# medical-genomics-group/VAMPomi

Measured on AMD Instinct MI355X. Metric: VAMP iterations/s (+ achieved HBM GB/s of the A/A^T kernels), higher is better.
Workload: dtype f64

## Files before the change

include/vampomi.h:

```cpp
#ifndef VAMPOMI_H
#define VAMPOMI_H

#include <stdint.h>

#ifdef __cplusplus
extern "C" {
#endif

#define VAMPOMI_ABI_VERSION 3
#define VAMPOMI_MAX_L 64
#define VAMPOMI_UNIQUE_ID_BYTES 128

typedef enum {
    VAMPOMI_OK = 0,
    VAMPOMI_ERR_ARG = 1,
    VAMPOMI_ERR_HIP = 2,
    VAMPOMI_ERR_RCCL = 3,
    VAMPOMI_ERR_IO = 4,
    VAMPOMI_ERR_NAN_PHEN = 5,
    VAMPOMI_ERR_STATE = 6,
    VAMPOMI_ERR_OOM = 7,
    VAMPOMI_ERR_MODEL = 8
} vampomi_status;

// ... 57 lines not shown

vampomi_status vampomi_denoise_bin(vampomi_ctx* ctx, const double* p1, double tau1, double* z1,
                                   double* sum_d, int mem);

typedef struct {
    double gam1, h2;
    int max_iter, CG_max_iter;
    double CG_err_tol;
    int EM_max_iter;
    double EM_err_thr, rho;
    int learn_vars, learn_prior_delay;
    double stop_criteria_thr, merge_vars_thr;
    int L;
    double vars[VAMPOMI_MAX_L];
    double probs[VAMPOMI_MAX_L];
    uint64_t seed;
    const char* out_dir;
    const char* out_name;
    int verbosity;
    const double* true_signal;
    const double* x1hat_init;
    int batch_rhs;
    const char* model;
} vampomi_params;

typedef struct {
    int iterations_run;
    int* cg_iters;
    int* ons_iters;
    int* L_hist;
    double* params;
    double* metrics;
    double* x1_hist;
    double* r1_hist;
    double* x1_final;
    double probs_final[VAMPOMI_MAX_L];
    double vars_final[VAMPOMI_MAX_L];
    int L_final;
    int64_t a_passes_ref;
    int64_t a_passes_exec;
    double* prior_hist;
} vampomi_result;

void vampomi_params_default(vampomi_params* p);
vampomi_status vampomi_infere(vampomi_ctx* ctx, const vampomi_params* p, vampomi_result* r);
vampomi_status vampomi_vamp_begin(vampomi_ctx* ctx, const vampomi_params* p, vampomi_result* r);
vampomi_status vampomi_vamp_step(vampomi_ctx* ctx, int* stopped);
vampomi_status vampomi_vamp_end(vampomi_ctx* ctx);
vampomi_status vampomi_step_phases(vampomi_ctx* ctx, double* solve_s, double* step_s);

vampomi_status vampomi_assoc_loo(vampomi_ctx* ctx, const double* est, double* pvals, double* stats,
                                 int mem);
vampomi_status vampomi_assoc_se(vampomi_ctx* ctx, const double* r1, double gam1, double* pvals, int mem);

vampomi_status vampomi_test_metrics(vampomi_ctx* ctx, const double* est, double* r2, double* corr2, int mem);

typedef struct {
    int64_t launches;
    double ms_total;
    double bytes_total;
    double flops_total;
    int64_t timed;
    double ms_timed;
} vampomi_kernel_stat;

typedef struct {
    vampomi_kernel_stat ax;
    vampomi_kernel_stat atx;
    vampomi_kernel_stat ax_k[4];
    vampomi_kernel_stat atx_k[4];
    int64_t a_passes_exec;
    int64_t host_syncs;
    vampomi_kernel_stat loo;
    vampomi_kernel_stat op;
    vampomi_kernel_stat op_k[4];
    vampomi_kernel_stat coll;
} vampomi_stats;

vampomi_status vampomi_set_timing(vampomi_ctx* ctx, int on);
vampomi_status vampomi_get_stats(vampomi_ctx* ctx, vampomi_stats* out);
vampomi_status vampomi_reset_stats(vampomi_ctx* ctx);

vampomi_status vampomi_dev_set_variant(vampomi_ctx* ctx, int which, int variant);
vampomi_status vampomi_dev_time_pass(vampomi_ctx* ctx, int which, int K, int reps, double* avg_ms);
vampomi_status vampomi_dev_read_ceiling(vampomi_ctx* ctx, int reps, double* us_med, double* bytes, int* variant);
vampomi_status vampomi_dev_kernel_name(const vampomi_ctx* ctx, int which, int K, int mode, char* out, int cap);
vampomi_status vampomi_dev_ax_plan(int64_t N, int64_t M, int cus, int variant, int K, int* T, int* TR, int* S,
                                   int* grid, int* nslots, char* name, int cap);
vampomi_status vampomi_dev_op_plan(int64_t N, int64_t M, int cus, int variant, int K, int* T, int* S, int* TR,
                                   int* grid, int64_t* nslots, char* name, int cap);
vampomi_status vampomi_dev_op_lds(int64_t N, int64_t M, int cus, int variant, int K, int64_t* out);
vampomi_status vampomi_dev_op_timestamps(vampomi_ctx* ctx, unsigned long long* out, int cap, int* n);
vampomi_status vampomi_dev_mem_plan(int64_t N, int64_t Mt, int nranks, int rank, int cus, int probit, int writer,
                                    int64_t* bytes);
vampomi_status vampomi_dev_op_apply(vampomi_ctx* ctx, int K, const double* ar, const double* qo, const double* p,
                                    const double* z, const double* beta, double diag, double tau, double gam2,
                                    double* d, double* ad, double* dp);

#ifdef __cplusplus
}
#endif
#endif
```

vampomi_amd/__init__.py:

```python
from __future__ import annotations

import ctypes as C
from dataclasses import dataclass, field
from typing import Optional, Sequence

import numpy as np

from ._lib import (CLI_PATH, GEN_GAUSS, GEN_METH, LIB_PATH, MAX_L, MEM_DEVICE, MEM_HOST, UNIQUE_ID_BYTES,
                   Params, Result, ShardDesc, Stats, VampomiError, check, load)

__all__ = ["Data", "Vamp", "VampOptions", "divide_work", "comm_unique_id", "VampomiError", "LIB_PATH", "CLI_PATH",
           "GEN_GAUSS", "GEN_METH", "load"]


def _dp(a: np.ndarray):
    return a.ctypes.data_as(C.c_void_p)


def divide_work(Mt: int, nranks: int, rank: int):
    M, S, Mm = C.c_int64(), C.c_int64(), C.c_int64()
    load().vampomi_divide_work(Mt, nranks, rank, C.byref(M), C.byref(S), C.byref(Mm))
    return M.value, S.value, Mm.value


# ... 134 lines not shown
        check(self._lib.vampomi_test_metrics(self.ctx, _dp(est), C.byref(r2), C.byref(c2), MEM_HOST))
        return r2.value, c2.value

    test_metrics.__test__ = False

    def assoc_loo(self, est: np.ndarray, mem_device: bool = False):
        est = np.ascontiguousarray(est, dtype=np.float64)
        if est.shape != (self.M,):
            raise ValueError("estimate slice must have M entries")
        pv = np.zeros(max(self.M, 1))
        st = np.zeros((max(self.M, 1), 5))
        check(self._lib.vampomi_assoc_loo(self.ctx, _dp(est), _dp(pv), _dp(st), MEM_HOST))
        return pv[: self.M], st[: self.M]

    def assoc_se(self, r1: np.ndarray, gam1: float) -> np.ndarray:
        r1 = np.ascontiguousarray(r1, dtype=np.float64)
        pv = np.zeros(max(self.M, 1))
        check(self._lib.vampomi_assoc_se(self.ctx, _dp(r1), gam1, _dp(pv), MEM_HOST))
        return pv[: self.M]

    def update_prior(self, r1: np.ndarray, gam1: float, probs, vars_scaled, EM_max_iter: int = 1,
                     EM_err_thr: float = 1e-2, learn_vars: int = 1, merge_vars_thr: float = 0.5):
        r1 = np.ascontiguousarray(r1, dtype=np.float64)
        L = C.c_int(len(probs))
        pr = np.zeros(MAX_L)
        va_ = np.zeros(MAX_L)
        pr[: L.value] = probs
        va_[: L.value] = vars_scaled
        check(self._lib.vampomi_update_prior(self.ctx, _dp(r1), gam1, C.byref(L), _dp(pr), _dp(va_), EM_max_iter,
                                             EM_err_thr, learn_vars, merge_vars_thr, MEM_HOST))
        return pr[: L.value].copy(), va_[: L.value].copy()

    def denoise_bin(self, p1: np.ndarray, tau1: float):
        p1 = np.ascontiguousarray(p1, dtype=np.float64)
        z = np.zeros(self.N)
        sd = C.c_double()
        check(self._lib.vampomi_denoise_bin(self.ctx, _dp(p1), tau1, _dp(z), C.byref(sd), MEM_HOST))
        return z, sd.value

    def denoise(self, r1: np.ndarray, gam1: float, probs: Sequence[float], vars_scaled: Sequence[float]):
        r1 = np.ascontiguousarray(r1, dtype=np.float64)
        L = len(probs)
        pr = np.ascontiguousarray(probs, dtype=np.float64)
        va = np.ascontiguousarray(vars_scaled, dtype=np.float64)
        x1 = np.zeros(max(self.M, 1))
        x1d = np.zeros(max(self.M, 1))
        s = C.c_double()
        check(self._lib.vampomi_denoise(self.ctx, _dp(r1), gam1, _dp(pr), _dp(va), L, _dp(x1), _dp(x1d),
                                        C.byref(s), MEM_HOST))
        return x1[: self.M], x1d[: self.M], s.value

    def kernel_name(self, which: int, K: int, mode: int = 0) -> str:
        buf = C.create_string_buffer(256)
        check(self._lib.vampomi_dev_kernel_name(self.ctx, which, K, mode, buf, 256))
        return buf.value.decode()

    def op_apply(self, ar, p, diag: float, tau: float, gam2: float, z=None, qo=None, beta=None):
        ar = np.ascontiguousarray(np.atleast_2d(ar), dtype=np.float64)
        p = np.ascontiguousarray(np.atleast_2d(p), dtype=np.float64)
        K = ar.shape[0]
        if ar.shape != (K, self.N) or p.shape != (K, self.M):
            raise ValueError("ar must be K x N and p K x M")
        fz = z is not None
        if fz:
            z = np.ascontiguousarray(np.atleast_2d(z), dtype=np.float64)
            qo = np.ascontiguousarray(np.atleast_2d(qo), dtype=np.float64)
            beta = np.ascontiguousarray(beta, dtype=np.float64)
        d = np.zeros((K, max(self.M, 1)))
        ad = np.zeros((K, self.N))
        dp = np.zeros(K)
        check(self._lib.vampomi_dev_op_apply(self.ctx, K, _dp(ar), _dp(qo) if fz else None, _dp(p),
                                             _dp(z) if fz else None, _dp(beta) if fz else None, diag, tau, gam2,
                                             _dp(d), _dp(ad), _dp(dp)))
        return d[:, : self.M], ad, dp

    def read_ceiling(self, reps: int = 9) -> dict:
        us, nb, var = C.c_double(), C.c_double(), C.c_int()
        check(self._lib.vampomi_dev_read_ceiling(self.ctx, int(reps), C.byref(us), C.byref(nb), C.byref(var)))
        return {"us_med": us.value, "bytes": nb.value, "GBs": nb.value / (us.value * 1e-6) / 1e9,
                "variant": ("lockstep 8-wave workgroups, one per CU", "1 MiB chunk per wave")[var.value]}

    def set_variant(self, which: int, variant: int):
        check(self._lib.vampomi_dev_set_variant(self.ctx, which, variant))

    def all_ok(self, local_ok: bool) -> bool:
        out = C.c_int()
        check(self._lib.vampomi_all_ok(self.ctx, 1 if local_ok else 0, C.byref(out)))
        return bool(out.value)

    def comm_abort(self):
        check(self._lib.vampomi_comm_abort(self.ctx))

    def set_timing(self, on: bool = True, period: int = 1):
        check(self._lib.vampomi_set_timing(self.ctx, (max(1, int(period)) if on else 0)))

    def stats(self) -> Stats:
        s = Stats()
        check(self._lib.vampomi_get_stats(self.ctx, C.byref(s)))
        return s

    def reset_stats(self):
        check(self._lib.vampomi_reset_stats(self.ctx))


@dataclass
class VampOptions:
    gam1: float = 1e-6
    h2: float = 0.5
    max_iter: int = 50
    CG_max_iter: int = 500
    CG_err_tol: float = 1e-5
    EM_max_iter: int = 1
    EM_err_thr: float = 1e-2
    rho: float = 0.5
    learn_vars: int = 1
    learn_prior_delay: int = 1
    stop_criteria_thr: float = 0.01
    merge_vars_thr: float = 0.5
    vars: Sequence[float] = (0, 1e-06, 6e-06, 3e-05, 2e-04, 1e-03, 6e-03, 3e-02, 2e-01, 1e+00)
    probs: Sequence[float] = (9.9e-01, 5e-03, 2.5e-03, 1.25e-03, 6.25e-04, 3.125e-04, 1.5625e-04, 7.8125e-05,
                              3.90625e-05, 3.90625e-05)
    seed: int = 0x5EED5EED
    out_dir: str = ""
    out_name: str = ""
    verbosity: int = 0
    batch_rhs: int = 4
    model: str = "linear"

    def to_struct(self) -> Params:
        p = Params()
        load().vampomi_params_default(C.byref(p))
        for k in ("gam1", "h2", "max_iter", "CG_max_iter", "CG_err_tol", "EM_max_iter", "EM_err_thr", "rho",
                  "learn_vars", "learn_prior_delay", "stop_criteria_thr", "merge_vars_thr", "seed", "verbosity",
                  "batch_rhs"):
            setattr(p, k, getattr(self, k))
        if len(self.vars) != len(self.probs) or not 1 <= len(self.vars) <= MAX_L:
            raise ValueError("vars and probs must have the same length (1..64)")
        p.L = len(self.vars)
        for j, (v, q) in enumerate(zip(self.vars, self.probs)):
            p.vars[j] = v
            p.probs[j] = q
        self._keep = [self.out_dir.encode(), self.out_name.encode(), self.model.encode()]
        p.out_dir, p.out_name, p.model = self._keep
        return p


class Vamp:

    def __init__(self, data: Data, opts: Optional[VampOptions] = None, true_signal: Optional[np.ndarray] = None,
                 x1hat_init: Optional[np.ndarray] = None):
        self.data = data
        self.opts = opts or VampOptions()
        self.true_signal = None if true_signal is None else np.ascontiguousarray(true_signal, dtype=np.float64)
        self.x1hat_init = None if x1hat_init is None else np.ascontiguousarray(x1hat_init, dtype=np.float64)
        self._active = False

    def _prepare(self, keep_hist: bool):
        o, M = self.opts, self.data.M
        it = o.max_iter
        self.p = o.to_struct()
        if self.true_signal is not None:
            self.p.true_signal = self.true_signal.ctypes.data
        if self.x1hat_init is not None:
            self.p.x1hat_init = self.x1hat_init.ctypes.data
        self.cg = np.zeros(it, dtype=np.int32)
        self.ons = np.zeros(it, dtype=np.int32)
# ... 70 lines not shown
```

vampomi_amd/_lib.py:

```python
from __future__ import annotations

import ctypes as C
import os

try:
    import torch
except Exception:
    torch = None

HERE = os.path.dirname(os.path.abspath(__file__))
LIB_PATH = os.environ.get("VAMPOMI_LIB") or os.path.join(HERE, "lib", "libvampomi.so")
CLI_PATH = os.path.join(HERE, "bin", "main_meth.exe")

MAX_L = 64
UNIQUE_ID_BYTES = 128
MEM_HOST, MEM_DEVICE = 0, 1
GEN_GAUSS, GEN_METH = 0, 1

STATUS = {
    0: "OK", 1: "ERR_ARG", 2: "ERR_HIP", 3: "ERR_RCCL", 4: "ERR_IO",
    5: "ERR_NAN_PHEN", 6: "ERR_STATE", 7: "ERR_OOM", 8: "ERR_MODEL",
}


# ... 19 lines not shown
        ("stop_criteria_thr", C.c_double), ("merge_vars_thr", C.c_double),
        ("L", C.c_int),
        ("vars", C.c_double * MAX_L), ("probs", C.c_double * MAX_L),
        ("seed", C.c_uint64),
        ("out_dir", C.c_char_p), ("out_name", C.c_char_p),
        ("verbosity", C.c_int),
        ("true_signal", C.c_void_p), ("x1hat_init", C.c_void_p),
        ("batch_rhs", C.c_int),
        ("model", C.c_char_p),
    ]


class Result(C.Structure):
    _fields_ = [
        ("iterations_run", C.c_int),
        ("cg_iters", C.POINTER(C.c_int)), ("ons_iters", C.POINTER(C.c_int)), ("L_hist", C.POINTER(C.c_int)),
        ("params", C.POINTER(C.c_double)), ("metrics", C.POINTER(C.c_double)),
        ("x1_hist", C.POINTER(C.c_double)), ("r1_hist", C.POINTER(C.c_double)),
        ("x1_final", C.POINTER(C.c_double)),
        ("probs_final", C.c_double * MAX_L), ("vars_final", C.c_double * MAX_L),
        ("L_final", C.c_int),
        ("a_passes_ref", C.c_int64), ("a_passes_exec", C.c_int64),
        ("prior_hist", C.POINTER(C.c_double)),
    ]


class KernelStat(C.Structure):
    _fields_ = [("launches", C.c_int64), ("ms_total", C.c_double), ("bytes_total", C.c_double),
                ("flops_total", C.c_double), ("timed", C.c_int64), ("ms_timed", C.c_double)]


class Stats(C.Structure):
    _fields_ = [("ax", KernelStat), ("atx", KernelStat), ("ax_k", KernelStat * 4), ("atx_k", KernelStat * 4),
                ("a_passes_exec", C.c_int64), ("host_syncs", C.c_int64), ("loo", KernelStat),
                ("op", KernelStat), ("op_k", KernelStat * 4), ("coll", KernelStat)]


_D = C.POINTER(C.c_double)
_P = C.c_void_p
SIGNATURES = {
    "vampomi_abi_version": (C.c_int, []),
    "vampomi_last_error": (C.c_char_p, []),
    "vampomi_divide_work": (None, [C.c_int64, C.c_int, C.c_int, C.POINTER(C.c_int64), C.POINTER(C.c_int64),
                                   C.POINTER(C.c_int64)]),
    "vampomi_comm_unique_id": (C.c_int, [_P]),
    "vampomi_open": (C.c_int, [C.POINTER(ShardDesc), C.POINTER(_P)]),
    "vampomi_close": (None, [_P]),
    "vampomi_shard_info": (C.c_int, [_P, C.POINTER(C.c_int64), C.POINTER(C.c_int64), C.POINTER(C.c_int64)]),
    "vampomi_sync": (C.c_int, [_P]),
    "vampomi_barrier": (C.c_int, [_P]),
    "vampomi_barrier_timeout": (C.c_int, [_P, C.c_double]),
    "vampomi_load_meth_file": (C.c_int, [_P, C.c_char_p]),
    "vampomi_load_meth_host": (C.c_int, [_P, _P, C.c_int64]),
    "vampomi_generate_meth": (C.c_int, [_P, C.c_uint64, C.c_int]),
    "vampomi_read_phen": (C.c_int, [_P, C.c_char_p, C.c_int]),
    "vampomi_set_phen": (C.c_int, [_P, _P, C.c_int]),
    "vampomi_get_phen": (C.c_int, [_P, _P]),
    "vampomi_simulate_phen": (C.c_int, [_P, C.c_uint64, C.c_double, C.c_double, _P]),
    "vampomi_simulate_phen_binary": (C.c_int, [_P, C.c_uint64, C.c_double, C.c_double, _P]),
    "vampomi_get_marker_stats": (C.c_int, [_P, _P, _P]),
    "vampomi_read_markers": (C.c_int, [_P, C.c_int64, C.c_int64, _P]),
    "vampomi_ax": (C.c_int, [_P, _P, _P, C.c_int]),
    "vampomi_atx": (C.c_int, [_P, _P, _P, C.c_int]),
    "vampomi_lmmse_mult": (C.c_int, [_P, _P, C.c_double, C.c_double, _P, C.c_int]),
    "vampomi_pcg": (C.c_int, [_P, _P, _P, C.c_double, C.c_double, C.c_int, C.c_int, C.c_double, _P,
                              C.POINTER(C.c_int), C.c_int]),
    "vampomi_test_metrics": (C.c_int, [_P, _P, C.POINTER(C.c_double), C.POINTER(C.c_double), C.c_int]),
    "vampomi_assoc_loo": (C.c_int, [_P, _P, _P, _P, C.c_int]),
    "vampomi_assoc_se": (C.c_int, [_P, _P, C.c_double, _P, C.c_int]),
    "vampomi_update_prior": (C.c_int, [_P, _P, C.c_double, C.POINTER(C.c_int), _P, _P, C.c_int, C.c_double,
                                        C.c_int, C.c_double, C.c_int]),
    "vampomi_denoise_bin": (C.c_int, [_P, _P, C.c_double, _P, C.POINTER(C.c_double), C.c_int]),
    "vampomi_denoise": (C.c_int, [_P, _P, C.c_double, _P, _P, C.c_int, _P, _P, C.POINTER(C.c_double), C.c_int]),
    "vampomi_params_default": (None, [C.POINTER(Params)]),
    "vampomi_infere": (C.c_int, [_P, C.POINTER(Params), C.POINTER(Result)]),
    "vampomi_vamp_begin": (C.c_int, [_P, C.POINTER(Params), C.POINTER(Result)]),
    "vampomi_vamp_step": (C.c_int, [_P, C.POINTER(C.c_int)]),
    "vampomi_step_phases": (C.c_int, [_P, C.POINTER(C.c_double), C.POINTER(C.c_double)]),
    "vampomi_vamp_end": (C.c_int, [_P]),
    "vampomi_set_timing": (C.c_int, [_P, C.c_int]),
    "vampomi_get_stats": (C.c_int, [_P, C.POINTER(Stats)]),
    "vampomi_reset_stats": (C.c_int, [_P]),
    "vampomi_dev_set_variant": (C.c_int, [_P, C.c_int, C.c_int]),
    "vampomi_dev_time_pass": (C.c_int, [_P, C.c_int, C.c_int, C.c_int, C.POINTER(C.c_double)]),
    "vampomi_dev_read_ceiling": (C.c_int, [_P, C.c_int, C.POINTER(C.c_double), C.POINTER(C.c_double),
                                           C.POINTER(C.c_int)]),
    "vampomi_dev_kernel_name": (C.c_int, [_P, C.c_int, C.c_int, C.c_int, C.c_char_p, C.c_int]),
    "vampomi_dev_mem_plan": (C.c_int, [C.c_int64, C.c_int64, C.c_int, C.c_int, C.c_int, C.c_int, C.c_int, _P]),
    "vampomi_dev_ax_plan": (C.c_int, [C.c_int64, C.c_int64, C.c_int, C.c_int, C.c_int, _P, _P, _P, _P, _P, C.c_char_p,
                                      C.c_int]),
    "vampomi_dev_op_plan": (C.c_int, [C.c_int64, C.c_int64, C.c_int, C.c_int, C.c_int, _P, _P, _P, _P, _P, C.c_char_p,
                                      C.c_int]),
    "vampomi_dev_op_lds": (C.c_int, [C.c_int64, C.c_int64, C.c_int, C.c_int, C.c_int, _P]),
    "vampomi_dev_op_apply": (C.c_int, [_P, C.c_int, _P, _P, _P, _P, _P, C.c_double, C.c_double, C.c_double, _P, _P,
                                       _P]),
    "vampomi_dev_op_timestamps": (C.c_int, [_P, _P, C.c_int, C.POINTER(C.c_int)]),
    "vampomi_all_ok": (C.c_int, [_P, C.c_int, C.POINTER(C.c_int)]),
    "vampomi_comm_abort": (C.c_int, [_P]),
}

_lib = None


def load() -> C.CDLL:
    global _lib
    if _lib is None:
        if not os.path.exists(LIB_PATH):
            raise ImportError(f"{LIB_PATH} not built: run `python -m vampomi_amd.build`")
        lib = C.CDLL(LIB_PATH, mode=C.RTLD_GLOBAL)
        other = bool(os.environ.get("VAMPOMI_LIB"))
        for name, (res, args) in SIGNATURES.items():
            if other and not hasattr(lib, name):
                continue
            f = getattr(lib, name)
            f.restype = res
            f.argtypes = args
        _lib = lib
    return _lib


def check(status: int) -> None:
    if status != 0:
        msg = load().vampomi_last_error()
        raise VampomiError(status, msg.decode() if msg else "")
```

vampomi_amd/csrc/atax_team.hip:

```cpp
#include <hip/hip_ext.h>

#include <algorithm>
#include <cstdio>
#include <mutex>
#include <string>

#include "kdev.h"

namespace vk {

typedef unsigned int v4u __attribute__((ext_vector_type(4)));
typedef unsigned int v2u __attribute__((ext_vector_type(2)));

#ifndef TM_FMA
#define TM_FMA 1
#endif
#ifndef TM_SAFE
#define TM_SAFE 0
#endif
#ifndef TM_TS
#define TM_TS 0
#endif
#ifndef TM_TEAMS_BY_XCD
#define TM_TEAMS_BY_XCD 1
// ... 59 lines not shown
    return __builtin_bit_cast(double, ((unsigned long long)hi << 32) | lo);
}

template <int CTRL>
__device__ __forceinline__ double dpp_d(double v) {
    const unsigned long long u = __builtin_bit_cast(unsigned long long, v);
    const unsigned lo = (unsigned)__builtin_amdgcn_mov_dpp((int)(unsigned)u, CTRL, 0xf, 0xf, false);
    const unsigned hi = (unsigned)__builtin_amdgcn_mov_dpp((int)(unsigned)(u >> 32), CTRL, 0xf, 0xf, false);
    return __builtin_bit_cast(double, ((unsigned long long)hi << 32) | lo);
}
__device__ __forceinline__ double pack_d(unsigned lo, unsigned hi) {
    return __builtin_bit_cast(double, ((unsigned long long)hi << 32) | lo);
}
__device__ __forceinline__ double swap16_sum(double v) {
    const unsigned long long u = __builtin_bit_cast(unsigned long long, v);
    const auto l = __builtin_amdgcn_permlane16_swap((unsigned)u, (unsigned)u, false, false);
    const auto h = __builtin_amdgcn_permlane16_swap((unsigned)(u >> 32), (unsigned)(u >> 32), false, false);
    return pack_d(l[0], h[0]) + pack_d(l[1], h[1]);
}
__device__ __forceinline__ void swap32(double a, double b, double& r0, double& r1) {
    const unsigned long long ua = __builtin_bit_cast(unsigned long long, a), ub = __builtin_bit_cast(unsigned long long, b);
    const auto l = __builtin_amdgcn_permlane32_swap((unsigned)ua, (unsigned)ub, false, false);
    const auto h = __builtin_amdgcn_permlane32_swap((unsigned)(ua >> 32), (unsigned)(ub >> 32), false, false);
    r0 = pack_d(l[0], h[0]);
    r1 = pack_d(l[1], h[1]);
}
template <int G>
__device__ __forceinline__ double group_sum(double v) {
    if constexpr (G >= 2) v = v + dpp_d<0xb1>(v);
    if constexpr (G >= 4) v = v + dpp_d<0x4e>(v);
    if constexpr (G >= 8) v = v + dpp_d<0x141>(v);
    if constexpr (G >= 16) v = v + dpp_d<0x140>(v);
    if constexpr (G >= 32) v = swap16_sum(v);
    if constexpr (G >= 64) {
        double a, b;
        swap32(v, v, a, b);
        v = a + b;
    }
    return v;
}

template <int N>
__device__ __forceinline__ double tree_sum(const double* x, int s) {
    if constexpr (N == 1) {
        return x[0];
    } else {
        constexpr int H = N / 2;
        return tree_sum<H>(x, s) + tree_sum<N - H>(x + H * s, s);
    }
}

__device__ __forceinline__ void tm_poll(v4u& dst, const unsigned long long* p) {
    asm volatile("global_load_dwordx4 %0, %1, off sc1" : "=v"(dst) : "v"(p) : "memory");
}
template <int N>
__device__ __forceinline__ void tm_wait(v4u& r) {
    asm volatile("s_waitcnt vmcnt(%1)" : "+v"(r) : "n"(N) : "memory");
}
__device__ __forceinline__ void tm_load8(v2u& dst, const double* p) {
    asm volatile("global_load_dwordx2 %0, %1, off" : "=v"(dst) : "v"(p) : "memory");
}
template <int N>
__device__ __forceinline__ void tm_wait2(v4u& r, v2u& q) {
    asm volatile("s_waitcnt vmcnt(%2)" : "+v"(r), "+v"(q) : "n"(N) : "memory");
}
__device__ __forceinline__ void tm_publish(unsigned long long* p, const v4u& v) {
    asm volatile("s_nop 4\n\tglobal_store_dwordx4 %0, %1, off sc1\n\ts_nop 1" ::"v"(p), "v"(v) : "memory");
}
__device__ __forceinline__ void tm_publish_l2(unsigned long long* p, const v4u& v) {
    asm volatile("s_nop 4\n\tglobal_store_dwordx4 %0, %1, off\n\ts_nop 1" ::"v"(p), "v"(v) : "memory");
}

template <class Tp>
__device__ __forceinline__ Tp* tm_chk(Tp* p, const void* lo, const void* hi, unsigned code, unsigned* err) {
#if TM_SAFE
    if ((const char*)p < (const char*)lo || (const char*)p >= (const char*)hi) {
        __hip_atomic_fetch_or(err, 1u | (code << 1), __ATOMIC_RELAXED, __HIP_MEMORY_SCOPE_SYSTEM);
        return (Tp*)lo;
    }
#endif
    return p;
}

template <int K, int S, int F, int L, int P, bool COMM, int E, bool FMA, int KP>
__device__ __forceinline__ void atax_team_body(const double* __restrict__ X, int64_t ld, int64_t N, int64_t M,
                                               const double* __restrict__ mave, const double* __restrict__ msig,
                                               const OpArgs& a, int T, int TR, int ilv,
                                               const int* __restrict__ gate) {
    extern __shared__ __attribute__((aligned(16))) double lds[];
    double* s_beta = lds;
    if (a.fold.on) {
        double& s_go = lds[kOpMaxK];
        if (threadIdx.x == 0) {
            CgState cs = *a.fold.src;
            double r[3 * kMaxRhs];
#pragma unroll
            for (int q = 0; q < 3 * kMaxRhs; ++q) r[q] = q < 3 * cs.K ? a.fold.red[q] : 0.0;
            const bool ran = cg_decide_into(cs, r, a.fold.it, a.fold.mask);
            if (blockIdx.x == 0) {
                *a.fold.dst = cs;
                cg_publish(cs, ran, a.fold.it, a.fold.mirror, a.fold.flag, a.fold.seq, a.fold.pack);
            }
            s_go = cs.any ? 1.0 : 0.0;
#pragma unroll
            for (int k = 0; k < kOpMaxK; ++k) s_beta[k] = cs.beta[k];
        }
        __syncthreads();
        if (s_go == 0.0) return;
    } else if (gate && !*gate) {
        return;
    }
    const double* beta = a.fold.on ? s_beta : a.beta;
    static_assert(K + KP <= kMaxRhs, "partial slots per team");
#if TM_TS
    const unsigned long long ts0 = __builtin_amdgcn_s_memrealtime();
#endif
    const int dbg = TM_ABL ? TM_ABL : (TM_DBG || !COMM) ? a.dbg : 0;
    constexpr int CW = COMM ? 7 : 8;
    constexpr int RS = tm_rows_per_step(COMM, E);
    static_assert(E == 1 || E == 2, "doubles per lane per load");
    constexpr int RING = F + L + 1;
    static_assert(COMM || L == 0, "without a hand-off the column is finished in its own step");
    static_assert(!COMM || (P >= 1 && P <= L), "polls in flight");
    static_assert(!COMM || P < RING, "a poll's slot is consumed before it is reissued");
    const int wave = threadIdx.x >> 6, lane = threadIdx.x & 63;
    const int g = blockIdx.x >> 3;
    const int member = g % T;
    const int nteams = gridDim.x / T;
#if TM_TEAMS_BY_XCD
    const int team = g / T + (nteams >> 3) * (int)(blockIdx.x & 7);
#else
    const int team = (blockIdx.x & 7) + 8 * (g / T);
#endif
    const int64_t cs = ilv ? nteams : 1;
    const int64_t mb = ilv ? team : (int64_t)team * M / nteams;
    const int n = (int)(ilv ? (M - team + nteams - 1) / nteams : (int64_t)(team + 1) * M / nteams - mb);
    const int64_t nmax = (M + nteams - 1) / nteams;
    const int64_t gwords = (M + gridDim.x) * kOpMaxK * T * 2;
    const int64_t r0 = (int64_t)member * TR;
    const int nrows = (int)(N - r0 < TR ? N - r0 : TR);
    constexpr bool QFULL = tm_qfull(K, S, COMM, E);
    const TmLds lay = tm_lds(K, S, COMM, E, TR < N ? TR : N);
    const int QS = (int)lay.qs;
    double* q_lds = lds + lay.q;
    double* s_part = lds + lay.part;
    double* s_tot = lds + lay.tot;
    const int jb = 64 * E * wave + E * lane;
    const int nbytes = (E == 2 ? (nrows + 1) & ~1 : nrows) * 8;

    if (COMM && wave == CW) {
        const int nq = K * T;
        unsigned long long* xg = a.xg + (int64_t)team * nmax * nq * 2;
        unsigned long long* dummy = a.xg + gwords + (int64_t)blockIdx.x * 2 * K;
        const bool qv = (lane >> 5) < K && (lane & 31) < T;
        const int ql2 = qv ? 2 * ((lane >> 5) * T + (lane & 31)) : 0;
        const int nq2 = 2 * nq;
        const int csi = (int)cs;
        const unsigned tag = a.tag;
        const double* scp = msig;
#pragma unroll
        for (int k = 0; k < K; ++k) {
            if (lane == 1 + k) scp = a.p.p[k];
            if (lane == 1 + K + k && ((a.fuse >> k) & 1)) scp = a.z.p[k];
        }
        scp += mb;
        double bk[K], dpacc[K];
#pragma unroll
        for (int k = 0; k < K; ++k) {
            bk[k] = ((a.fuse >> k) & 1) ? beta[k] : 0.0;
            dpacc[k] = 0.0;
        }
        v4u pl[RING];
        v2u ps[RING];
        bool dead = false;
        unsigned nslow = 0, nspin = 0;
        if (n > 0) {
            bool l2 = false;
            {
                unsigned long long* hdr = a.xg + gwords + (int64_t)gridDim.x * 2 * kOpMaxK + (int64_t)team * T;
                unsigned xcc;
                asm volatile("s_getreg_b32 %0, hwreg(HW_REG_XCC_ID)" : "=s"(xcc));
                xcc &= 0xf;
                if (lane == 0)
                    __hip_atomic_store(hdr + member, ((unsigned long long)tag << 32) | xcc, __ATOMIC_RELAXED,
                                       __HIP_MEMORY_SCOPE_AGENT);
                unsigned long long h = 0;
                for (unsigned spins = 0;; ++spins) {
                    h = lane < T ? __hip_atomic_load(hdr + lane, __ATOMIC_RELAXED, __HIP_MEMORY_SCOPE_AGENT)
                                 : ((unsigned long long)tag << 32) | xcc;
                    if (__all((unsigned)(h >> 32) == tag)) break;
                    if (spins >= kTmMaxSpins) {
                        dead = true;
                        if (lane == 0) __hip_atomic_store(a.err, 1u, __ATOMIC_RELAXED, __HIP_MEMORY_SCOPE_SYSTEM);
                        break;
                    }
                    __builtin_amdgcn_s_sleep(2);
                }
                l2 = !dead && __all((unsigned)h == xcc);
                if (dbg & 32) l2 = false;
            }
            for (int base = -F; base - L < n; base += RING) {
#pragma unroll
                for (int i = 0; i < RING; ++i) {
                    const int m = base + i;
                    if (dbg & 4096) {
                        __syncthreads();
                        continue;
                    }
                    const int ci = m - L + P, cf = m - L;
                    const int cic = ci < 0 ? 0 : ci < n ? ci : n - 1;
                    tm_load8(ps[(i + RING - L + P) % RING], scp + cic * csi);
                    tm_poll(pl[(i + RING - L + P) % RING], xg + (cic * nq2 + ql2));
                    v4u& g = pl[(i + RING - L) % RING];
                    v2u& sc = ps[(i + RING - L) % RING];
                    if (!(dbg & 1)) tm_wait2<3 * P>(g, sc);
                    if (cf >= 0 && cf < n) {
                        if (!(__all(g.y == tag && g.w == tag) || dead || (dbg & 1))) {
#pragma unroll 1
                            for (unsigned spins = 0;; ++spins) {
                                if (dbg & 64) {
                                    nslow += spins == 0;
                                    nspin++;
                                }
                                if (spins >= kTmMaxSpins) {
                                    dead = true;
                                    if (lane == 0) __hip_atomic_store(a.err, 1u, __ATOMIC_RELAXED, __HIP_MEMORY_SCOPE_SYSTEM);
                                    break;
                                }
                                __builtin_amdgcn_s_sleep(2);
                                tm_poll(g, tm_chk(xg + ((int64_t)cf * nq2 + ql2), a.xg, a.xg + gwords, 64, a.err));
                                tm_wait<0>(g);
                                if (__all(g.y == tag && g.w == tag)) break;
                            }
                        }
                        double v = qv ? __builtin_bit_cast(double, ((unsigned long long)g.z << 32) | g.x) : 0.0;
                        if (dbg & 512) {
                            for (int o = T >> 1; o > 0; o >>= 1) v += __shfl_xor(v, o, 64);
                        } else if (!(dbg & 256)) {
                            v = group_sum<32>(v);
                        }
                        const double scv = __builtin_bit_cast(double, ((unsigned long long)sc.y << 32) | sc.x);
                        const double sg = readlane_d(scv, 0);
                        const bool own = (cf & (T - 1)) == member;
                        const int64_t mg = mb + cf * csi;
                        double tsc[K], dval[K], pdir[K];
#pragma unroll
                        for (int k = 0; k < K; ++k) {
                            double t = sg * readlane_d(v, 32 * k);
                            t *= a.scale;
                            double p = readlane_d(scv, 1 + k);
                            if ((a.fuse >> k) & 1) p = readlane_d(scv, 1 + K + k) + bk[k] * p;
                            double val = t * a.tau;
                            val += a.gam2 * p;
                            tsc[k] = t;
                            dval[k] = val;
                            pdir[k] = p;
                        }
#pragma unroll
                        for (int k = 0; k < K; ++k)
                            if (lane == 0) s_tot[(cf & 1) * K + k] = (dbg & 128) ? 0.0 : sg * dval[k];
                        if (own) {
#pragma unroll
                            for (int k = 0; k < K; ++k) {
                                if (lane == 0 && !(dbg & 1024)) {
                                    if (a.sraw.p[0]) a.sraw.p[k][mg] = tsc[k];
                                    *tm_chk(a.d.p[k] + mg, a.d.p[k], a.d.p[k] + M, 128, a.err) = dval[k];
                                }
                                dpacc[k] += dval[k] * pdir[k];
                            }
                        }
                    }
                    __syncthreads();
                    if (lane < K && !(dbg & 2)) {
                        const bool real = m >= 0 && m < n;
                        double v = 0.0;
                        if (real) v = tree_sum<CW>(s_part + (m & 1) * CW * K + lane, K);
                        const unsigned long long u = __builtin_bit_cast(unsigned long long, v);
                        const v4u gr = {(unsigned)u, tag, (unsigned)(u >> 32), tag};
                        unsigned long long* dst =
                            tm_chk(real ? xg + ((int64_t)m * nq2 + (lane * T + member) * 2) : dummy + 2 * lane, a.xg,
                                   a.xg + gwords + (int64_t)gridDim.x * 2 * kOpMaxK, 512, a.err);
                        if (l2)
                            tm_publish_l2(dst, gr);
                        else
                            tm_publish(dst, gr);
                    }
                }
            }
#pragma unroll
            for (int s = 0; s < RING; ++s) tm_wait2<0>(pl[s], ps[s]);
            if ((dbg & 64) && lane == 0) {
                __hip_atomic_fetch_add(a.err + 1, nslow, __ATOMIC_RELAXED, __HIP_MEMORY_SCOPE_SYSTEM);
                __hip_atomic_fetch_add(a.err + 2, nspin, __ATOMIC_RELAXED, __HIP_MEMORY_SCOPE_SYSTEM);
                __hip_atomic_fetch_add(a.err + 3, (unsigned)n, __ATOMIC_RELAXED, __HIP_MEMORY_SCOPE_SYSTEM);
            }
        }
        if (lane == 0) {
#pragma unroll
            for (int k = 0; k < K; ++k) red_put(a.ro, (int64_t)blockIdx.x * K + k, dpacc[k]);
        }
        asm volatile("s_waitcnt vmcnt(0)" ::: "memory");
        __syncthreads();
        return;
    }

#pragma unroll
    for (int s = 0; s < S; ++s) {
        const int jl = RS * s + jb;
        if (jl >= QS) continue;
#pragma unroll
        for (int k = 0; k < K; ++k) {
#pragma unroll
            for (int h = 0; h < E; ++h) {
                double q = 0.0;
                if (jl + h < nrows) {
                    const int64_t j = r0 + jl + h;
                    q = a.ar.p[k][j] / a.diag;
                    if ((a.fuse >> k) & 1) q = q + beta[k] * a.qo.p[k][j];
                }
                q_lds[k * QS + jl + h] = q;
            }
        }
    }
    double bk[K];
#pragma unroll
    for (int k = 0; k < K; ++k) bk[k] = ((a.fuse >> k) & 1) ? beta[k] : 0.0;
    const double* pkp = mave;
    if (lane == 1) pkp = msig;
#pragma unroll
    for (int k = 0; k < K; ++k) {
        if (lane == 2 + k) pkp = a.p.p[k];
        if (lane == 2 + K + k && ((a.fuse >> k) & 1)) pkp = a.z.p[k];
    }
#pragma unroll
    for (int k = 0; k < KP; ++k)
        if (lane == 2 + 2 * K + k) pkp = a.px.p[k];
    pkp += mb;
    bool valid[S];
#pragma unroll
    for (int s = 0; s < S; ++s) valid[s] = RS * s + jb < nrows;
    double acc[K][S][E];
#pragma unroll
    for (int k = 0; k < K; ++k)
#pragma unroll
        for (int s = 0; s < S; ++s)
#pragma unroll
            for (int e = 0; e < E; ++e) acc[k][s][e] = 0.0;
    double dpacc[K];
#pragma unroll
    for (int k = 0; k < K; ++k) dpacc[k] = 0.0;
    constexpr int KPA = KP > 0 ? KP : 1;
    double accp[KPA][S][E];
#pragma unroll
    for (int k = 0; k < KPA; ++k)
#pragma unroll
        for (int s = 0; s < S; ++s)
#pragma unroll
            for (int e = 0; e < E; ++e) accp[k][s][e] = 0.0;

    double xr[RING][S][E];
    double pk[RING];
    const char* xtile = reinterpret_cast<const char*>(X + mb * ld + r0);
    auto load = [&](int slot, int m) {
        const int64_t c = m * cs;
        pk[slot] = *tm_chk(pkp + c, pkp - mb, pkp - mb + M, 1024, a.err);
        const __amdgpu_buffer_rsrc_t rs =
            __builtin_amdgcn_make_buffer_rsrc((void*)(xtile + c * ld * 8), (short)0, nbytes, 0x00020000);
#pragma unroll
        for (int s = 0; s < S; ++s) {
            if constexpr (E == 2) {
                const v2d x = __builtin_bit_cast(v2d, __builtin_amdgcn_raw_buffer_load_b128(rs, (RS * s + jb) * 8, 0, 2));
                xr[slot][s][0] = x.x;
                xr[slot][s][E - 1] = x.y;
            } else {
                xr[slot][s][0] = __builtin_bit_cast(double, __builtin_amdgcn_raw_buffer_load_b64(rs, (RS * s + jb) * 8, 0, 2));
            }
        }
    };
    auto dot = [&](int slot, int par) {
        const double mu = readlane_d(pk[slot], 0);
        double cp[KPA];
        if constexpr (KP > 0) {
            const double sgp = readlane_d(pk[slot], 1);
#pragma unroll
            for (int k = 0; k < KP; ++k) cp[k] = sgp * readlane_d(pk[slot], 2 + 2 * K + k);
        }
        double v[K];
#pragma unroll
        for (int k = 0; k < K; ++k) v[k] = 0.0;
#pragma unroll
        for (int s = 0; s < S; ++s) {
            const double me_ = QFULL || valid[s] ? mu : 0.0;
            const int jq = QFULL || RS * s + jb < QS ? RS * s + jb : QS - E;
            double dx[E], q[K][E];
#pragma unroll
            for (int e = 0; e < E; ++e) {
                dx[e] = xr[slot][s][e] - me_;
                xr[slot][s][e] = dx[e];
            }
            if constexpr (KP > 0) {
#pragma unroll
                for (int k = 0; k < KP; ++k)
#pragma unroll
                    for (int e = 0; e < E; ++e) {
                        if constexpr (FMA)
                            accp[k][s][e] = __builtin_fma(dx[e], cp[k], accp[k][s][e]);
                        else
                            accp[k][s][e] += dx[e] * cp[k];
                    }
            }
#pragma unroll
            for (int k = 0; k < K; ++k) {
                if ((TM_DBG || TM_ABL) && (dbg & 2048)) {
                    q[k][0] = 0.5;
                    q[k][E - 1] = 0.25;
                } else if constexpr (E == 2) {
                    const v2d qq = *reinterpret_cast<const v2d*>(q_lds + k * QS + jq);
                    q[k][0] = qq.x;
                    q[k][E - 1] = qq.y;
                } else {
                    q[k][0] = q_lds[k * QS + jq];
                }
#pragma unroll
                for (int e = 0; e < E; ++e) {
                    if constexpr (FMA)
                        v[k] = __builtin_fma(dx[e], q[k][e], v[k]);
                    else
                        v[k] += dx[e] * q[k][e];
                }
            }
        }
        if (K == 2) {
            double r0, r1;
            swap32(v[0], v[K - 1], r0, r1);
            double keep = r0 + r1;
            if (dbg & 512) {
                for (int o = 16; o > 0; o >>= 1) keep += __shfl_xor(keep, o, 64);
            } else if (!(dbg & 4)) {
                keep = group_sum<32>(keep);
            }
            if ((lane & 31) == 0) s_part[(par * CW + wave) * K + (lane >> 5)] = keep;
        } else {
            if (!(dbg & 4)) v[0] = group_sum<64>(v[0]);
            if (lane == 0) s_part[(par * CW + wave) * K] = v[0];
        }
    };
    auto finish = [&](int slot, int m, const double (&tot)[K]) {
        double cc[K];
        if constexpr (COMM) {
#pragma unroll
            for (int k = 0; k < K; ++k) cc[k] = tot[k];
        } else {
            const double sg = readlane_d(pk[slot], 1);
            const bool own = (m % T) == member;
            const int64_t mg = mb + m * cs;
#pragma unroll
            for (int k = 0; k < K; ++k) {
                double t = sg * tot[k];
                t *= a.scale;
                double p = readlane_d(pk[slot], 2 + k);
                if ((a.fuse >> k) & 1) p = readlane_d(pk[slot], 2 + K + k) + bk[k] * p;
                double val = t * a.tau;
                val += a.gam2 * p;
                if (own) {
                    if (threadIdx.x == 0) {
                        if (a.sraw.p[0]) a.sraw.p[k][mg] = t;
                        a.d.p[k][mg] = val;
                    }
                    dpacc[k] += val * p;
                }
                cc[k] = sg * val;
            }
        }
#pragma unroll
        for (int s = 0; s < S; ++s) {
            if (dbg & 8) break;
#pragma unroll
            for (int k = 0; k < K; ++k)
#pragma unroll
                for (int e = 0; e < E; ++e) {
                    if constexpr (FMA)
                        acc[k][s][e] = __builtin_fma(xr[slot][s][e], cc[k], acc[k][s][e]);
                    else
                        acc[k][s][e] += xr[slot][s][e] * cc[k];
                }
        }
    };
    if (n > 0) {
        for (int base = -F;; base += RING) {
            if (base - L >= n) break;
#pragma unroll
            for (int i = 0; i < RING; ++i) {
                const int m = base + i;
                load((i + F) % RING, m + F < n ? m + F : n - 1);
                if (m >= 0 && m < n) dot(i, m & 1);
                __syncthreads();
                const int cf = m - L;
                if (cf >= 0 && cf < n) {
                    double tot[K];
                    if (COMM) {
#pragma unroll
                        for (int k = 0; k < K; ++k) tot[k] = s_tot[(cf & 1) * K + k];
                    } else {
#pragma unroll
                        for (int k = 0; k < K; ++k) {
                            double t = 0.0;
#pragma unroll
                            for (int w = 0; w < CW; ++w) t += s_part[((m & 1) * CW + w) * K + k];
                            tot[k] = t;
                        }
                    }
                    finish((i + RING - L) % RING, cf, tot);
                }
            }
        }
    }
    double* dst = a.part + (int64_t)team * kMaxRhs * ld + r0;
#pragma unroll
    for (int s = 0; s < S; ++s) {
        const int jl = RS * s + jb;
        if (jl >= nrows) continue;
#pragma unroll
        for (int k = 0; k < K; ++k)
#pragma unroll
            for (int e = 0; e < E; ++e)
                if (jl + e < nrows) dst[(int64_t)k * ld + jl + e] = acc[k][s][e];
        if constexpr (KP > 0) {
#pragma unroll
            for (int k = 0; k < KP; ++k)
#pragma unroll
                for (int e = 0; e < E; ++e)
                    if (jl + e < nrows) dst[(int64_t)(K + k) * ld + jl + e] = accp[k][s][e];
        }
    }
    if constexpr (COMM) {
        __syncthreads();
    } else if (threadIdx.x == 0) {
#pragma unroll
        for (int k = 0; k < K; ++k) red_put(a.ro, (int64_t)blockIdx.x * K + k, dpacc[k]);
    }
    if (wave == 0) ticket_sum_blocks<K>(a.ro);
#if TM_TS
    if (a.ts && threadIdx.x == 0) {
        unsigned xcc, hw;
        asm volatile("s_getreg_b32 %0, hwreg(HW_REG_XCC_ID)" : "=s"(xcc));
        asm volatile("s_getreg_b32 %0, hwreg(HW_REG_HW_ID)" : "=s"(hw));
        unsigned long long* t = a.ts + 4 * (int64_t)blockIdx.x;
        t[0] = ts0;
        t[1] = __builtin_amdgcn_s_memrealtime();
        t[2] = xcc;
// ... 147 lines not shown
    if (S > c.maxS) return false;
    for (int K = 1; K <= kOpMaxK; ++K)
        if (tm_lds(K, S, c.comm, c.E, std::min<int64_t>(TR, N)).words * 8 > kTmLdsMaxBytes) return false;
    OpPlan p{};
    p.grid = grid;
    p.S = S;
    p.T = T;
    p.TR = (int)TR;
    p.cfg = cfg;
    p.nslots = grid / T;
    (void)M;
    *out = p;
    return true;
}

bool team_lds_layout(const OpPlan& pl, int64_t N, int K, int64_t out[6]) {
    if (pl.T < 1 || pl.cfg < 0 || pl.cfg >= kTmNCfg || K < 1 || K > kOpMaxK || N < 1) return false;
    const TmCfg& c = kTmCfg[pl.cfg];
    const TmLds l = tm_lds(K, pl.S, c.comm, c.E, std::min<int64_t>(pl.TR, N));
    out[0] = kTmLdsHead;
    out[1] = l.q;
    out[2] = l.qs;
    out[3] = l.part;
    out[4] = l.tot;
    out[5] = l.words;
    return true;
}

template <int K, int S, int C, bool PL>
static hipError_t launch_tm(const Shard& s, const OpPlan& pl, const OpArgs& a, hipStream_t st, const Timing& tm,
                            const int* gate, int* occ) {
    constexpr TmCfg c = kTmCfg[C];
    static_assert(!PL || K == 1, "the head-start kernel has one operator system");
    void (*kern)(const double*, int64_t, int64_t, int64_t, const double*, const double*, OpArgs, int, int, int,
                 const int*);
    if constexpr (PL)
        kern = atax_team_plain_kernel<S, c.F, c.L, c.P, c.comm, c.E, (bool)TM_FMA>;
    else
        kern = atax_team_kernel<K, S, c.F, c.L, c.P, c.comm, c.E, (bool)TM_FMA>;
    const size_t lds = (size_t)tm_lds(K, S, c.comm, c.E, std::min<int64_t>(pl.TR, s.N)).words * sizeof(double);
    if (lds > (size_t)kTmLdsMaxBytes) return hipErrorInvalidValue;
    static std::atomic<unsigned long long> allowed{0};
    if (const hipError_t e = lds_allow(reinterpret_cast<const void*>(kern), allowed, (int)kTmLdsMaxBytes))
        return e;
    if (occ) {
        if (hipOccupancyMaxActiveBlocksPerMultiprocessor(occ, kern, kTmThreads, lds) != hipSuccess) *occ = 0;
        return hipSuccess;
    }
    hipExtLaunchKernelGGL(kern, dim3(pl.grid), dim3(kTmThreads), lds, st, tm.start, tm.stop, 0, s.X, s.ld, s.N, s.M,
                          s.mave, s.msig, a, pl.T, pl.TR, c.ilv ? 1 : 0, gate);
    return hipSuccess;
}

static constexpr int tm_plain_maxS(int cfg) {
    return cfg == 0 ? 8 : cfg == 2 ? 3 : cfg == 3 ? 4 : cfg == 4 ? 5 : 0;
}

template <int K, int C, int S, bool PL>
static hipError_t launch_tm_if(const Shard& s, const OpPlan& pl, const OpArgs& a, hipStream_t st, const Timing& tm,
                               const int* gate, int* occ) {
    if constexpr (S <= (PL ? tm_plain_maxS(C) : kTmCfg[C].maxS))
        return launch_tm<K, S, C, PL>(s, pl, a, st, tm, gate, occ);
    return hipErrorInvalidValue;
}

template <int K, int C, bool PL>
static hipError_t launch_tm_s(int S, const Shard& s, const OpPlan& pl, const OpArgs& a, hipStream_t st,
                        const Timing& tm, const int* gate, int* occ) {
    switch (S) {
        case 1: return launch_tm_if<K, C, 1, PL>(s, pl, a, st, tm, gate, occ);
        case 2: return launch_tm_if<K, C, 2, PL>(s, pl, a, st, tm, gate, occ);
        case 3: return launch_tm_if<K, C, 3, PL>(s, pl, a, st, tm, gate, occ);
        case 4: return launch_tm_if<K, C, 4, PL>(s, pl, a, st, tm, gate, occ);
        case 5: return launch_tm_if<K, C, 5, PL>(s, pl, a, st, tm, gate, occ);
        case 6: return launch_tm_if<K, C, 6, PL>(s, pl, a, st, tm, gate, occ);
        case 7: return launch_tm_if<K, C, 7, PL>(s, pl, a, st, tm, gate, occ);
        case 8: return launch_tm_if<K, C, 8, PL>(s, pl, a, st, tm, gate, occ);
        case 9: return launch_tm_if<K, C, 9, PL>(s, pl, a, st, tm, gate, occ);
        case 10: return launch_tm_if<K, C, 10, PL>(s, pl, a, st, tm, gate, occ);
        default: return hipErrorInvalidValue;
    }
}

template <int K, bool PL = false>
static hipError_t launch_tm_c(const Shard& s, const OpPlan& pl, const OpArgs& a, hipStream_t st, const Timing& tm,
                        const int* gate, int* occ = nullptr) {
    if constexpr (PL) {
        switch (pl.cfg) {
            case 0: return launch_tm_s<1, 0, true>(pl.S, s, pl, a, st, tm, gate, occ);
            case 2: return launch_tm_s<1, 2, true>(pl.S, s, pl, a, st, tm, gate, occ);
            case 3: return launch_tm_s<1, 3, true>(pl.S, s, pl, a, st, tm, gate, occ);
            case 4: return launch_tm_s<1, 4, true>(pl.S, s, pl, a, st, tm, gate, occ);
            default: return hipErrorInvalidValue;
        }
    }
    switch (pl.cfg) {
        case 0: return launch_tm_s<K, 0, false>(pl.S, s, pl, a, st, tm, gate, occ);
        case 1: return launch_tm_s<K, 1, false>(pl.S, s, pl, a, st, tm, gate, occ);
        case 2: return launch_tm_s<K, 2, false>(pl.S, s, pl, a, st, tm, gate, occ);
        case 3: return launch_tm_s<K, 3, false>(pl.S, s, pl, a, st, tm, gate, occ);
        case 4: return launch_tm_s<K, 4, false>(pl.S, s, pl, a, st, tm, gate, occ);
        case 5: return launch_tm_s<K, 5, false>(pl.S, s, pl, a, st, tm, gate, occ);
        case 6: return launch_tm_s<K, 6, false>(pl.S, s, pl, a, st, tm, gate, occ);
        default: return hipErrorInvalidValue;
    }
}

hipError_t atax_team(const Shard& s, const OpPlan& pl, int K, const OpArgs& a, hipStream_t st, const Timing& tm,
                     const int* gate) {
    if (pl.T < 1 || pl.grid < pl.T || pl.grid % pl.T) return hipErrorInvalidValue;
    if (pl.T > 1 && (!a.xg || !a.err || a.tag == 0)) return hipErrorInvalidValue;
    if (s.M <= 0) return hipSuccess;
    hipError_t e = hipErrorInvalidValue;
    switch (K) {
        case 1: e = launch_tm_c<1>(s, pl, a, st, tm, gate); break;
        case 2: e = launch_tm_c<2>(s, pl, a, st, tm, gate); break;
        default: break;
    }
    if (e != hipSuccess) return e;
    return hipGetLastError();
}

hipError_t atax_team_plain(const Shard& s, const OpPlan& pl, const OpArgs& a, hipStream_t st, const Timing& tm,
                           const int* gate) {
    if (pl.T < 1 || pl.grid < pl.T || pl.grid % pl.T) return hipErrorInvalidValue;
    if (pl.T > 1 && (!a.xg || !a.err || a.tag == 0)) return hipErrorInvalidValue;
    for (int k = 0; k < kTmPlain; ++k)
        if (!a.px.p[k]) return hipErrorInvalidValue;
    if (s.M <= 0) return hipSuccess;
    if (const hipError_t e = launch_tm_c<1, true>(s, pl, a, st, tm, gate)) return e;
    return hipGetLastError();
}

bool ax_team_plan(int64_t N, int64_t M, int cus, AxPlan* out) {
    if (N < 1 || cus < 8) return false;
    constexpr int RS = tm_rows_per_step(false, 2);
    for (int T = 1; T <= kTmMaxT; T *= 2) {
        if (cus / (8 * T) < 1) break;
        const int grid = (cus / (8 * T)) * 8 * T;
        const int64_t TR = T == 1 ? N : ((N + T - 1) / T + 127) / 128 * 128;
        if ((int64_t)(T - 1) * TR >= N) continue;
        const int S = (int)((TR + RS - 1) / RS);
        if (S > kAxTmMaxS) continue;
        AxPlan p{};
        p.variant = kAxTeam;
        p.T = T;
        p.TR = (int)TR;
        p.S = S;
        p.groups = grid;
        p.nslots = grid / T;
        p.rows = N;
        p.tiles = 1;
        p.total = M;
        p.sa = p.nslots;
        p.sb = 1;
        *out = p;
        return true;
    }
    return false;
}

template <int S, int K, bool FU>
static void launch_axt(const Shard& s, const AxPlan& pl, CPtrs x, double* part, hipStream_t st, const Timing& tm,
                       const AxFuse& fu) {
    hipExtLaunchKernelGGL((ax_team_kernel<S, K, FU>), dim3(pl.groups), dim3(kTmThreads), 0, st, tm.start, tm.stop, 0,
                          s.X, s.ld, s.N, s.M, s.mave, s.msig, x, part, fu, pl.T, pl.TR);
}

template <int S>
// ... 87 lines not shown
```

vampomi_amd/csrc/ctx.h:

```cpp
#pragma once
#include <hip/hip_runtime.h>
#include <rccl/rccl.h>

#include <cstdint>
#include <initializer_list>
#include <memory>
#include <string>
#include <utility>
#include <vector>

#include "../../include/vampomi.h"
#include "kernels.h"

vampomi_status fail(vampomi_status s, const std::string& msg);

#define HIPCHK(expr)                                                                                  \
    do {                                                                                              \
        hipError_t _e = (expr);                                                                       \
        if (_e != hipSuccess)                                                                         \
            return fail(VAMPOMI_ERR_HIP, std::string(#expr) + ": " + hipGetErrorString(_e));          \
    } while (0)

#define NCCLCHK(expr)                                                                                 \
    do {                                                                                              \
// ... 13 lines not shown
    explicit CollScope(vampomi_ctx* c);
    ~CollScope();
    vampomi_ctx* prev;
};
struct VampRun;
class IterWriter;
struct LoopbackComm;
struct ShmComm;
std::shared_ptr<ShmComm> shm_join(const void* id, int P, int rank, double limit_s, std::string* err);
std::string shm_allreduce(ShmComm& s, int rank, double* buf, size_t n, uint64_t seq, const char* site, int line,
                          double limit_s);
void shm_poison(ShmComm& s, const std::string& why);

struct TimedLaunch {
    hipEvent_t a, b;
    int cls;
    int K;
    double bytes, flops;
};

enum : int { SL_DP = 0, SL_CG = 4, SL_SYNC = 16, SL_NSYNC = 256, SL_LOCAL = SL_SYNC + SL_NSYNC, SL_NLOCAL = 128,
             SL_CGI = SL_LOCAL + SL_NLOCAL, SL_CHECK = SL_CGI + 16, SL_AGREE = SL_CHECK + 8, SL_CHAIN = SL_AGREE + 8, SL_TOTAL = 512, SL_BARRIER = SL_TOTAL - 1 };

struct vampomi_ctx {
    int rank = 0, nranks = 1, device = 0;
    int64_t N = 0, Mt = 0, M = 0, S = 0, Mm = 0, ld = 0;
    double alpha_scale = 1.0;
    double sqrtN = 1.0;
    hipStream_t st = nullptr;
    bool mr_tail = true;
    double coll_limit_s = 0.0;
    bool mr_tail_req = true;
    bool cg_fold = true;
    bool team_reg = false;
    hipEvent_t team_ev = nullptr;
    ncclComm_t comm = nullptr;
    bool use_comm = false;
    std::shared_ptr<LoopbackComm> loopback;
    std::shared_ptr<ShmComm> shm;
    uint64_t coll_seq = 0;
    bool aborted = false;

    double* X = nullptr;
    double* mave = nullptr;
    double* msig = nullptr;
    double* y = nullptr;
    std::vector<double> y_host;
    bool have_X = false, have_y = false;

    vk::AxPlan axp{};
    int atx_variant = vk::kAtxDefault, loo_variant = vk::kLooDefault;
    double* ax_part = nullptr;
    double* red_part = nullptr;
    size_t red_cap = 0;
    double* scal = nullptr;
    double* h_scal = nullptr;
    double* d_hscal = nullptr;
    unsigned* ticket = nullptr;
    unsigned long long* h_flag = nullptr;
    unsigned long long* d_flag = nullptr;
    unsigned long long sync_seq = 0;
    vk::CgState* cgs = nullptr;
    vk::CgMirror* h_cgm = nullptr;
    vk::CgMirror* d_cgm = nullptr;
    vk::OpPlan opp{};
    int op_variant = vk::kOpDefault;
    bool op_ready = false;
    bool op_ok_mine = false;
    bool op_ok = false;
    bool op_agreed = false;
    int op_variant_req = vk::kOpDefault;
    int cus = 0;
    double* op_part = nullptr;
    int64_t op_part_slots = 0;
    double* op_nvec = nullptr;
    unsigned long long* op_xg = nullptr;
    size_t op_xg_words = 0;
    unsigned op_tag = 0;
    vk::OpPlan opp_hs{};
    bool hs_ok_mine = false;
    bool hs_ok = false;
    bool hs_on = true;
    bool hs_on_req = true;
    unsigned long long* op_ts = nullptr;
    double* nbuf = nullptr;
    double* mbuf = nullptr;

    bool timing = false;
    int tperiod = 1;
    int64_t tcount[5][vk::kMaxRhs] = {};
    std::vector<TimedLaunch> pending;
    std::vector<hipEvent_t> ev_pool;
    vampomi_stats stats{};

    std::unique_ptr<VampRun> run;
    std::unique_ptr<IterWriter> writer;

    vk::Shard shard() const { return vk::Shard{X, ld, N, M, mave, msig}; }
    vampomi_ctx();
    ~vampomi_ctx();
};

vampomi_status dev_alloc(double** p, size_t n);
void dev_free(double*& p);
vampomi_status host_sync(vampomi_ctx* c);
vampomi_status wait_flag(vampomi_ctx* c, unsigned long long seq, int word = 0);
vampomi_status sync_stream(vampomi_ctx* c, hipStream_t st);
vampomi_status allreduce_dev(vampomi_ctx* c, double* buf, size_t n, const char* site = __builtin_FUNCTION(),
                             int line = __builtin_LINE());
vampomi_status sum_over_ranks(vampomi_ctx* c, double local, double* total, const char* site = __builtin_FUNCTION(),
                              int line = __builtin_LINE());
void comm_abort(vampomi_ctx* c, const std::string& why);
void resolve_timing(vampomi_ctx* c);
TimedLaunch launch_stat(vampomi_ctx* c, int cls, int K, double bytes, double flops);
void drop_launches(vampomi_ctx* c, size_t pending_mark, const vampomi_stats& before);
void release_ctx_resources(vampomi_ctx* c);

vampomi_status ax_dev(vampomi_ctx* c, int K, const double* const* x, double* outbase,
                      const vk::AxFuse* fu = nullptr, const vk::DotArgs* tail = nullptr);
vampomi_status atx_dev(vampomi_ctx* c, int K, const double* const* u, double* const* out, int mode, double tau,
                       double gam2, const double* const* p, const int* gate = nullptr,
                       const double* const* zf = nullptr, const double* beta = nullptr, bool dp = true,
                       double* const* sraw = nullptr);
vampomi_status lmmse_dev(vampomi_ctx* c, int K, const double* const* v, double* const* d, double tau, double gam2,
                         double* nscratch);

class DotBatch {
   public:
    explicit DotBatch(vampomi_ctx* c) : c_(c) {}
    vampomi_status add(std::initializer_list<vk::DotTerm> terms, int64_t n, bool sync, double* out);
    struct Group {
        std::vector<vk::DotTerm> terms;
        bool sync;
        double* out;
    };
    vampomi_status add_many(int64_t n, const std::vector<Group>& groups, const vk::G1Chain* chain = nullptr,
                            const double* chain_of = nullptr,
                            const std::vector<std::pair<const double*, double*>>& copies = {});
    vampomi_status add_pair(int64_t na, const std::vector<Group>& ga, const vk::G1Chain* chain,
                            const double* chain_of, const std::vector<std::pair<const double*, double*>>& ca,
                            int64_t nb, const std::vector<Group>& gb,
                            const std::vector<std::pair<const double*, double*>>& cb);
    vampomi_status sink(int nq, bool sync, double* out, vk::RedOut* ro);
    vampomi_status flush();
    bool empty() const { return sinks_.empty(); }
    const double* dev_result(const double* out) const;
    vampomi_status reduce_now();
    double* dev_slot(const double* out) const;
    hipStream_t stream() const;

   private:
    vampomi_status build(const std::vector<Group>& groups, const vk::G1Chain* chain, const double* chain_of,
                         const std::vector<std::pair<const double*, double*>>& copies, vk::DotArgs& a,
                         vk::RedOut& ro);
    struct Sink {
        int slot, count;
        double* out;
    };
    vampomi_ctx* c_;
    int nsync_ = 0, nlocal_ = 0;
    int nred_ = 0;
    unsigned long long last_seq_ = 0;
    std::vector<Sink> sinks_;
};

inline vk::DotTerm T(const double* a, const double* b, int op = vk::DOT) { return vk::DotTerm{a, b, op}; }

struct CgSystem {
    const double* v = nullptr;
    double* mu = nullptr;
    bool mu0_nonzero = false;
    const double* atx0 = nullptr;
    double* W = nullptr;
    double* S = nullptr;
    double* AW = nullptr;
    bool onsager = false;
    int iters = 0;
    double *r = nullptr, *z = nullptr, *p = nullptr, *d = nullptr;
};
struct HeadStart {
    double* abern = nullptr;
    const double* xnext = nullptr;
    double* axnext = nullptr;
    bool used = false;
};
enum class PreMode { normal, ahead, queued };
vampomi_status pcg_run(vampomi_ctx* c, const std::vector<CgSystem*>& sys, double tau, double gam2, int max_iter,
                       double tol, double* nscratch, int64_t* ref_passes, DotBatch* init,
                       const double* extra_x = nullptr, double* ex_out = nullptr, bool onepass = false,
                       const double* const* ar0 = nullptr, HeadStart* hs = nullptr,
                       const vk::Prelude* pre = nullptr, PreMode pm = PreMode::normal);
vampomi_status op_prepare(vampomi_ctx* c);
vampomi_status op_agree(vampomi_ctx* c);
vampomi_status headstart_available(vampomi_ctx* c, bool* yes);
unsigned* op_err_dev(vampomi_ctx* c);
vampomi_status op_check_err(vampomi_ctx* c);
vampomi_status op_dev(vampomi_ctx* c, int K, const vk::OpArgs& a, const int* gate, bool reduce = true,
                      bool divide = true);
vampomi_status op_dev_plain(vampomi_ctx* c, const vk::OpArgs& a, const double* const* px, double* const* out,
                            const int* gate);
```

vampomi_amd/csrc/engine.cpp:

```cpp
#include <hip/hip_runtime.h>
#include <rccl/rccl.h>

#include <algorithm>
#include <atomic>
#include <cfloat>
#include <chrono>
#include <condition_variable>
#include <map>
#include <mutex>
#include <cmath>
#include <cstdio>
#include <cstdlib>
#include <cstring>
#include <memory>
#include <string>
#include <thread>
#include <vector>

#include <fcntl.h>
#include <unistd.h>

#include "ctx.h"
#include "hostio.h"
#include "writer.h"
// ... 948 lines not shown
    c->op_part_slots = 0;
    c->op_ready = false;
    c->op_agreed = false;
    if (c->h_scal) (void)hipHostFree(c->h_scal);
    c->h_scal = nullptr;
    if (c->ticket) (void)hipFree(c->ticket);
    c->ticket = nullptr;
    if (c->h_flag) (void)hipHostFree(c->h_flag);
    c->h_flag = nullptr;
    if (c->h_cgm) (void)hipHostFree(c->h_cgm);
    c->h_cgm = nullptr;
    if (c->cgs) (void)hipFree(c->cgs);
    c->cgs = nullptr;
    if (c->comm) {
        if (nccl_settle(c, ncclCommFinalize(c->comm), "ncclCommFinalize", 30.0) == VAMPOMI_OK && c->comm)
            (void)ncclCommDestroy(c->comm);
        else if (c->comm)
            (void)ncclCommAbort(c->comm);
    }
    c->comm = nullptr;

    if (c->st) (void)hipStreamDestroy(c->st);
    c->st = nullptr;
}

extern "C" void vampomi_close(vampomi_ctx* c) { delete c; }

extern "C" vampomi_status vampomi_open(const vampomi_shard_desc* d, vampomi_ctx** out) {
    if (!d || !out) return fail(VAMPOMI_ERR_ARG, "null argument");
    *out = nullptr;
    if (d->N < 2 || d->Mt < 1 || d->nranks < 1 || d->rank < 0 || d->rank >= d->nranks)
        return fail(VAMPOMI_ERR_ARG, "invalid shard description (N >= 2, Mt >= 1, 0 <= rank < nranks)");
    if (d->nranks > 1 && !d->comm_id) return fail(VAMPOMI_ERR_ARG, "nranks > 1 needs a communicator id");
    if (d->Mt < d->nranks) return fail(VAMPOMI_ERR_ARG, "every rank needs at least one marker (Mt >= nranks)");
    std::unique_ptr<vampomi_ctx> c(new vampomi_ctx());
    c->rank = d->rank;
    c->nranks = d->nranks;
    c->N = d->N;
    c->Mt = d->Mt;
    c->alpha_scale = d->alpha_scale == 0.0 ? 1.0 : d->alpha_scale;
    vampomi_divide_work(c->Mt, c->nranks, c->rank, &c->M, &c->S, &c->Mm);
    c->ld = (c->N + 15) / 16 * 16;
    c->sqrtN = std::sqrt((double)c->N);
    int ndev = 0;
    HIPCHK(hipGetDeviceCount(&ndev));
    if (ndev < 1) return fail(VAMPOMI_ERR_HIP, "no HIP device visible");
    c->device = d->device >= 0 ? d->device : c->rank % ndev;
    HIPCHK(hipSetDevice(c->device));
    HIPCHK(hipStreamCreateWithFlags(&c->st, hipStreamNonBlocking));
    team_gate_join(c.get());
    const int64_t Mx = std::max<int64_t>(c->M, 1);
    c->axp = vk::ax_plan(c->N, Mx);
    STCHK(dev_alloc(&c->mave, Mx));
    STCHK(dev_alloc(&c->msig, Mx));
    STCHK(dev_alloc(&c->y, c->ld));
    HIPCHK(hipMemsetAsync(c->y, 0, c->ld * 8, c->st));
    STCHK(dev_alloc(&c->ax_part, (size_t)c->axp.nslots * vk::kMaxRhs * c->ld));
    c->red_cap = red_capacity(Mx);
    STCHK(dev_alloc(&c->red_part, c->red_cap));
    c->writer.reset(new IterWriter());
    STCHK(c->writer->open(c.get()));
    STCHK(dev_alloc(&c->scal, SL_TOTAL));
    HIPCHK(hipHostMalloc((void**)&c->h_scal, SL_TOTAL * sizeof(double), hipHostMallocMapped | hipHostMallocCoherent));
    HIPCHK(hipHostGetDevicePointer((void**)&c->d_hscal, c->h_scal, 0));
    HIPCHK(hipHostMalloc((void**)&c->h_flag, 64, hipHostMallocMapped | hipHostMallocCoherent));
    std::memset(c->h_flag, 0, 64);
    HIPCHK(hipHostGetDevicePointer((void**)&c->d_flag, c->h_flag, 0));
    HIPCHK(hipMalloc((void**)&c->ticket, 64 * sizeof(unsigned)));
    HIPCHK(hipMemsetAsync(c->ticket, 0, 64 * sizeof(unsigned), c->st));
    STCHK(dev_alloc(&c->nbuf, (size_t)vk::kMaxRhs * c->ld));
    HIPCHK(hipMemsetAsync(c->nbuf, 0, (size_t)vk::kMaxRhs * c->ld * 8, c->st));
    STCHK(dev_alloc(&c->mbuf, (size_t)2 * vk::kMaxRhs * Mx));
    HIPCHK(hipMalloc((void**)&c->cgs, 2 * sizeof(vk::CgState)));
    HIPCHK(hipMemsetAsync(c->cgs, 0, 2 * sizeof(vk::CgState), c->st));
    HIPCHK(hipHostMalloc((void**)&c->h_cgm, vk::kCgMirrorSlots * sizeof(vk::CgMirror),
                         hipHostMallocMapped | hipHostMallocCoherent));
    std::memset(c->h_cgm, 0, vk::kCgMirrorSlots * sizeof(vk::CgMirror));
    HIPCHK(hipHostGetDevicePointer((void**)&c->d_cgm, c->h_cgm, 0));
    const char* force = std::getenv("VAMPOMI_FORCE_RCCL");
    c->use_comm = c->nranks > 1 || (force && std::atoi(force) != 0);
    if (const char* mv = std::getenv("VAMPOMI_MR_TAIL")) c->mr_tail = c->mr_tail_req = std::atoi(mv) != 0;
    if (const char* fv = std::getenv("VAMPOMI_CG_FOLD")) c->cg_fold = std::atoi(fv) != 0;
    if (const char* hv = std::getenv("VAMPOMI_HEADSTART")) c->hs_on = c->hs_on_req = std::atoi(hv) != 0;
    const char* mode = std::getenv("VAMPOMI_COMM");
    if (c->use_comm && mode && std::strcmp(mode, "loopback") == 0) {
        if (!d->comm_id) return fail(VAMPOMI_ERR_ARG, "the loopback communicator needs a communicator id");
        c->loopback = loopback_join(d->comm_id, c->nranks);
    } else if (c->use_comm && mode && std::strcmp(mode, "shm") == 0) {
        if (!d->comm_id) return fail(VAMPOMI_ERR_ARG, "the shm communicator needs a communicator id");
        std::string err;
        c->shm = shm_join(d->comm_id, c->nranks, c->rank, comm_init_timeout_s(), &err);
        if (!c->shm) return fail(VAMPOMI_ERR_STATE, err);
    } else if (c->use_comm) {
        ncclUniqueId id;
        if (d->comm_id)
            std::memcpy(&id, d->comm_id, sizeof id);
        else
            NCCLCHK(ncclGetUniqueId(&id));
        ncclConfig_t cfg = NCCL_CONFIG_INITIALIZER;
        cfg.blocking = 0;
        STCHK(nccl_settle(c.get(), ncclCommInitRankConfig(&c->comm, c->nranks, id, c->rank, &cfg),
                          "ncclCommInitRankConfig", comm_init_timeout_s()));
    }
    STCHK(sync_stream(c.get(), c->st));
    *out = c.release();
    return VAMPOMI_OK;
}

extern "C" vampomi_status vampomi_shard_info(const vampomi_ctx* c, int64_t* M, int64_t* S, int64_t* ld) {
    if (!c) return fail(VAMPOMI_ERR_ARG, "null context");
    if (M) *M = c->M;
    if (S) *S = c->S;
    if (ld) *ld = c->ld;
    return VAMPOMI_OK;
}

extern "C" vampomi_status vampomi_sync(vampomi_ctx* c) {
    if (!c) return fail(VAMPOMI_ERR_ARG, "null context");
    HIPCHK(hipSetDevice(c->device));
    STCHK(sync_stream(c, c->st));
    return VAMPOMI_OK;
}

extern "C" vampomi_status vampomi_barrier(vampomi_ctx* c) {
    CollScope cs_(c);
    if (!c) return fail(VAMPOMI_ERR_ARG, "null context");
    if (c->use_comm) STCHK(allreduce_dev(c, c->scal + SL_BARRIER, 1));
    STCHK(sync_stream(c, c->st));
    return VAMPOMI_OK;
}

extern "C" vampomi_status vampomi_barrier_timeout(vampomi_ctx* c, double seconds) {
    if (!c || !(seconds > 0)) return fail(VAMPOMI_ERR_ARG, "null context or no limit");
    c->coll_limit_s = seconds;
    const vampomi_status st = vampomi_barrier(c);
    c->coll_limit_s = 0.0;
    return st;
}

static vampomi_status ensure_X(vampomi_ctx* c) {
    if (c->X) return VAMPOMI_OK;
    return dev_alloc(&c->X, (size_t)std::max<int64_t>(c->M, 1) * (size_t)c->ld);
}

static vampomi_status finish_X(vampomi_ctx* c) {
    if (c->ld > c->N && c->M > 0)
        HIPCHK(hipMemset2DAsync(c->X + c->N, (size_t)c->ld * 8, 0, (size_t)(c->ld - c->N) * 8, (size_t)c->M, c->st));
    HIPCHK(vk::marker_stats(c->X, c->ld, c->N, c->M, (double)c->N, c->alpha_scale, c->mave, c->msig, c->st));
    STCHK(sync_stream(c, c->st));
    c->have_X = true;
    return VAMPOMI_OK;
}

extern "C" vampomi_status vampomi_load_meth_host(vampomi_ctx* c, const double* X, int64_t ld_in) {
    if (!c || (!X && c->M > 0) || ld_in < c->N) return fail(VAMPOMI_ERR_ARG, "invalid host shard");
    HIPCHK(hipSetDevice(c->device));
    STCHK(ensure_X(c));
    if (c->M > 0)
        HIPCHK(hipMemcpy2DAsync(c->X, (size_t)c->ld * 8, X, (size_t)ld_in * 8, (size_t)c->N * 8, (size_t)c->M,
                                hipMemcpyHostToDevice, c->st));
    return finish_X(c);
}

static bool pread_parallel(int fd, char* dst, size_t want, off_t off, int nt) {
    if (nt <= 1 || want < ((size_t)8 << 20)) nt = 1;
    const size_t per = ((want + nt - 1) / nt + 4095) & ~(size_t)4095;
// ... 392 lines not shown

extern "C" vampomi_status vampomi_assoc_se(vampomi_ctx* c, const double* r1, double gam1, double* pvals, int mem) {
    if (!c || (!r1 && c->M > 0) || (!pvals && c->M > 0)) return fail(VAMPOMI_ERR_ARG, "null argument");
    HIPCHK(hipSetDevice(c->device));
    const int64_t Mx = std::max<int64_t>(c->M, 1);
    STCHK(stage_in(c, r1, c->M, mem, c->mbuf));
    HIPCHK(vk::se_pvals(c->M, c->mbuf, gam1, c->N, c->mbuf + Mx, c->st));
    STCHK(stage_out(c, c->mbuf + Mx, c->M, mem, pvals));
    return VAMPOMI_OK;
}

extern "C" vampomi_status vampomi_set_timing(vampomi_ctx* c, int on) {
    if (!c) return fail(VAMPOMI_ERR_ARG, "null context");
    c->timing = on != 0;
    c->tperiod = on > 1 ? on : 1;
    for (auto& row : c->tcount)
        for (auto& n : row) n = 0;
    return VAMPOMI_OK;
}

extern "C" vampomi_status vampomi_get_stats(vampomi_ctx* c, vampomi_stats* out) {
    if (!c || !out) return fail(VAMPOMI_ERR_ARG, "null argument");
    STCHK(sync_stream(c, c->st));
    resolve_timing(c);
    *out = c->stats;
    auto fill = [](vampomi_kernel_stat& x) {
        x.ms_total = x.timed > 0 ? x.ms_timed / (double)x.timed * (double)x.launches : 0.0;
    };
    for (vampomi_kernel_stat* x : {&out->loo, &out->coll}) fill(*x);
    for (int k = 0; k < 4; ++k)
        for (vampomi_kernel_stat* x : {&out->ax_k[k], &out->atx_k[k], &out->op_k[k]}) fill(*x);
    for (auto pr : {std::make_pair(&out->ax, out->ax_k), std::make_pair(&out->atx, out->atx_k),
                    std::make_pair(&out->op, out->op_k)}) {
        int64_t n = 0;
        double ms = 0.0;
        for (int k = 0; k < 4; ++k) {
            n += pr.second[k].launches;
            ms += pr.second[k].ms_total;
        }
        if (n == pr.first->launches) pr.first->ms_total = ms;
        else fill(*pr.first);
    }
    return VAMPOMI_OK;
}

extern "C" vampomi_status vampomi_reset_stats(vampomi_ctx* c) {
    if (!c) return fail(VAMPOMI_ERR_ARG, "null context");
    STCHK(sync_stream(c, c->st));
    resolve_timing(c);
    c->stats = vampomi_stats{};
    return VAMPOMI_OK;
}

extern "C" vampomi_status vampomi_dev_set_variant(vampomi_ctx* c, int which, int variant) {
    if (!c) return fail(VAMPOMI_ERR_ARG, "null context");
    HIPCHK(hipSetDevice(c->device));
    STCHK(sync_stream(c, c->st));
    if (which == 0) {
        if (!vk::ax_variant_ok(variant)) return fail(VAMPOMI_ERR_ARG, "no such A.x variant");
        const vk::AxPlan np = vk::ax_plan(c->N, std::max<int64_t>(c->M, 1), variant);
        if (np.nslots > c->axp.nslots) {
            dev_free(c->ax_part);
            STCHK(dev_alloc(&c->ax_part, (size_t)np.nslots * vk::kMaxRhs * c->ld));
        }
        c->axp = np;
    } else if (which == 1) {
        if (!vk::atx_variant_ok(variant)) return fail(VAMPOMI_ERR_ARG, "no such A^T.u variant");
        c->atx_variant = variant;
    } else if (which == 3) {
        vk::OpPlan p{};
        if (!vk::op_plan(c->N, std::max<int64_t>(c->M, 1), c->cus > 0 ? c->cus : 256, variant, &p))
            return fail(VAMPOMI_ERR_ARG, "no such one-pass operator plan for this N");
        c->op_variant_req = variant;
        if (!c->use_comm) {
            c->op_variant = variant;
            c->op_ready = false;
        }
    } else if (which == 4) {
        return fail(VAMPOMI_ERR_ARG, "no side stream: every launch runs on the context's stream (DESIGN.md §6)");
    } else if (which == 5) {
        if (variant != 0 && variant != 1) return fail(VAMPOMI_ERR_ARG, "head start: 0 or 1");
        c->hs_on_req = variant == 1;
        if (!c->use_comm) c->hs_on = c->hs_on_req;
    } else if (which == 6) {
        if (variant != 0 && variant != 1) return fail(VAMPOMI_ERR_ARG, "multi-rank tail: 0 or 1");
        c->mr_tail_req = variant == 1;
        if (!c->use_comm) c->mr_tail = c->mr_tail_req;
    } else {
        if (!vk::loo_variant_ok(variant)) return fail(VAMPOMI_ERR_ARG, "no such association-pass variant");
        c->loo_variant = variant;
    }
    return VAMPOMI_OK;
}

extern "C" vampomi_status vampomi_dev_time_pass(vampomi_ctx* c, int which, int K, int reps, double* avg_ms) {
    if (!c || !avg_ms || K < 1 || K > (which == 0 ? 4 : which == 1 ? 3 : which == 3 ? 2 : 1) || reps < 1)
        return fail(VAMPOMI_ERR_ARG, "bad argument");
    if (!c->have_X) return fail(VAMPOMI_ERR_STATE, "no methylation data loaded");
    HIPCHK(hipSetDevice(c->device));
    if (which == 3) {
        STCHK(op_prepare(c));
        if (!c->op_ok_mine) return fail(VAMPOMI_ERR_ARG, "no one-pass operator plan for this N");
    }
    const int64_t Mx = std::max<int64_t>(c->M, 1);
    vk::CPtrs in{};
    vk::Ptrs out{};
    for (int k = 0; k < K; ++k) {
        in.p[k] = which == 0 ? c->mbuf + k * Mx : c->nbuf + k * c->ld;
        out.p[k] = which == 0 ? c->nbuf + k * c->ld : c->mbuf + k * Mx;
    }
    hipEvent_t a, b;
    HIPCHK(hipEventCreate(&a));
    HIPCHK(hipEventCreate(&b));
    HIPCHK(hipEventRecord(a, c->st));
    for (int r = 0; r < reps; ++r) {
        if (which == 0)
            HIPCHK(vk::ax_partial(c->shard(), c->axp, K, in, c->ax_part, c->st));
        else if (which == 1)
            HIPCHK(vk::atx(c->shard(), K, in, out, 1.0 / c->sqrtN, 0, 0.0, 0.0, vk::CPtrs{}, c->st, c->atx_variant));
        else if (which == 3) {
            vk::OpArgs x{};
            for (int k = 0; k < K; ++k) {
                x.ar.p[k] = c->nbuf + k * c->ld;
                x.p.p[k] = c->mbuf + k * Mx;
                x.d.p[k] = c->mbuf + (2 + k) * Mx;
            }
            x.diag = 1.0;
            x.scale = 1.0 / c->sqrtN;
            x.tau = 1.0;
            x.part = c->op_part;
            x.ro = vk::RedOut{c->red_part, c->scal + SL_DP, c->ticket, nullptr, 0, nullptr};
            if (c->opp.T > 1) {
                x.xg = c->op_xg;
                if (++c->op_tag == 0) ++c->op_tag;
                x.tag = c->op_tag;
                x.err = op_err_dev(c);
            }
            x.dbg = std::getenv("VAMPOMI_OP_DBG") ? std::atoi(std::getenv("VAMPOMI_OP_DBG")) : 0;
            if (c->opp.T > 1) x.err = op_err_dev(c);
            x.ts = c->op_ts;
            STCHK(team_launch(c, c->opp.T, [&] { return vk::atax(c->shard(), c->opp, K, x, c->st); }));
        }
        else
            HIPCHK(vk::loo_sums(c->shard(), c->nbuf, c->mbuf, c->sqrtN, c->mbuf + 3 * Mx, c->st, c->loo_variant));
    }
    HIPCHK(hipEventRecord(b, c->st));
    HIPCHK(hipEventSynchronize(b));
    if (which == 3 && std::getenv("VAMPOMI_OP_DBG") && (std::atoi(std::getenv("VAMPOMI_OP_DBG")) & 64)) {
        unsigned* w = reinterpret_cast<unsigned*>(c->h_flag + 4);
        std::fprintf(stderr, "op dbg: slow polls %u, spins %u, columns polled %u (over %d launches)\n", w[1], w[2], w[3],
                     reps);
        w[1] = w[2] = w[3] = 0;
    }
    float ms = 0.f;
    HIPCHK(hipEventElapsedTime(&ms, a, b));
    (void)hipEventDestroy(a);
    (void)hipEventDestroy(b);
    *avg_ms = (double)ms / reps;
    return VAMPOMI_OK;
}

extern "C" vampomi_status vampomi_dev_op_apply(vampomi_ctx* c, int K, const double* ar, const double* qo,
                                               const double* p, const double* z, const double* beta, double diag,
                                               double tau, double gam2, double* d, double* ad, double* dp) {
    if (!c || K < 1 || K > vk::kOpMaxK || !ar || !p || !d || !ad || !dp || (z && (!qo || !beta)))
        return fail(VAMPOMI_ERR_ARG, "bad argument");
    if (c->use_comm) return fail(VAMPOMI_ERR_ARG, "vampomi_dev_op_apply: one rank only");
    HIPCHK(hipSetDevice(c->device));
    STCHK(op_prepare(c));
    if (!c->op_ok) return fail(VAMPOMI_ERR_ARG, "no one-pass operator plan for this N");
    const int64_t Mx = std::max<int64_t>(c->M, 1);
    double* AR = c->op_nvec;
    double* Q = c->op_nvec + (int64_t)vk::kMaxRhs * c->ld;
    vk::OpArgs a{};
// ... 28 lines not shown
    }
    HIPCHK(hipMemcpyAsync(dp, c->scal + SL_DP, (size_t)K * 8, hipMemcpyDeviceToHost, c->st));
    STCHK(sync_stream(c, c->st));
    return op_check_err(c);
}

extern "C" vampomi_status vampomi_dev_op_timestamps(vampomi_ctx* c, unsigned long long* out, int cap, int* n) {
    if (!c || !out || !n) return fail(VAMPOMI_ERR_ARG, "null argument");
    if (!c->op_ts) return fail(VAMPOMI_ERR_STATE, "no timestamps (VAMPOMI_OP_TS=1 at the first operator use)");
    STCHK(sync_stream(c, c->st));
    *n = std::min(cap, 4 * c->opp.grid);
    HIPCHK(hipMemcpy(out, c->op_ts, (size_t)*n * 8, hipMemcpyDeviceToHost));
    return VAMPOMI_OK;
}

extern "C" vampomi_status vampomi_dev_ax_plan(int64_t N, int64_t M, int cus, int variant, int K, int* T, int* TR,
                                              int* S, int* grid, int* nslots, char* name, int cap) {
    if (N < 1 || M < 1 || cus < 1 || K < 1 || K > vk::kMaxRhs || !vk::ax_variant_ok(variant))
        return fail(VAMPOMI_ERR_ARG, "bad argument");
    const vk::AxPlan p = vk::ax_plan_for(N, M, cus, variant);
    if (T) *T = p.T;
    if (TR) *TR = p.TR;
    if (S) *S = p.S;
    if (grid) *grid = p.groups;
    if (nslots) *nslots = p.nslots;
    if (name && cap > 0) std::snprintf(name, (size_t)cap, "%s", vk::ax_kernel_name(K, false, p).c_str());
    return VAMPOMI_OK;
}

extern "C" vampomi_status vampomi_dev_op_plan(int64_t N, int64_t M, int cus, int variant, int K, int* T, int* S,
                                              int* TR, int* grid, int64_t* nslots, char* name, int cap) {
    vk::OpPlan p{};
    if (K < 1 || K > vk::kOpMaxK || !vk::op_plan(N, std::max<int64_t>(M, 1), cus, variant, &p))
        return fail(VAMPOMI_ERR_ARG, "no one-pass operator plan");
    if (T) *T = p.T;
    if (S) *S = p.S;
    if (TR) *TR = p.TR;
    if (grid) *grid = p.grid;
    if (nslots) *nslots = p.nslots;
    if (name && cap > 0) std::snprintf(name, (size_t)cap, "%s", vk::op_kernel_name(K, p).c_str());
    return VAMPOMI_OK;
}

extern "C" vampomi_status vampomi_dev_op_lds(int64_t N, int64_t M, int cus, int variant, int K, int64_t* out) {
    vk::OpPlan p{};
    if (!out || !vk::op_plan(N, std::max<int64_t>(M, 1), cus, variant, &p) || !vk::team_lds_layout(p, N, K, out))
        return fail(VAMPOMI_ERR_ARG, "no team plan with that system count");
    return VAMPOMI_OK;
}

extern "C" vampomi_status vampomi_dev_mem_plan(int64_t N, int64_t Mt, int nranks, int rank, int cus, int probit,
                                               int writer, int64_t* bytes) {
    if (!bytes || N < 2 || Mt < nranks || nranks < 1 || rank < 0 || rank >= nranks || cus < 1)
        return fail(VAMPOMI_ERR_ARG, "bad argument");
    int64_t M = 0, S = 0, Mm = 0;
    vampomi_divide_work(Mt, nranks, rank, &M, &S, &Mm);
    const int64_t Mx = std::max<int64_t>(M, 1), ld = (N + 15) / 16 * 16;
    int64_t total = 0;
    auto add = [&](int64_t n, int64_t elem) {
        const int64_t b = std::max<int64_t>(n, 1) * elem, g = 2 << 20;
        total += (b + g - 1) / g * g;
    };
    const vk::AxPlan axp = vk::ax_plan(N, Mx);
    add(Mx * ld, 8);
    add(Mx, 8), add(Mx, 8), add(ld, 8);
    add((int64_t)axp.nslots * vk::kMaxRhs * ld, 8);
    add((int64_t)red_capacity(Mx), 8), add((int64_t)red_capacity(Mx), 8);
    add(SL_TOTAL, 8), add(64, 4), add(64, 4);
    add((int64_t)vk::kMaxRhs * ld, 8);
    add((int64_t)2 * vk::kMaxRhs * Mx, 8);
    add((int64_t)sizeof(vk::CgState), 1);
    vk::OpPlan op{}, hs{};
    if (vk::op_plan(N, Mx, cus, vk::kOpDefault, &op)) {
        const bool h = vk::team_plain_plan(N, Mx, cus, op, &hs);
        add((int64_t)3 * vk::kMaxRhs * ld + 16, 8);
        add(std::max<int64_t>(op.nslots, h ? hs.nslots : 0) * vk::kMaxRhs * ld, 8);
        size_t w = op.T > 1 ? op_xg_words_for(Mx, op) : 0;
        if (h && hs.T > 1) w = std::max(w, op_xg_words_for(Mx, hs));
        if (w) add((int64_t)w, 8);
    }
    for (int q = 0; q < 25; ++q) add(Mx, 8);
    add(ld, 8), add((int64_t)vk::kMaxRhs * ld, 8), add((int64_t)vk::kMaxRhs * ld, 8), add(ld, 8);
    add(2 * ld, 8);
    if (probit) {
        for (int q = 0; q < 3; ++q) add(ld, 8);
        for (int q = 0; q < 3; ++q) add(Mx, 8);
    }
    (void)writer;
    *bytes = total;
    return VAMPOMI_OK;
}

static std::string op_name(const vampomi_ctx* c, int K) {
    vk::OpPlan p{};
    int cus = c->cus;
    if (cus <= 0 && hipDeviceGetAttribute(&cus, hipDeviceAttributeMultiprocessorCount, c->device) != hipSuccess) cus = 256;
    if (!vk::op_plan(c->N, std::max<int64_t>(c->M, 1), cus, c->op_variant, &p)) return "(no one-pass plan)";
    if (K == 1 + vk::kOpPlain) {
        vk::OpPlan h{};
        if (!vk::team_plain_plan(c->N, std::max<int64_t>(c->M, 1), cus, p, &h)) return "(no head-start plan)";
        return vk::team_kernel_name(K, h);
    }
    return vk::op_kernel_name(K, p);
}

extern "C" vampomi_status vampomi_dev_read_ceiling(vampomi_ctx* c, int reps, double* us_med, double* bytes,
                                                   int* variant) {
    if (!c || reps < 1 || !us_med) return fail(VAMPOMI_ERR_ARG, "bad argument");
    if (!c->have_X) return fail(VAMPOMI_ERR_STATE, "no methylation data loaded");
    HIPCHK(hipSetDevice(c->device));
    if (c->cus <= 0) HIPCHK(hipDeviceGetAttribute(&c->cus, hipDeviceAttributeMultiprocessorCount, c->device));
    STCHK(sync_stream(c, c->st));
    const int64_t n = std::max<int64_t>(c->M, 1) * c->ld;
    hipEvent_t a, b;
    HIPCHK(hipEventCreate(&a));
    HIPCHK(hipEventCreate(&b));
    double best = -1.0, best_bytes = 0.0;
    int best_kind = -1;
    for (int kind = 0; kind < 2; ++kind) {
        double nb = 0.0;
        if (vk::stream_read(c->X, n, kind, c->cus, c->st, vk::Timing{}, c->red_part, &nb) != hipSuccess) {
            (void)hipGetLastError();
            continue;
        }
        std::vector<float> ms((size_t)reps);
        for (int r = 0; r < reps; ++r) {
            HIPCHK(vk::stream_read(c->X, n, kind, c->cus, c->st, vk::Timing{a, b}, c->red_part, &nb));
            HIPCHK(hipEventSynchronize(b));
            HIPCHK(hipEventElapsedTime(&ms[(size_t)r], a, b));
        }
        std::sort(ms.begin(), ms.end());
        const double med = 1e3 * (double)ms[(size_t)reps / 2];
        if (best < 0.0 || nb / med > best_bytes / best) {
            best = med;
            best_bytes = nb;
            best_kind = kind;
        }
    }
    (void)hipEventDestroy(a);
    (void)hipEventDestroy(b);
    if (best_kind < 0) return fail(VAMPOMI_ERR_ARG, "the matrix is too small for a read-ceiling stream");
    *us_med = best;
    if (bytes) *bytes = best_bytes;
    if (variant) *variant = best_kind;
    return VAMPOMI_OK;
}

extern "C" vampomi_status vampomi_dev_kernel_name(const vampomi_ctx* c, int which, int K, int mode, char* out,
                                                  int cap) {
    if (!c || !out || cap < 1) return fail(VAMPOMI_ERR_ARG, "bad argument");
    const std::string n = which == 2   ? vk::loo_kernel_name(c->loo_variant)
                          : which == 3 ? op_name(c, K)
                          : which == 0 ? vk::ax_kernel_name(K, mode == 1, c->axp)
                                       : vk::kernel_name(1, K, mode, c->atx_variant);
    std::snprintf(out, (size_t)cap, "%s", n.c_str());
    return VAMPOMI_OK;
}
```

vampomi_amd/csrc/kdev.h:

```cpp
#pragma once
#include <hip/hip_runtime.h>

#include <cstdint>

#include "kernels.h"

namespace vk {

typedef double v2d __attribute__((ext_vector_type(2)));

__device__ __forceinline__ double wave_sum(double v) {
#pragma unroll
    for (int o = 32; o > 0; o >>= 1) v += __shfl_xor(v, o, 64);
    return v;
}

__device__ __forceinline__ void red_put(const RedOut& ro, int64_t idx, double v) {
    __hip_atomic_store(ro.part + idx, v, __ATOMIC_RELAXED, __HIP_MEMORY_SCOPE_AGENT);
}

template <int K>
__device__ __forceinline__ void ticket_sum_blocks(const RedOut& ro) {
    const int lane = threadIdx.x & 63;
    asm volatile("s_waitcnt vmcnt(0)" ::: "memory");
    unsigned old = 0;
    if (lane == 0) old = __hip_atomic_fetch_add(ro.ticket, 1u, __ATOMIC_RELAXED, __HIP_MEMORY_SCOPE_AGENT);
    old = __shfl(old, 0, 64);
    if (old != gridDim.x - 1) return;
    const int nblk = (int)gridDim.x;
#pragma unroll
    for (int k = 0; k < K; ++k) {
        double t = 0.0;
        for (int b = lane; b < nblk; b += 64)
            t += __hip_atomic_load(ro.part + (int64_t)b * K + k, __ATOMIC_RELAXED, __HIP_MEMORY_SCOPE_AGENT);
        t = wave_sum(t);
        if (lane == 0) ro.out[k] = t;
    }
    if (lane == 0) __hip_atomic_store(ro.ticket, 0u, __ATOMIC_RELAXED, __HIP_MEMORY_SCOPE_AGENT);
}

__device__ inline bool cg_decide_into(CgState& s, const double* red, int it, int mask) {
    const bool ran = s.any != 0;
    if (ran) {
        int any = 0;
#pragma unroll
        for (int k = 0; k < kMaxRhs; ++k) {
            if (k >= s.K || !s.active[k]) continue;
            if (!((mask >> k) & 1)) {
                any = 1;
                continue;
            }
            s.iters[k] = it + 1 + s.off[k];
            const double rz_new = red[3 * k], rr = red[3 * k + 1], vmu = red[3 * k + 2];
            if (s.onsager[k]) {
                const double ons = s.gam2 * vmu;
                const double rel = ons != 0 ? fabs((ons - s.prev_ons[k]) / ons) : 1;
                if (rel < 1e-8) {
                    s.active[k] = 0;
                    continue;
                }
                s.prev_ons[k] = ons;
            }
            double bt = 1.0 / s.rz[k];
            bt *= rz_new;
            s.rz[k] = rz_new;
            const double rel_err = sqrt(rr) / sqrt(s.vv[k]);
            if (rel_err < s.tol) {
                s.active[k] = 0;
                continue;
            }
            s.beta[k] = bt;
            if (s.iters[k] >= s.maxit) {
                s.active[k] = 0;
                continue;
            }
            any = 1;
        }
        s.any = any;
    }
    return ran;
}

__device__ inline void cg_publish(const CgState& s, bool ran, int it, CgMirror* mirror, unsigned long long* flag,
                                  unsigned long long seq, int pack) {
    if (pack) {
        if (flag && ran)
            __hip_atomic_store(flag, cg_pack(seq, s.any, s.iters[0], s.iters[1]), __ATOMIC_RELAXED,
                               __HIP_MEMORY_SCOPE_SYSTEM);
        return;
    }
    if (mirror) {
        CgMirror* m = mirror + (it & 1);
        __hip_atomic_store(&m->seq, seq, __ATOMIC_RELAXED, __HIP_MEMORY_SCOPE_SYSTEM);
        __hip_atomic_store(&m->any, s.any, __ATOMIC_RELAXED, __HIP_MEMORY_SCOPE_SYSTEM);
#pragma unroll
        for (int k = 0; k < kMaxRhs; ++k)
            __hip_atomic_store(&m->iters[k], s.iters[k], __ATOMIC_RELAXED, __HIP_MEMORY_SCOPE_SYSTEM);
    }
    if (flag) {
        asm volatile("s_waitcnt vmcnt(0)" ::: "memory");
        __hip_atomic_store(flag, seq, __ATOMIC_RELAXED, __HIP_MEMORY_SCOPE_SYSTEM);
    }
}

__device__ inline void cg_decide_from(CgState s, CgState* cs, const double* red, int it, CgMirror* mirror,
                                      unsigned long long* flag, unsigned long long seq, int mask, int pack = 0) {
    const bool ran = cg_decide_into(s, red, it, mask);
    if (ran) *cs = s;
    cg_publish(s, ran, it, mirror, flag, seq, pack);
}

__device__ inline void cg_decide_body(CgState* cs, const double* red, int it, CgMirror* mirror, unsigned long long* flag,
                                      unsigned long long seq, int mask, int pack = 0) {
    const CgState s = *cs;
    double r[3 * kMaxRhs];
#pragma unroll
    for (int q = 0; q < 3 * kMaxRhs; ++q) r[q] = q < 3 * s.K ? red[q] : 0.0;
    cg_decide_from(s, cs, r, it, mirror, flag, seq, mask, pack);
}

}
```

vampomi_amd/csrc/kernels.h:

```cpp
#pragma once
#include <hip/hip_runtime.h>

#include <atomic>
#include <cstdint>
#include <string>

namespace vk {

constexpr int kMaxRhs = 4;
constexpr int kMaxL = 64;
constexpr int kMaxTerms = 12;
constexpr int kRedBlocks = 1024;

struct CPtrs { const double* p[kMaxRhs]; };
struct Timing { hipEvent_t start = nullptr, stop = nullptr; };
struct RedOut {
    double* part;
    double* out;
    unsigned* ticket;
    unsigned long long* flag = nullptr;
    unsigned long long seq = 0;
    const int* gate = nullptr;
    double* out2 = nullptr;
    int split = 0;
};
struct Ptrs { double* p[kMaxRhs]; };

struct Shard {
    const double* X;
    int64_t ld, N, M;
    const double* mave;
    const double* msig;
};

struct AxPlan {
    int variant;
    int64_t rows;
    int64_t tiles;
    int64_t total;
    int64_t span;
    int64_t nband;
    int64_t sa, sb;
    int groups;
    int nslots;
    int T = 0, TR = 0, S = 0;
};
inline int64_t ax_slots(const AxPlan& p, int64_t t) { return ((t + 1) * p.sa - 1) / p.sb - (t * p.sa) / p.sb + 1; }
constexpr int kAxDefault = -1, kAxTeam = 7, kAxTeamMinT = 8, kAtxDefault = -1 , kLooDefault = 16;
AxPlan ax_plan(int64_t N, int64_t M, int variant = kAxDefault);
AxPlan ax_plan_for(int64_t N, int64_t M, int cus, int variant);
int ax_variant_count();
bool ax_variant_ok(int v);
int atx_variant_count();
bool atx_variant_ok(int v);
struct AxFuse {
    CPtrs z{};
    const double* beta = nullptr;
    const int* gate = nullptr;
};
hipError_t ax_partial(const Shard& s, const AxPlan& pl, int K, CPtrs x, double* part, hipStream_t st,
                      const Timing& tm = Timing{}, const AxFuse& fu = AxFuse{});
hipError_t stream_read(const double* x, int64_t n, int kind, int cus, hipStream_t st, const Timing& tm,
                       double* sink, double* bytes);
bool ax_team_plan(int64_t N, int64_t M, int cus, AxPlan* out);
hipError_t ax_team(const Shard& s, const AxPlan& pl, int K, CPtrs x, double* part, hipStream_t st, const Timing& tm,
                   const AxFuse& fu);
std::string ax_kernel_name(int K, bool fused, const AxPlan& pl);
hipError_t ax_reduce(const AxPlan& pl, int K, int64_t N, int64_t ld, const double* part, Ptrs out,
                     double div, hipStream_t st, const int* gate = nullptr);
hipError_t vec_div(int K, int64_t n, int64_t ld, Ptrs v, double div, hipStream_t st, const Ptrs* dst = nullptr);

int atx_blocks(int64_t M, int K, int variant);
std::string kernel_name(int which, int K, int mode, int variant);
hipError_t atx(const Shard& s, int K, CPtrs u, Ptrs out, double scale, int mode, double tau,
               double gam2, CPtrs p, hipStream_t st, int variant = kAtxDefault, const Timing& tm = Timing{},
               const int* gate = nullptr, CPtrs zf = CPtrs{}, const double* beta = nullptr, Ptrs sraw = Ptrs{});

constexpr int kOpMaxK = 2;
constexpr int kOpPlain = 3;
struct OpPlan {
    int grid;
    int S;
    int64_t nslots;
    int T = 0;
    int TR = 0;
    int cfg = 0;
};
constexpr int kOpDefault = -1;
bool op_plan(int64_t N, int64_t M, int cus, int variant, OpPlan* out);
bool op_supported(int64_t N, int K);
bool team_plan(int64_t N, int64_t M, int cus, int T, int cfg, OpPlan* out);
bool team_lds_layout(const OpPlan& pl, int64_t N, int K, int64_t out[6]);
hipError_t lds_allow(const void* kern, std::atomic<unsigned long long>& done, int bytes);
struct CgState;
struct CgMirror;
struct OpFold {
    const CgState* src = nullptr;
    CgState* dst = nullptr;
    const double* red = nullptr;
    int on = 0, it = 0, mask = 0xf, pack = 0;
    CgMirror* mirror = nullptr;
    unsigned long long* flag = nullptr;
    unsigned long long seq = 0;
};
struct OpArgs {
    CPtrs ar, qo;
    CPtrs p, z;
    const double* beta;
    int fuse;
    double diag, scale, tau, gam2;
    Ptrs d, sraw;
    CPtrs px;
    double* part;
    RedOut ro;
    unsigned long long* xg;
    unsigned tag;
    unsigned* err;
    unsigned long long* ts;
    int dbg;
    OpFold fold;
};
std::string op_kernel_name(int K, const OpPlan& pl);
std::string team_kernel_name(int K, const OpPlan& pl);
int team_occupancy(const OpPlan& pl, int K);
hipError_t atax(const Shard& s, const OpPlan& pl, int K, const OpArgs& a, hipStream_t st, const Timing& tm = Timing{},
                const int* gate = nullptr);
hipError_t atax_team(const Shard& s, const OpPlan& pl, int K, const OpArgs& a, hipStream_t st, const Timing& tm,
                     const int* gate);
hipError_t atax_team_plain(const Shard& s, const OpPlan& pl, const OpArgs& a, hipStream_t st, const Timing& tm,
                           const int* gate);
bool team_plain_plan(int64_t N, int64_t M, int cus, const OpPlan& main, OpPlan* out);
hipError_t op_reduce(const OpPlan& pl, int K, int64_t N, int64_t ld, const double* part, Ptrs out, double div,
                     hipStream_t st, const int* gate = nullptr, int k0 = 0);

hipError_t marker_stats(const double* X, int64_t ld, int64_t N, int64_t M, double nonas,
                        double alpha_scale, double* mave, double* msig, hipStream_t st);

hipError_t gen_markers(uint64_t seed, int kind, int64_t N, int64_t ld, int64_t S, int64_t M, double* X,
                       hipStream_t st);
hipError_t gen_beta(uint64_t seed, double lam, int64_t S, int64_t M, double* beta, const RedOut& ro, hipStream_t st);
hipError_t scale_vec(int64_t n, double* v, double a, hipStream_t st);
hipError_t add_noise(uint64_t seed, int64_t N, double sd, double* y, hipStream_t st);

enum DotOp { DOT = 0, DIFF2 = 1, SUM = 2, PUPD = 3, SQPUPD = 4 };
struct DotTerm {
    const double* a;
    const double* b;
    int op;
    const double* c = nullptr;
    const double* beta = nullptr;
};
struct G1Chain {
    int term = 0;
    double gam2 = 0.0, rho = 0.0, gam1_prev = 0.0;
    double* out = nullptr;
};
struct DotCopy {
    int n = 0;
    int term[2] = {0, 0};
    double* dst[2] = {nullptr, nullptr};
};
struct DotArgs {
    DotTerm t[kMaxTerms];
    int nt;
    G1Chain g1;
    DotCopy copy;
};
int red_blocks(int64_t n);
hipError_t dots(const DotArgs& a, int64_t n, const RedOut& ro, hipStream_t st);
hipError_t dots2(const DotArgs& a, int64_t na, const RedOut& roa, const DotArgs& b, int64_t nb, const RedOut& rob,
                 hipStream_t st);

struct Mix {
    double probs[kMaxL];
    double vars[kMaxL];
    int L;
};
constexpr int kMixWords = 2 + 2 * kMaxL;
struct PreOut;
hipError_t denoise(int64_t M, const double* r1, double gam1, const Mix& mix, double* x1,
                   const double* x1_prev, int damp, double rho, double* x1d, const RedOut& ro, hipStream_t st,
                   const double* mixw = nullptr, const double* gam1dev = nullptr, const PreOut* po = nullptr);

struct EmUpd {
    int64_t Mt = 0;
    int learn_vars = 0;
    double merge_vars_thr = 0.0;
    double* out = nullptr;
    double* mirror = nullptr;
};
struct EmArgs {
    double omegas[kMaxL];
    double vars[kMaxL];
    double v[kMaxL];
    double lambda, noise_var, gam1, max_sigma;
    int L;
    const double* lx;
    const double* ly;
    double la, lb, lc;
    double* r1out;
    const double* dsc;
    EmUpd upd;
};
hipError_t em_sums(int64_t M, const double* r1, const EmArgs& a, const RedOut& ro, hipStream_t st);
// ... 9 lines not shown
    const double* tc = nullptr;
    double Mt = 0.0, N = 0.0;
    double* out = nullptr;
    double* mirror = nullptr;
};
struct TailPost {
    int mode = 0;
    const double* src = nullptr;
    G1Chain g1;
    const double* cp_src[2] = {nullptr, nullptr};
    double* cp_dst[2] = {nullptr, nullptr};
    int L = 0;
    double vars[kMaxL] = {};
    EmUpd upd;
    PreOut po;
    const double* gam1dev = nullptr;
};
hipError_t tail_post(const TailPost& t, hipStream_t st);
struct PreDev {
    const double* scal = nullptr;
};
struct Prelude {
    double eta1, gam1, gam2, gamw;
    PreDev dev;
    const double* x1;
    const double* r1;
    const double* atxy;
    double* r2;
    double* v;
    uint64_t seed;
    int it;
    int64_t S;
    double sqrtMt;
    double* bern;
    double* bern_next;
    double* zero[2];
};
hipError_t prelude(int64_t M, const Prelude& p, hipStream_t st);
hipError_t div_scalar(int64_t n, const double* x, double d, double* out, hipStream_t st);
hipError_t div2_scalar(int64_t n, const double* x, const double* r, double d, double* out, hipStream_t st);

hipError_t probit_denoise(int64_t N, const double* p1, const double* y, double tau1, double* z1, const RedOut& ro,
                          hipStream_t st);
hipError_t probit_confusion(int64_t N, int nz, const double* z, int64_t ld, const double* y, const RedOut& ro,
                            hipStream_t st);
hipError_t probit_p1(uint64_t seed, int64_t N, double* p1, hipStream_t st);

hipError_t loo_sums(const Shard& s, const double* ymod, const double* x1, double sqrtN, double* stats,
                    hipStream_t st, int variant = kLooDefault, const Timing& tm = Timing{});
std::string loo_kernel_name(int variant);
int loo_variant_count();
bool loo_variant_ok(int v);
hipError_t loo_pvals(int64_t M, const double* stats, int n, double* pvals, hipStream_t st);
hipError_t se_pvals(int64_t M, const double* r1, double gam1, int64_t N, double* pvals, hipStream_t st);
hipError_t set_scalar(double* p, double v, hipStream_t st);
hipError_t mul_scalar(int64_t n, const double* x, double a, double* out, hipStream_t st);

hipError_t signal_host(unsigned long long* flag, unsigned long long seq, hipStream_t st);
hipError_t post_flag(unsigned long long* flag, unsigned long long seq, hipStream_t st);
hipError_t publish_host(const double* a, int na, double* ha, const double* b, int nb, double* hb,
                        unsigned long long* flag, unsigned long long seq, hipStream_t st);

struct CgVecs {
    double* mu[kMaxRhs];
    double* r[kMaxRhs];
    double* z[kMaxRhs];
    double* p[kMaxRhs];
    const double* d[kMaxRhs];
    const double* v[kMaxRhs];
    const double* atx0[kMaxRhs];
    double tau, gam2;
    double* W[kMaxRhs];
    const double* S[kMaxRhs];
    double* AW[kMaxRhs];
    const double* AS[kMaxRhs];
    int64_t nA;
    double* Q[kMaxRhs];
    double* AR[kMaxRhs];
    const double* AD[kMaxRhs];
    const double* adpart;
    int64_t adld;
    int adslots;
    double addiv;
};
hipError_t cg_init(int K, int64_t M, const CgVecs& c, double diag, const RedOut& ro, hipStream_t st);
struct CgState {
    double rz[kMaxRhs], vv[kMaxRhs], prev_ons[kMaxRhs], beta[kMaxRhs];
    double gam2, tol;
    int active[kMaxRhs], iters[kMaxRhs], onsager[kMaxRhs], off[kMaxRhs];
    int K, any, maxit;
};
constexpr int kCgPackMaxIter = (1 << 15) - 2;
__host__ __device__ inline unsigned long long cg_pack(unsigned long long seq, int any, int it0, int it1) {
    return (seq << 32) | ((unsigned long long)(any ? 1 : 0) << 30) | ((unsigned long long)(it1 & 0x7fff) << 15) |
           (unsigned long long)(it0 & 0x7fff);
}
struct CgMirror {
    unsigned long long seq;
    int any;
    int iters[kMaxRhs];
};
constexpr int kCgMirrorSlots = 2;
hipError_t cg_start(const CgState& init, CgState* dst, hipStream_t st);
hipError_t cg_start_from(const CgState& init, const double* sums, CgState* dst, hipStream_t st,
                         const double* gam2dev = nullptr);
hipError_t prelude_cg_init(int K, int64_t M, const Prelude& p, const CgVecs& c, double diag, const RedOut& ro,
                           const CgState* start, CgState* dst, hipStream_t st);
struct CgDecide {
    int on = 0, it = 0;
    int pack = 0;
    int mask = 0xf;
    CgMirror* mirror = nullptr;
    unsigned long long* flag = nullptr;
    unsigned long long seq = 0;
};
hipError_t cg_update(int K, int64_t M, const CgVecs& c, double diag, CgState* cs, const double* dp_dev,
                     const double* pp_dev, int fuse, const RedOut& ro, const CgDecide& dc, hipStream_t st);
hipError_t cg_decide(CgState* cs, const double* red, int it, CgMirror* mirror, unsigned long long* flag,
                     unsigned long long seq, hipStream_t st, int mask = 0xf, int pack = 0);

}
```

vampomi_amd/csrc/kernels.hip:

```cpp
#include "kernels.h"
#include "kdev.h"

#include <algorithm>
#include <cstdlib>

#include <hip/hip_ext.h>

#include <hip/hip_runtime.h>

#include <cstdio>
#include <mutex>
#include <string>

namespace vk {

static constexpr int kBlock = 256;

__device__ __forceinline__ double block_sum(double v, double* lds4) {
    v = wave_sum(v);
    const int lane = threadIdx.x & 63, w = threadIdx.x >> 6;
    __syncthreads();
    if (lane == 0) lds4[w] = v;
    __syncthreads();
    return ((lds4[0] + lds4[1]) + lds4[2]) + lds4[3];
// ... 1716 lines not shown
    }
    block_put_sums<2 * kMaxRhs>(acc, 2 * K, ro, (int64_t)blockIdx.x * 2 * K);
    if (red_finish(ro, 2 * K, lds, fin) && dst && threadIdx.x == 0) {
        *dst = start;
        dst->gam2 = cgam2;
        for (int k = 0; k < K; ++k) {
            dst->rz[k] = fin[2 * k];
            dst->vv[k] = fin[2 * k + 1];
        }
    }
}

hipError_t prelude_cg_init(int K, int64_t M, const Prelude& p, const CgVecs& c, double diag, const RedOut& ro,
                           const CgState* start, CgState* dst, hipStream_t st) {
    hipLaunchKernelGGL(prelude_cg_init_kernel, dim3(red_blocks(M)), dim3(kBlock), 0, st, K, M, p, c, diag, ro,
                       start ? *start : CgState{}, start ? dst : nullptr);
    return hipGetLastError();
}

hipError_t cg_init(int K, int64_t M, const CgVecs& c, double diag, const RedOut& ro, hipStream_t st) {
    hipLaunchKernelGGL(cg_init_kernel, dim3(red_blocks(M)), dim3(kBlock), 0, st, K, M, c, diag, ro);
    return hipGetLastError();
}

__global__ void cg_start_kernel(CgState init, CgState* dst) {
    if (threadIdx.x == 0) *dst = init;
}

hipError_t cg_start(const CgState& init, CgState* dst, hipStream_t st) {
    hipLaunchKernelGGL(cg_start_kernel, dim3(1), dim3(64), 0, st, init, dst);
    return hipGetLastError();
}

__global__ void cg_start_from_kernel(CgState init, const double* __restrict__ sums, CgState* dst,
                                     const double* __restrict__ gam2dev) {
    if (threadIdx.x != 0) return;
    for (int k = 0; k < init.K; ++k) {
        init.rz[k] = sums[2 * k];
        init.vv[k] = sums[2 * k + 1];
    }
    if (gam2dev) init.gam2 = gam2dev[0];
    *dst = init;
}

hipError_t cg_start_from(const CgState& init, const double* sums, CgState* dst, hipStream_t st,
                         const double* gam2dev) {
    hipLaunchKernelGGL(cg_start_from_kernel, dim3(1), dim3(64), 0, st, init, sums, dst, gam2dev);
    return hipGetLastError();
}

__global__ void cg_decide_kernel(CgState* cs, const double* __restrict__ red, int it, CgMirror* mirror,
                                 unsigned long long* flag, unsigned long long seq, int mask, int pack) {
    if (threadIdx.x == 0) cg_decide_body(cs, red, it, mirror, flag, seq, mask, pack);
}

#ifndef CGU_ABL
#define CGU_ABL 0
#endif
template <int K, int W>
__global__ __launch_bounds__(kBlock) void cg_update_kernel(int64_t M, CgVecs c, double diag,
                                                           CgState* cs, const double* __restrict__ dp_dev,
                                                           const double* __restrict__ pp_dev, int fuse, RedOut ro,
                                                           CgDecide dc, int mblocks) {
#if CGU_ABL & 32
    CgState st{};
    st.K = K;
    st.any = 1;
    for (int k = 0; k < K; ++k) {
        st.active[k] = 1;
        st.rz[k] = st.vv[k] = 1.0;
    }
    double dpv[K], ppv[K];
    for (int k = 0; k < K; ++k) dpv[k] = 1.0, ppv[k] = 0.0;
#else
    const CgState st = *cs;
    double dpv[K], ppv[K];
#pragma unroll
    for (int k = 0; k < K; ++k) {
        dpv[k] = dp_dev[k];
        ppv[k] = pp_dev ? pp_dev[k] : 0.0;
    }
#endif
    if (!st.any) return;
    __shared__ double fin[3 * kMaxRhs];
    const bool mpart = (int)blockIdx.x < mblocks;
    double alpha[K];
    bool on[K];
#pragma unroll
    for (int k = 0; k < K; ++k) {
        on[k] = st.active[k] && ((dc.mask >> k) & 1);
        const double dp = pp_dev ? c.tau * dpv[k] + c.gam2 * ppv[k] : dpv[k];
        alpha[k] = on[k] ? st.rz[k] / dp : 0.0;
    }
    double acc[3 * K];
#pragma unroll
    for (int q = 0; q < 3 * K; ++q) acc[q] = 0.0;
    double beta[K];
    bool fk[K];
#pragma unroll
    for (int k = 0; k < K; ++k) {
        fk[k] = on[k] && ((fuse >> k) & 1);
        beta[k] = fk[k] ? st.beta[k] : 0.0;
    }
    const int64_t mstride = (int64_t)mblocks * kBlock;
    constexpr int H = W >= 32 || K >= 3 ? 2 : 1;
    for (int64_t i0 = (int64_t)blockIdx.x * kBlock + threadIdx.x; mpart && !(CGU_ABL & 2) && i0 < M;
         i0 += H * mstride) {
        double pv[H][K], zv[H][K], muv[H][K], rv[H][K], dv[H][K], vv[H][K], wv[H][K], sv[H][K];
        const bool two = H == 2 && i0 + mstride < M;
#pragma unroll
        for (int h = 0; h < H; ++h) {
            const int64_t i = i0 + h * mstride;
            if (h == 1 && !two) break;
#pragma unroll
            for (int k = 0; k < K; ++k) {
                if (on[k]) {
                    pv[h][k] = c.p[k][i];
                    zv[h][k] = fk[k] ? c.z[k][i] : 0.0;
                    muv[h][k] = c.mu[k][i];
                    rv[h][k] = c.r[k][i];
                    dv[h][k] = c.d[k][i];
                    vv[h][k] = c.v[k][i];
                    wv[h][k] = c.W[k] ? c.W[k][i] : 0.0;
                    sv[h][k] = c.W[k] ? c.S[k][i] : 0.0;
                }
            }
        }
#pragma unroll
        for (int h = 0; h < H; ++h) {
            const int64_t i = i0 + h * mstride;
            if (h == 1 && !two) break;
#pragma unroll
            for (int k = 0; k < K; ++k) {
                if (on[k]) {
                    double pi = pv[h][k];
                    if (fk[k]) {
                        pi = zv[h][k] + beta[k] * pi;
                        c.p[k][i] = pi;
                    }
                    const double mu = muv[h][k] + alpha[k] * pi;
                    const double r = rv[h][k] - dv[h][k] * alpha[k];
                    const double z = r / diag;
                    c.mu[k][i] = mu;
                    c.r[k][i] = r;
                    c.z[k][i] = z;
                    if (c.W[k]) c.W[k][i] = wv[h][k] + alpha[k] * sv[h][k];
                    acc[3 * k] += r * z;
                    acc[3 * k + 1] += r * r;
                    acc[3 * k + 2] += vv[h][k] * mu;
                }
            }
        }
    }
    if (c.adpart) {
        __shared__ v2d wsum[4][64];
        const int lane = threadIdx.x & 63, w = threadIdx.x >> 6, ns = c.adslots;
        const int nb = (int)gridDim.x - mblocks;
        const int64_t tpk = (c.nA + 127) / 128;
        for (int64_t tile = (int)blockIdx.x - mblocks; !(CGU_ABL & 1) && !mpart && tile < K * tpk; tile += nb) {
            const int k = (int)(tile / tpk);
            const int64_t i = (tile - k * tpk) * 128 + 2 * lane;
            const bool ok = i < c.nA;
            bool onk = false, fuk = false;
            double alk = 0.0, bek = 0.0;
#pragma unroll
            for (int kk = 0; kk < (K < kOpMaxK ? K : kOpMaxK); ++kk)
                if (kk == k) {
                    onk = on[kk];
                    fuk = fk[kk];
                    alk = alpha[kk];
                    bek = beta[kk];
                }
            const bool upd = w == 0 && ok && onk;
            v2d arv{0.0, 0.0}, qov{0.0, 0.0}, awv{0.0, 0.0};
            if (upd) {
                arv = *reinterpret_cast<const v2d*>(c.AR[k] + i);
                if (fuk) qov = *reinterpret_cast<const v2d*>(c.Q[k] + i);
                if (c.AW[k]) awv = *reinterpret_cast<const v2d*>(c.AW[k] + i);
            }
            wsum[w][lane] = ok ? slot_sum<W>(c.adpart + (int64_t)k * c.adld + i, (int64_t)kMaxRhs * c.adld,
                                             w * ns / 4, (w + 1) * ns / 4)
                               : v2d{0.0, 0.0};
            __syncthreads();
            if (upd) {
                const v2d ad = (((wsum[0][lane] + wsum[1][lane]) + wsum[2][lane]) + wsum[3][lane]) / c.addiv;
#pragma unroll
                for (int e = 0; e < 2; ++e) {
                    const int64_t j = i + e;
                    if (j >= c.nA) break;
                    double q = arv[e] / diag;
                    if (fuk) q = q + bek * qov[e];
                    c.Q[k][j] = q;
                    if (c.AW[k]) c.AW[k][j] = awv[e] + alk * q;
                    c.AR[k][j] = arv[e] - ad[e] * alk;
                }
            }
            __syncthreads();
        }
    } else if (c.Q[0]) {
        for (int64_t i = (int64_t)blockIdx.x * kBlock + threadIdx.x; i < c.nA; i += (int64_t)gridDim.x * kBlock) {
            double ar[K], qo[K], ad[K], aw[K];
#pragma unroll
            for (int k = 0; k < K; ++k)
                if (on[k]) {
                    ar[k] = c.AR[k][i];
                    qo[k] = fk[k] ? c.Q[k][i] : 0.0;
                    ad[k] = c.addiv > 0 ? c.AD[k][i] / c.addiv : c.AD[k][i];
                    aw[k] = c.AW[k] ? c.AW[k][i] : 0.0;
                }
#pragma unroll
            for (int k = 0; k < K; ++k)
                if (on[k]) {
                    double q = ar[k] / diag;
                    if (fk[k]) q = q + beta[k] * qo[k];
                    c.Q[k][i] = q;
                    if (c.AW[k]) c.AW[k][i] = aw[k] + alpha[k] * q;
                    c.AR[k][i] = ar[k] - ad[k] * alpha[k];
                }
        }
    } else
    for (int64_t i = (int64_t)blockIdx.x * kBlock + threadIdx.x; i < c.nA; i += (int64_t)gridDim.x * kBlock) {
        double aw[K], as[K];
#pragma unroll
        for (int k = 0; k < K; ++k)
            if (on[k] && c.AW[k]) {
                aw[k] = c.AW[k][i];
                as[k] = c.AS[k][i];
            }
#pragma unroll
        for (int k = 0; k < K; ++k)
            if (on[k] && c.AW[k]) c.AW[k][i] = aw[k] + alpha[k] * as[k];
    }
    bool last = false;
    if (CGU_ABL & 16) {
    } else if (mpart) {
        block_put_sums<3 * K>(acc, 3 * K, ro, (int64_t)blockIdx.x * 3 * K);
        last = red_ticket(ro, (int)gridDim.x);
    } else {
        last = red_ticket_nowait(ro, (int)gridDim.x);
    }
    if (last && !(CGU_ABL & 8)) red_final(ro, 3 * K, mblocks, fin, true);
    if (last && dc.on && threadIdx.x == 0 && !(CGU_ABL & 12)) {
        double r[3 * kMaxRhs];
#pragma unroll
        for (int q = 0; q < 3 * kMaxRhs; ++q) r[q] = q < 3 * K ? fin[q] : 0.0;
        cg_decide_from(st, cs, r, dc.it, dc.mirror, dc.flag, dc.seq, dc.mask, dc.pack);
    }
}

constexpr int kCguBlocks = 512;
hipError_t cg_update(int K, int64_t M, const CgVecs& c, double diag, CgState* cs, const double* dp_dev,
                     const double* pp_dev, int fuse, const RedOut& ro, const CgDecide& dc, hipStream_t st) {
    static const int ept = std::getenv("VAMPOMI_CG_EPT") ? std::max(1, std::atoi(std::getenv("VAMPOMI_CG_EPT"))) : 2;
    const int mb = (int)std::min<int64_t>(std::max<int64_t>(cdiv(M, (int64_t)kBlock * ept), 1), kRedBlocks / 2);
    int nb = 0;
    if (c.adpart) {
        if (K > kOpMaxK || c.adslots < 1 || !c.Q[0]) return hipErrorInvalidValue;
        static const int nbset = std::getenv("VAMPOMI_CGU_NB") ? std::atoi(std::getenv("VAMPOMI_CGU_NB")) : 0;
        nb = (int)std::min<int64_t>(K * cdiv(c.nA, 128), nbset > 0 ? nbset : std::max(kCguBlocks - mb, 1));
        nb = std::max(std::min(nb, kRedBlocks - mb), 1);
    }
    const bool wide = c.adpart && c.adslots >= 4 * 32;
#define VAMPOMI_CGU(KK)                                                                                          \
    case KK:                                                                                                     \
        if (wide)                                                                                                \
            hipLaunchKernelGGL((cg_update_kernel<KK, 32>), dim3(mb + nb), dim3(kBlock), 0, st, M, c, diag, cs,   \
                               dp_dev, pp_dev, fuse, ro, dc, mb);                                                \
        else                                                                                                     \
            hipLaunchKernelGGL((cg_update_kernel<KK, 8>), dim3(mb + nb), dim3(kBlock), 0, st, M, c, diag, cs,    \
                               dp_dev, pp_dev, fuse, ro, dc, mb);                                                \
        break;
    switch (K) {
        VAMPOMI_CGU(1)
        VAMPOMI_CGU(2)
        VAMPOMI_CGU(3)
        VAMPOMI_CGU(4)
        default: return hipErrorInvalidValue;
    }
#undef VAMPOMI_CGU
    return hipGetLastError();
}

hipError_t cg_decide(CgState* cs, const double* red, int it, CgMirror* mirror, unsigned long long* flag,
                     unsigned long long seq, hipStream_t st, int mask, int pack) {
    hipLaunchKernelGGL(cg_decide_kernel, dim3(1), dim3(64), 0, st, cs, red, it, mirror, flag, seq, mask, pack);
    return hipGetLastError();
}


__constant__ double kErfcxPoly[24] = {
    0x1.edcad78fc8044p-31,  0x1.b1548f14735d1p-30,  -0x1.a1ad2e6c4a7a8p-27, -0x1.1985b48f08574p-26,
    0x1.c6a8093ac4f83p-24,  0x1.31c2b2b44b731p-24,  -0x1.b87373facb29fp-21, 0x1.3fef1358803b7p-22,
    0x1.7eec072bb0be3p-18,  -0x1.78a680a741c4ap-17, -0x1.9951f39295cf4p-16, 0x1.3be1255ce180bp-13,
    -0x1.a1df71176b791p-13, -0x1.8d4aaa0099bc8p-11, 0x1.49c673066c831p-8,   -0x1.0962386ea02b7p-6,
    0x1.3079edf465cc3p-5,   -0x1.0fb06dfedc4ccp-4,  0x1.7fee004e266dfp-4,   -0x1.9ddb23c3e14d2p-4,
    0x1.16ecefcfa4865p-4,   0x1.f7f5df66fc349p-7,   -0x1.1df1ad154a27fp-3,  0x1.dd2c8b74febf6p-3};

__device__ __forceinline__ double erfcx_ref(double x) {
    if (x < -10.0) return __builtin_inf();
    if (x > 10.0) return -1.7976931348623157e308;
    const double a = fmax(x, 0.0 - x);
    const double inv = 1.0 / (a + 4.0);
    double q = (a - 4.0) * inv;
    const double t0 = __builtin_fma(q + 1.0, -4.0, a);
    q = __builtin_fma(inv, __builtin_fma(q, -a, t0), q);
    double p = kErfcxPoly[0];
#pragma unroll
    for (int k = 1; k < 24; ++k) p = __builtin_fma(p, q, kErfcxPoly[k]);
    const double h = (1.0 / (a + 0.5)) * 0.5;
    const double q1 = __builtin_fma(p, h, h);
    const double res = (p - q1) + __builtin_fma(q1 + q1, -a, 1.0);
    double r = __builtin_fma(res, h, q1);
    if (a > 1.7976931348623157e308) r = 0.0;
    if (x < 0.0) {
        const double s = x * x;
        const double lo = __builtin_fma(x, x, -s);
        const double e = exp_cr(s);
        r = __builtin_fma(e, lo + lo, e - r) + e;
        if (e > 1.7976931348623157e308) r = e;
    }
    return r;
}

__global__ __launch_bounds__(kBlock) void probit_denoise_kernel(int64_t N, const double* __restrict__ p1,
                                                                const double* __restrict__ y, double tau1,
                                                                double* __restrict__ z1, RedOut ro) {
    __shared__ double lds[4];
    const double sq = sqrt(1.0 + 1.0 / tau1);
    const double k0 = 2.0 / sqrt(2 * M_PI), rt2 = sqrt(2.0);
    const double den = 1 + tau1 * 1.0;
    double acc = 0.0;
    for (int64_t i = (int64_t)blockIdx.x * kBlock + threadIdx.x; i < N; i += (int64_t)gridDim.x * kBlock) {
        const double p = p1[i], s = 2 * y[i] - 1;
        const double c = (p + 0.0) / sq;
        const double ratio = k0 / erfcx_ref(-s * c / rt2);
        z1[i] = p + s * ratio / tau1 / sq;
        acc += 1 - ratio / den * (s * c + ratio);
    }
    acc = block_sum(acc, lds);
    if (threadIdx.x == 0) red_put(ro, blockIdx.x, acc);
    red_finish(ro, 1, lds);
}

hipError_t probit_denoise(int64_t N, const double* p1, const double* y, double tau1, double* z1, const RedOut& ro,
                          hipStream_t st) {
    hipLaunchKernelGGL(probit_denoise_kernel, dim3(red_blocks(N)), dim3(kBlock), 0, st, N, p1, y, tau1, z1, ro);
    return hipGetLastError();
}

__global__ __launch_bounds__(kBlock) void confusion_kernel(int64_t N, int nz, const double* __restrict__ z,
                                                           int64_t ld, const double* __restrict__ y,
                                                           RedOut ro) {
    __shared__ double lds[4];
    double cnt[8] = {0, 0, 0, 0, 0, 0, 0, 0};
    for (int64_t i = (int64_t)blockIdx.x * kBlock + threadIdx.x; i < N; i += (int64_t)gridDim.x * kBlock) {
        const double yi = y[i];
        for (int k = 0; k < nz; ++k) {
            const double yh = (0.5 * erfc(-z[k * ld + i] * M_SQRT1_2) >= 0.5) ? 1.0 : 0.0;
            if (yi == 1 && yh == 1)
                cnt[4 * k + 0] += 1;
            else if (yi == 0 && yh == 0)
                cnt[4 * k + 1] += 1;
            else if (yi == 0 && yh == 1)
                cnt[4 * k + 2] += 1;
            else if (yi == 1 && yh == 0)
                cnt[4 * k + 3] += 1;
        }
    }
// ... 366 lines not shown
```

vampomi_amd/csrc/pcg.cpp:

```cpp
#include <algorithm>
#include <cmath>
#include <cstddef>
#include <cstdlib>
#include <string>
#include <utility>

#include "ctx.h"

template <class T>
static T* field(vk::CgState* cs, size_t off) {
    return reinterpret_cast<T*>(reinterpret_cast<char*>(cs) + off);
}

struct CgOutcome {
    int any = 0;
    int iters[vk::kMaxRhs] = {};
};

static constexpr int kCgPackWord = 2;

template <class Enqueue, class Settle>
static vampomi_status cg_loop(vampomi_ctx* c, int max_iter, bool packed, Enqueue&& enqueue, CgOutcome* last,
                              Settle&& settle) {
    unsigned long long prev = 0, cur = 0;
    STCHK(enqueue(0, &prev));
    for (int i = 1;; ++i) {
        const size_t mark = c->pending.size();
        const vampomi_stats before = c->stats;
        if (i < max_iter)
            STCHK(enqueue(i, &cur));
        else
            STCHK(settle());
        c->stats.host_syncs++;
        CgOutcome o;
        if (packed) {
            const int word = kCgPackWord + ((i - 1) & 1);
            STCHK(wait_flag(c, prev << 32, word));
            STCHK(op_check_err(c));
            const unsigned long long w = __atomic_load_n(c->h_flag + word, __ATOMIC_ACQUIRE);
            if ((w >> 32) != (prev & 0xffffffffULL))
                return fail(VAMPOMI_ERR_STATE, "CG step " + std::to_string(i - 1) + ": decision word holds sequence " +
                                                   std::to_string(w >> 32) + ", expected " + std::to_string(prev));
            o.any = (int)((w >> 30) & 1);
            o.iters[0] = (int)(w & 0x7fff);
            o.iters[1] = (int)((w >> 15) & 0x7fff);
        } else {
            STCHK(wait_flag(c, prev));
            STCHK(op_check_err(c));
            const vk::CgMirror* m = c->h_cgm + ((i - 1) & 1);
            if (__atomic_load_n(&m->seq, __ATOMIC_ACQUIRE) != prev)
                return fail(VAMPOMI_ERR_STATE, "CG step " + std::to_string(i - 1) + ": decision slot holds sequence " +
                                                   std::to_string(m->seq) + ", expected " + std::to_string(prev));
            o.any = m->any;
            for (int k = 0; k < vk::kMaxRhs; ++k) o.iters[k] = m->iters[k];
        }
        *last = o;
        if (!o.any || i >= max_iter) {
            if (i < max_iter) drop_launches(c, mark, before);
            break;
        }
        prev = cur;
    }
    return VAMPOMI_OK;
}

vampomi_status pcg_run(vampomi_ctx* c, const std::vector<CgSystem*>& sys, double tau, double gam2, int max_iter,
                       double tol, double* nscratch, int64_t* ref_passes, DotBatch* init, const double* extra_x,
                       double* ex_out, bool onepass, const double* const* ar0, HeadStart* hs, const vk::Prelude* pre,
                       PreMode pm) {
    const int64_t M = c->M, N = c->N;
    const double diag = tau * (double)(N - 1) / (double)N + gam2;
    const int K = (int)sys.size();
    if (K < 1 || K > vk::kMaxRhs) return fail(VAMPOMI_ERR_ARG, "pcg: 1..4 systems");
    if (extra_x && (!ex_out || K + 1 >= vk::kMaxRhs)) return fail(VAMPOMI_ERR_ARG, "pcg: extra A.x needs K <= 2");
    if (hs) {
        hs->used = false;
        if (!onepass || K != 2 || !extra_x || ar0 || sys[0]->mu0_nonzero || (hs->xnext && !hs->axnext))
            return fail(VAMPOMI_ERR_ARG, "pcg: the head start needs the one-pass form, two systems, extra_x, "
                                         "system 0 from zero and no ar0");
    }
    const double* xnext = hs ? hs->xnext : nullptr;
    auto extra_alone = [&]() -> vampomi_status {
        const double* px[2];
        double* out[2];
        int n = 0;
        if (extra_x) px[n] = extra_x, out[n++] = ex_out;
        if (xnext) px[n] = xnext, out[n++] = hs->axnext;
        if (n == 0) return VAMPOMI_OK;
        STCHK(ax_dev(c, n, px, nscratch));
        for (int j = 0; j < n; ++j)
            HIPCHK(hipMemcpyAsync(out[j], nscratch + (int64_t)j * c->ld, (size_t)N * 8, hipMemcpyDeviceToDevice,
                                  c->st));
        return VAMPOMI_OK;
    };
    {
        std::vector<CgSystem*> nz;
        for (auto* s : sys) {
            if (s->mu0_nonzero && !s->atx0) nz.push_back(s);
            if (s->mu0_nonzero && ref_passes) *ref_passes += 2;
        }
        if (!nz.empty()) {
            if (pm != PreMode::normal) return fail(VAMPOMI_ERR_ARG, "pcg: a start queued ahead needs no lmmse pass");
            const double* vv[vk::kMaxRhs];
            double* dd[vk::kMaxRhs];
            for (size_t k = 0; k < nz.size(); ++k) {
                vv[k] = nz[k]->mu;
                dd[k] = nz[k]->d;
            }
            STCHK(lmmse_dev(c, (int)nz.size(), vv, dd, tau, gam2, nscratch));
        }
    }
    if (onepass && K <= vk::kOpMaxK && c->have_X) STCHK(op_prepare(c));
    const bool op1 = onepass && K <= vk::kOpMaxK && c->have_X && c->op_ok;
    vk::CgVecs cv{};
    cv.tau = tau;
    cv.gam2 = gam2;
    for (int k = 0; k < K; ++k) {
        CgSystem* s = sys[k];
        cv.mu[k] = s->mu;
        cv.r[k] = s->r;
        cv.z[k] = s->z;
        cv.p[k] = s->p;
        cv.v[k] = s->v;
        cv.atx0[k] = s->mu0_nonzero ? s->atx0 : nullptr;
        cv.d[k] = (s->mu0_nonzero && !s->atx0) ? s->d : nullptr;
    }
    const bool head = hs && hs->abern && c->hs_ok && c->op_ok && max_iter > 0;
    vk::CgState s0{};
    s0.K = K;
    s0.gam2 = gam2;
    s0.tol = tol;
    s0.maxit = max_iter;
    s0.off[0] = head ? 1 : 0;
    s0.any = max_iter > 0 ? 1 : 0;
    for (int k = 0; k < K; ++k) {
        s0.active[k] = 1;
        s0.onsager[k] = sys[k]->onsager ? 1 : 0;
        sys[k]->iters = 0;
    }
    if (pre && init) return fail(VAMPOMI_ERR_ARG, "pcg: the prelude rides only in the device-side start");
    if (pm != PreMode::normal && !pre) return fail(VAMPOMI_ERR_ARG, "pcg: a start queued ahead is the prelude's");
    if (init) {
        std::vector<double> rzvv(2 * K);
        vk::RedOut ro{};
        STCHK(init->sink(2 * K, true, rzvv.data(), &ro));
        HIPCHK(vk::cg_init(K, M, cv, diag, ro, c->st));
        STCHK(init->flush());
        for (int k = 0; k < K; ++k) {
            s0.rz[k] = rzvv[2 * k];
            s0.vv[k] = rzvv[2 * k + 1];
        }
        if (max_iter <= 0) return extra_alone();
        HIPCHK(vk::cg_start(s0, c->cgs, c->st));
    } else {
        const vk::RedOut ro{c->red_part, c->scal + SL_CGI, c->ticket, nullptr, 0, nullptr};
        const bool own_start = pre && !c->use_comm;
        if (pm != PreMode::normal && (!pre || (pm == PreMode::ahead) != (pre->dev.scal != nullptr)))
            return fail(VAMPOMI_ERR_ARG, "pcg: a start queued ahead needs the prelude and its device scalars");
        if (pm == PreMode::queued) {
        } else {
            if (pre)
                HIPCHK(vk::prelude_cg_init(K, M, *pre, cv, diag, ro, own_start ? &s0 : nullptr, c->cgs, c->st));
            else
                HIPCHK(vk::cg_init(K, M, cv, diag, ro, c->st));
            if (!own_start) {
                STCHK(allreduce_dev(c, c->scal + SL_CGI, (size_t)(2 * K)));
                if (max_iter > 0)
                    HIPCHK(vk::cg_start_from(s0, c->scal + SL_CGI, c->cgs, c->st,
                                             pm == PreMode::ahead ? pre->dev.scal + 1 : nullptr));
            }
            if (pm == PreMode::ahead) return VAMPOMI_OK;
        }
        if (max_iter <= 0) return extra_alone();
    }
    const int* gate = field<int>(c->cgs, offsetof(vk::CgState, any));
    const double* beta = field<double>(c->cgs, offsetof(vk::CgState, beta));
    if (op1) {
        const bool fold = c->use_comm && c->cg_fold && c->opp.T >= 1 && (!head || c->opp_hs.T >= 1);
        int cur = 0;
        struct Pending {
            bool on = false;
            int it = 0, mask = 0xf, pack = 0;
            vk::CgMirror* mirror = nullptr;
            unsigned long long* flag = nullptr;
            unsigned long long seq = 0;
        } pend;
        auto state = [&](int s) { return c->cgs + s; };
        double* AR = c->op_nvec;
        double* Q = c->op_nvec + (int64_t)vk::kMaxRhs * c->ld;
        const double* AD = c->op_nvec + (int64_t)2 * vk::kMaxRhs * c->ld;
        bool given = false;
        for (int k = 0; k < K; ++k) given = given || (ar0 && ar0[k]);
        if (head) {
        } else if (!given) {
            const double* px[vk::kMaxRhs];
            for (int k = 0; k < K; ++k) px[k] = sys[k]->r;
            int n = K;
            if (extra_x) px[n++] = extra_x;
            if (xnext) px[n++] = xnext;
            STCHK(ax_dev(c, n, px, AR));
            if (extra_x)
                HIPCHK(hipMemcpyAsync(ex_out, AR + (int64_t)K * c->ld, (size_t)N * 8, hipMemcpyDeviceToDevice, c->st));
            if (xnext)
                HIPCHK(hipMemcpyAsync(hs->axnext, AR + (int64_t)(n - 1) * c->ld, (size_t)N * 8,
                                      hipMemcpyDeviceToDevice, c->st));
        } else {
            const double* px[vk::kMaxRhs];
            int slot[vk::kMaxRhs], n = 0;
            for (int k = 0; k < K; ++k) {
                if (ar0[k]) {
                    if (sys[k]->mu0_nonzero) return fail(VAMPOMI_ERR_ARG, "pcg: A r0 given for a nonzero start");
                    HIPCHK(hipMemcpyAsync(AR + (int64_t)k * c->ld, ar0[k], (size_t)N * 8, hipMemcpyDeviceToDevice,
                                          c->st));
                } else {
                    slot[n] = k;
                    px[n++] = sys[k]->r;
                }
            }
            if (extra_x) {
                slot[n] = K;
                px[n++] = extra_x;
            }
            if (n > 0) {
                STCHK(ax_dev(c, n, px, nscratch));
                for (int j = 0; j < n; ++j) {
                    double* dst = slot[j] < K ? AR + (int64_t)slot[j] * c->ld : ex_out;
                    HIPCHK(hipMemcpyAsync(dst, nscratch + (int64_t)j * c->ld, (size_t)N * 8, hipMemcpyDeviceToDevice,
                                          c->st));
                }
            }
        }
        vk::CgVecs cu{};
        cu.tau = tau;
        cu.gam2 = gam2;
        cu.nA = N;
        for (int k = 0; k < K; ++k) {
            cu.mu[k] = sys[k]->mu;
            cu.r[k] = sys[k]->r;
            cu.z[k] = sys[k]->z;
            cu.p[k] = sys[k]->p;
            cu.d[k] = sys[k]->d;
            cu.v[k] = sys[k]->v;
            cu.W[k] = sys[k]->W;
            cu.S[k] = sys[k]->W ? sys[k]->S : nullptr;
            cu.AW[k] = sys[k]->AW;
            cu.Q[k] = Q + (int64_t)k * c->ld;
            cu.AR[k] = head && k == 0 ? hs->abern : AR + (int64_t)k * c->ld;
            cu.AD[k] = AD + (int64_t)k * c->ld;
        }
        if (!c->use_comm) {
            cu.adpart = c->op_part;
            cu.adld = c->ld;
            cu.adslots = c->opp.nslots;
        }
        cu.addiv = c->sqrtN;
        bool rec = false;
        for (int k = 0; k < K; ++k) rec = rec || sys[k]->W;
        if (rec)
            for (int k = 0; k < K; ++k)
                if (!sys[k]->S) return fail(VAMPOMI_ERR_ARG, "pcg: W needs an S scratch vector for every system");
        const int all = (1 << K) - 1;
        if (head) {
            vk::OpArgs a{};
            a.ar.p[0] = cu.AR[0];
            a.qo.p[0] = cu.Q[0];
            a.p.p[0] = sys[0]->p;
            a.z.p[0] = sys[0]->z;
            a.d.p[0] = sys[0]->d;
            a.sraw.p[0] = rec ? sys[0]->S : nullptr;
            a.beta = beta;
            a.fuse = 0;
            a.diag = diag;
            a.tau = tau;
            a.gam2 = gam2;
            const double* px[vk::kOpPlain] = {sys[1]->r, extra_x, xnext ? xnext : extra_x};
            double* out[vk::kOpPlain] = {cu.AR[1], ex_out, xnext ? hs->axnext : nscratch};
            STCHK(op_dev_plain(c, a, px, out, gate));
            vk::CgVecs ch = cu;
            if (!c->use_comm) ch.adslots = (int)c->opp_hs.nslots;
            else ch.addiv = 0.0;
            const double* dp = c->use_comm ? AD + (int64_t)(1 + vk::kOpPlain) * c->ld : c->scal + SL_DP;
            const vk::RedOut ro{c->red_part, c->scal + SL_CG, c->ticket, nullptr, 0, gate};
            vk::CgDecide dc{};
            dc.on = !c->use_comm;
            dc.it = -1;
            dc.mask = 1;
            HIPCHK(vk::cg_update(1, M, ch, diag, c->cgs, dp, nullptr, 0, ro, dc, c->st));
            if (c->use_comm) {
                STCHK(allreduce_dev(c, c->scal + SL_CG, 3));
                if (fold) {
                    pend.on = true;
                    pend.it = -1;
                    pend.mask = 1;
                } else {
                    HIPCHK(vk::cg_decide(c->cgs, c->scal + SL_CG, -1, nullptr, nullptr, 0, c->st, 1));
                }
            }
            hs->used = true;
        }
        const bool packed = K <= 2 && max_iter < vk::kCgPackMaxIter;
        auto enqueue = [&](int i, unsigned long long* seq) -> vampomi_status {
            const int fuse = i > 0 ? all : head ? 1 : 0;
            vk::OpArgs a{};
            for (int k = 0; k < K; ++k) {
                a.ar.p[k] = cu.AR[k];
                a.qo.p[k] = cu.Q[k];
                a.p.p[k] = sys[k]->p;
                a.z.p[k] = sys[k]->z;
                a.d.p[k] = sys[k]->d;
                a.sraw.p[k] = rec ? sys[k]->S : nullptr;
            }
            a.beta = fold ? nullptr : beta;
            a.fuse = fuse;
            a.diag = diag;
            a.tau = tau;
            a.gam2 = gam2;
            const int* g = gate;
            vk::CgState* cs = c->cgs;
            if (fold) {
                if (pend.on) {
                    a.fold.on = 1;
                    a.fold.src = state(cur);
                    a.fold.dst = state(cur ^ 1);
                    a.fold.red = c->scal + SL_CG;
                    a.fold.it = pend.it;
                    a.fold.mask = pend.mask;
                    a.fold.pack = pend.pack;
                    a.fold.mirror = pend.mirror;
                    a.fold.flag = pend.flag;
                    a.fold.seq = pend.seq;
                    cur ^= 1;
                    pend.on = false;
                }
                cs = state(cur);
                g = field<int>(cs, offsetof(vk::CgState, any));
                if (!a.fold.on) a.beta = field<double>(cs, offsetof(vk::CgState, beta));
            }
            STCHK(op_dev(c, K, a, g, c->use_comm, false));
            const double* dp = c->use_comm ? AD + (int64_t)K * c->ld : c->scal + SL_DP;
            const vk::RedOut ro{c->red_part, c->scal + SL_CG, c->ticket, nullptr, 0, g};
            *seq = ++c->sync_seq;
            unsigned long long* flag = packed ? c->d_flag + kCgPackWord + (i & 1) : c->d_flag;
            vk::CgMirror* mirror = packed ? nullptr : c->d_cgm;
            vk::CgDecide dc{};
            if (!c->use_comm) {
                dc.on = 1;
                dc.it = i;
                dc.mirror = mirror;
                dc.flag = flag;
                dc.seq = *seq;
                dc.pack = packed ? 1 : 0;
            }
            HIPCHK(vk::cg_update(K, M, cu, diag, cs, dp, nullptr, fuse, ro, dc, c->st));
            if (c->use_comm) {
                STCHK(allreduce_dev(c, c->scal + SL_CG, (size_t)(3 * K)));
                if (fold) {
                    pend.on = true;
                    pend.it = i;
                    pend.mask = 0xf;
                    pend.pack = packed ? 1 : 0;
                    pend.mirror = mirror;
                    pend.flag = flag;
                    pend.seq = *seq;
                } else {
                    HIPCHK(vk::cg_decide(c->cgs, c->scal + SL_CG, i, mirror, flag, *seq, c->st, 0xf, packed ? 1 : 0));
                }
            }
            return VAMPOMI_OK;
        };
        auto settle = [&]() -> vampomi_status {
            if (!pend.on) return VAMPOMI_OK;
            HIPCHK(vk::cg_decide(state(cur), c->scal + SL_CG, pend.it, pend.mirror, pend.flag, pend.seq, c->st,
                                 pend.mask, pend.pack));
            pend.on = false;
            return VAMPOMI_OK;
        };
        CgOutcome last;
        STCHK(cg_loop(c, max_iter, packed, enqueue, &last, settle));
        STCHK(op_check_err(c));
        for (int k = 0; k < K; ++k) {
            sys[k]->iters = last.iters[k];
            if (ref_passes) *ref_passes += 2 * (int64_t)sys[k]->iters;
        }
        return VAMPOMI_OK;
    }
    if (xnext) {
        STCHK(ax_dev(c, 1, &xnext, nscratch));
        HIPCHK(hipMemcpyAsync(hs->axnext, nscratch, (size_t)N * 8, hipMemcpyDeviceToDevice, c->st));
    }
    const double* pp[vk::kMaxRhs];
    const double* zz[vk::kMaxRhs];
    double* dd[vk::kMaxRhs];
    double* ss[vk::kMaxRhs];
    bool recur = false;
    for (int k = 0; k < K; ++k) {
        pp[k] = sys[k]->p;
        zz[k] = sys[k]->z;
        dd[k] = sys[k]->d;
        ss[k] = sys[k]->S;
        recur = recur || sys[k]->W;
    }
    if (recur)
        for (int k = 0; k < K; ++k)
            if (!ss[k]) return fail(VAMPOMI_ERR_ARG, "pcg: W needs an S scratch vector for every system");
    static const bool dp_separate = std::getenv("VAMPOMI_DP_SEPARATE") && std::atoi(std::getenv("VAMPOMI_DP_SEPARATE"));
    const bool split_dp = c->use_comm && K < vk::kMaxRhs && !dp_separate;
    vk::CgVecs cu{};
    cu.tau = tau;
    cu.gam2 = gam2;
    for (int k = 0; k < K; ++k) {
        cu.mu[k] = sys[k]->mu;
        cu.r[k] = sys[k]->r;
        cu.z[k] = sys[k]->z;
        cu.p[k] = sys[k]->p;
        cu.d[k] = sys[k]->d;
        cu.v[k] = sys[k]->v;
        cu.W[k] = sys[k]->W;
        cu.S[k] = sys[k]->W ? sys[k]->S : nullptr;
        cu.AW[k] = sys[k]->AW;
        cu.AS[k] = nscratch + (int64_t)k * c->ld;
        if (sys[k]->AW) cu.nA = N;
    }
    auto enqueue = [&](int i, unsigned long long* seq) -> vampomi_status {
        const bool fuse = i > 0;
        vk::AxFuse fu{};
        fu.gate = gate;
        if (fuse) {
            for (int k = 0; k < K; ++k) fu.z.p[k] = zz[k];
            fu.beta = beta;
        }
        const double* u[vk::kMaxRhs];
        for (int k = 0; k < K; ++k) u[k] = nscratch + (int64_t)k * c->ld;
        const double* px[vk::kMaxRhs];
        for (int k = 0; k < K; ++k) px[k] = pp[k];
        const bool ex = i == 0 && extra_x;
        if (ex) px[K] = extra_x;
        const int KA = ex ? K + 1 : K;
        const double* pp_dev = nullptr;
        if (split_dp) {
            vk::DotArgs tail{};
            tail.nt = K;
            for (int k = 0; k < K; ++k)
                tail.t[k] = fuse ? vk::DotTerm{pp[k], pp[k], vk::SQPUPD, zz[k], beta + k}
                                 : vk::DotTerm{pp[k], pp[k], vk::DOT};
            STCHK(ax_dev(c, KA, px, nscratch, &fu, &tail));
            if (ex) HIPCHK(hipMemcpyAsync(ex_out, nscratch + (int64_t)K * c->ld, (size_t)N * 8, hipMemcpyDeviceToDevice, c->st));
            pp_dev = nscratch + (int64_t)KA * c->ld;
            vk::DotArgs uu{};
            uu.nt = K;
            for (int k = 0; k < K; ++k) uu.t[k] = vk::DotTerm{u[k], u[k], vk::DOT};
            HIPCHK(vk::dots(uu, c->N, vk::RedOut{c->red_part, c->scal + SL_DP, c->ticket, nullptr, 0, gate}, c->st));
            STCHK(atx_dev(c, K, u, dd, 1, tau, gam2, pp, gate, fuse ? zz : nullptr, beta, false, recur ? ss : nullptr));
        } else {
            STCHK(ax_dev(c, KA, px, nscratch, &fu));
            if (ex) HIPCHK(hipMemcpyAsync(ex_out, nscratch + (int64_t)K * c->ld, (size_t)N * 8, hipMemcpyDeviceToDevice, c->st));
            STCHK(atx_dev(c, K, u, dd, 1, tau, gam2, pp, gate, fuse ? zz : nullptr, beta, true, recur ? ss : nullptr));
        }
        const vk::RedOut ro{c->red_part, c->scal + SL_CG, c->ticket, nullptr, 0, gate};
        *seq = ++c->sync_seq;
        vk::CgDecide dc{};
        if (!c->use_comm) {
            dc.on = 1;
            dc.it = i;
            dc.mirror = c->d_cgm;
            dc.flag = c->d_flag;
            dc.seq = *seq;
// ... 18 lines not shown
```

vampomi_amd/csrc/run.h:

```cpp
#pragma once
#include <string>
#include <vector>

#include "ctx.h"
#include "writer.h"

struct Mixture {
    int L = 0;
    double probs[VAMPOMI_MAX_L] = {};
    double vars[VAMPOMI_MAX_L] = {};
};

inline double smax(double a, double b) { return (a < b) ? b : a; }
inline double smin(double a, double b) { return (b < a) ? b : a; }

struct VampRun {
    vampomi_params prm{};
    vampomi_result* res = nullptr;
    bool probit = false;
    bool write = false;
    bool fuse = true;
    bool recur = false;
    bool arec = false;
    bool onepass = false;
    int z1n_slot = 2;
    int bern_it = 0;
    int abern_it = 0;
    int em_head = 0, z_head = 0;
    double zh_bsum = 0, zh_cnt[4] = {}, zh_xc[3] = {};
    int hs_it = 0;
    std::string out_dir, out_name, p_params, p_metrics, p_prior;
    int it = 0;
    bool stopped = false;
    bool io_err = false;
    std::string io_msg;
    IterWriter* writer = nullptr;
    Mixture mix, mix_next;
    bool have_next = false;
    double gam1 = 0, gam2 = 0, gamw = 0;
    double alpha1 = 0, alpha2 = 0, eta1 = 0, eta2 = 0, alpha1_next = 0;
    double metrics[12] = {}, params[8] = {};
    double e1m[3] = {}, e1n[2] = {}, e1s[3] = {}, e2m[3] = {}, e2n[2] = {}, e2s[3] = {};
    double tn = 0, tc = 0, nm[2] = {}, sum_d = 0, a2 = 0;
    double *r1 = nullptr, *x1 = nullptr, *x1p = nullptr, *x1n = nullptr, *x1d = nullptr, *r2 = nullptr;
    double *x2 = nullptr, *bern = nullptr, *invQ = nullptr, *v = nullptr, *atxy = nullptr, *ts = nullptr;
    double *tmpM = nullptr, *atx0 = nullptr;
    double* cgw[10] = {};
    double *z1buf = nullptr, *nb3 = nullptr , *nsc = nullptr;
    double* ax2 = nullptr;
    double* abern = nullptr;
    double* bern_next = nullptr;
    double* mixw = nullptr;
    double* mixh = nullptr;
    double* mixh_dev = nullptr;
    bool mix_pending = false;
    Mixture mix_expect;
    int pre_ahead = 0;
    bool pre_ahead_on = true;
    const double* z1 = nullptr;
    int64_t passes_ref = 0;
    double tau1 = 0, tau2 = 0, beta1 = 0, beta2 = 0;
    double* p1 = nullptr;
    double* p2 = nullptr;
    double* z1h = nullptr;
    double* x1s = nullptr;
    double* x1sn = nullptr;
    double* x2s = nullptr;
    double* prior_row = nullptr;
    double ph_solve_s = 0, ph_step_s = 0;

    ~VampRun();
};

struct EmParams {
    int EM_max_iter;
    double EM_err_thr;
    int learn_vars;
    double merge_vars_thr;
    int verbosity;
};
EmParams em_params(const VampRun& R);
vampomi_status update_prior(vampomi_ctx* c, const EmParams& P, Mixture& m, double gam1, const double* r1);
vampomi_status update_prior(vampomi_ctx* c, const VampRun& R, Mixture& m, double gam1, const double* r1);
struct EmState {
    int emit = 0;
    double lambda = 0;
    double omegas[VAMPOMI_MAX_L] = {};
    double sums[2 * VAMPOMI_MAX_L] = {};
};
struct R1From {
    const double* x2;
    const double* r2;
    double eta2, gam2, gam1;
    const double* dsc = nullptr;
};
vampomi_status em_begin(vampomi_ctx* c, const EmParams& P, const Mixture& m, double gam1, const double* r1,
                        DotBatch& b, EmState& s, const R1From* r1from = nullptr, const vk::EmUpd* upd = nullptr);
vampomi_status em_queue(vampomi_ctx* c, const Mixture& m, double gam1, const double* r1, DotBatch& b, EmState& s,
                        const R1From* r1from = nullptr, const vk::EmUpd* upd = nullptr);
vampomi_status em_finish(vampomi_ctx* c, const EmParams& P, Mixture& m, double gam1, const double* r1, EmState& s);
vampomi_status denoise_into(vampomi_ctx* c, const Mixture& m, double gam1, const double* r1, double* x1,
                            const double* x1_prev, bool damp, double rho, double* x1d, DotBatch& b, double* sum_out,
                            const double* mixw = nullptr, const double* gam1dev = nullptr,
                            const vk::PreOut* po = nullptr);
vampomi_status upload_or_zero(vampomi_ctx* c, double* dst, const double* host, int64_t n);
vampomi_status write_bins(vampomi_ctx* c, VampRun& R);
void write_row(VampRun& R, const std::string& path, int it, const double* vals, int n);
vampomi_status agree_io(vampomi_ctx* c, VampRun& R, bool wait_all = false);
vampomi_status end_iteration_io(vampomi_ctx* c, VampRun& R);
vampomi_status probit_begin(vampomi_ctx* c, VampRun& R);
vampomi_status probit_step(vampomi_ctx* c, VampRun& R);
```

vampomi_amd/csrc/vamp.cpp:

```cpp
#include <algorithm>
#include <chrono>
#include <cmath>
#include <cstdio>
#include <cstring>

#include "ctx.h"
#include "hostio.h"
#include "run.h"

VampRun::~VampRun() {
    if (writer) writer->drain(nullptr);
    for (double** p : {&r1, &x1, &x1p, &x1n, &x1d, &r2, &x2, &bern, &invQ, &v, &atxy, &ts, &tmpM, &atx0, &z1buf,
                       &nb3, &nsc, &ax2, &p1, &p2, &z1h, &x1s, &x1sn, &x2s, &abern, &bern_next})
        dev_free(*p);
    for (auto& p : cgw) dev_free(p);
    dev_free(mixw);
    if (mixh) (void)hipHostFree(mixh);
}

vampomi_ctx::vampomi_ctx() = default;

vampomi_ctx::~vampomi_ctx() {
    run.reset();
    writer.reset();
    release_ctx_resources(this);
}

vampomi_status em_begin(vampomi_ctx* c, const EmParams& P, const Mixture& m, double gam1, const double* r1,
                        DotBatch& b, EmState& s, const R1From* r1from, const vk::EmUpd* upd) {
    s.emit = 0;
    s.lambda = 1 - m.probs[0];
    for (int j = 0; j < m.L; ++j) s.omegas[j] = m.probs[j];
    for (int j = 1; j < m.L; ++j) s.omegas[j] /= s.lambda;
    if (P.EM_max_iter < 1) return VAMPOMI_OK;
    return em_queue(c, m, gam1, r1, b, s, r1from, upd);
}

vampomi_status em_queue(vampomi_ctx* c, const Mixture& m, double gam1, const double* r1, DotBatch& b,
                        EmState& s, const R1From* r1from, const vk::EmUpd* upd) {
    const int L = m.L;
    double max_sigma = m.vars[0];
    for (int j = 1; j < L; ++j) max_sigma = smax(max_sigma, m.vars[j]);
    vk::EmArgs a{};
    for (int j = 0; j < L; ++j) {
        a.omegas[j] = s.omegas[j];
        a.vars[j] = m.vars[j];
    }
    for (int j = 1; j < L; ++j) a.v[j - 1] = 1.0 / (1.0 / m.vars[j] + gam1);
    a.lambda = s.lambda;
    a.noise_var = 1 / gam1;
    a.gam1 = gam1;
    a.max_sigma = max_sigma;
    a.L = L;
    if (r1from) {
        a.lx = r1from->x2;
        a.ly = r1from->r2;
        a.la = r1from->eta2;
        a.lb = r1from->gam2;
        a.lc = r1from->gam1;
        a.r1out = const_cast<double*>(r1);
        a.dsc = r1from->dsc;
    }
    if (upd) a.upd = *upd;
    vk::RedOut ro{};
    STCHK(b.sink(1 + 2 * (L - 1), true, s.sums, &ro));
    HIPCHK(vk::em_sums(c->M, r1, a, ro, b.stream()));
    return VAMPOMI_OK;
}

vampomi_status em_finish(vampomi_ctx* c, const EmParams& P, Mixture& m, double gam1, const double* r1,
                         EmState& s) {
    for (; s.emit < P.EM_max_iter; ++s.emit) {
        if (s.emit > 0) {
            DotBatch b(c);
            STCHK(em_queue(c, m, gam1, r1, b, s));
            STCHK(b.flush());
        }
        const int L = m.L;
        double probs_prev[VAMPOMI_MAX_L], vars_prev[VAMPOMI_MAX_L];
        std::memcpy(probs_prev, m.probs, sizeof probs_prev);
        std::memcpy(vars_prev, m.vars, sizeof vars_prev);
        const double lambda_total = s.sums[0];
        s.lambda = lambda_total / (double)c->Mt;
        const double sum_of_pin = lambda_total;
        for (int j = 0; j < L - 1; ++j) {
            const double res_total = s.sums[1 + j];
            const double res_gammas_total = s.sums[L + j];
            if (P.learn_vars == 1) m.vars[j + 1] = res_gammas_total / res_total;
            s.omegas[j + 1] = res_total / sum_of_pin;
            m.probs[j + 1] = s.lambda * s.omegas[j + 1];
        }
        m.probs[0] = 1 - s.lambda;
        double dprob = 0, nprob = 0, dvar = 0, nvar = 0;
        for (int j = 0; j < L; ++j) {
            dprob += (m.probs[j] - probs_prev[j]) * (m.probs[j] - probs_prev[j]);
            nprob += m.probs[j] * m.probs[j];
// ... 30 lines not shown
    STCHK(b.flush());
    return em_finish(c, P, m, gam1, r1, s);
}

EmParams em_params(const VampRun& R) {
    return EmParams{R.prm.EM_max_iter, R.prm.EM_err_thr, R.prm.learn_vars, R.prm.merge_vars_thr, R.prm.verbosity};
}

vampomi_status update_prior(vampomi_ctx* c, const VampRun& R, Mixture& m, double gam1, const double* r1) {
    return update_prior(c, em_params(R), m, gam1, r1);
}

vampomi_status denoise_into(vampomi_ctx* c, const Mixture& m, double gam1, const double* r1, double* x1,
                                   const double* x1_prev, bool damp, double rho, double* x1d, DotBatch& b,
                                   double* sum_out, const double* mixw, const double* gam1dev,
                                   const vk::PreOut* po) {
    vk::Mix mix{};
    mix.L = m.L;
    for (int j = 0; j < m.L; ++j) {
        mix.probs[j] = m.probs[j];
        mix.vars[j] = m.vars[j];
    }
    vk::RedOut ro{};
    STCHK(b.sink(1, true, sum_out, &ro));
    HIPCHK(vk::denoise(c->M, r1, gam1, mix, x1, x1_prev, damp ? 1 : 0, rho, x1d, ro, b.stream(), mixw, gam1dev, po));
    return VAMPOMI_OK;
}

static void err_groups(vampomi_ctx* c, VampRun& R, const double* xhat, const double* Axest, double* m3, double* n2,
                       double* s3, std::vector<DotBatch::Group>& gm, std::vector<DotBatch::Group>& gn) {
    gm.push_back({{T(xhat, R.ts), T(xhat, xhat), T(R.ts, R.ts)}, true, m3});
    gn.push_back({{T(c->y, Axest, vk::DIFF2), T(c->y, c->y)}, false, n2});
    gn.push_back({{T(Axest, c->y), T(Axest, Axest), T(c->y, c->y)}, true, s3});
}

static vampomi_status err_queue(vampomi_ctx* c, VampRun& R, const double* xhat, const double* Axest, DotBatch& b,
                                double* m3, double* n2, double* s3, std::vector<DotBatch::Group> gm = {},
                                std::vector<DotBatch::Group> gn = {}) {
    err_groups(c, R, xhat, Axest, m3, n2, s3, gm, gn);
    STCHK(b.add_many(c->M, gm));
    return b.add_many(c->N, gn);
}

static void err_finish(VampRun& R, const double* m3, const double* n2, const double* s3, int ind) {
    const double corr = m3[0] / std::sqrt(m3[1] * m3[2]);
    const double l2_pred_err = std::sqrt(n2[0] / n2[1]);
    const double R2 = 1 - l2_pred_err * l2_pred_err;
    const double corr_y = s3[0] / std::sqrt(s3[1] * s3[2]);
    const double corr_y_2 = corr_y * corr_y;
    if (ind == 1) {
        R.metrics[1] = corr;
        R.metrics[0] = R2;
        R.metrics[4] = corr_y_2;
    } else {
        R.metrics[3] = corr;
        R.metrics[2] = R2;
        R.metrics[5] = corr_y_2;
    }
}

vampomi_status upload_or_zero(vampomi_ctx* c, double* dst, const double* host, int64_t n) {
    if (n <= 0) return VAMPOMI_OK;
    if (host)
        HIPCHK(hipMemcpyAsync(dst, host, (size_t)n * 8, hipMemcpyHostToDevice, c->st));
    else
        HIPCHK(hipMemsetAsync(dst, 0, (size_t)n * 8, c->st));
    return VAMPOMI_OK;
}

static bool keeps_hist(const VampRun& R) { return R.res && (R.res->x1_hist || R.res->r1_hist); }
vampomi_status ensure_writer(vampomi_ctx* c, VampRun& R);

static vampomi_status vamp_alloc(vampomi_ctx* c, VampRun& R) {
    const size_t M = (size_t)std::max<int64_t>(c->M, 1), ld = (size_t)c->ld;
    for (double** p : {&R.r1, &R.x1, &R.x1p, &R.x1n, &R.x1d, &R.r2, &R.x2, &R.bern, &R.invQ, &R.v, &R.atxy, &R.ts,
                       &R.tmpM, &R.atx0, &R.bern_next})
        STCHK(dev_alloc(p, M));
    for (auto& p : R.cgw) STCHK(dev_alloc(&p, M));
    STCHK(dev_alloc(&R.z1buf, ld));
    STCHK(dev_alloc(&R.nb3, vk::kMaxRhs * ld));
    STCHK(dev_alloc(&R.nsc, vk::kMaxRhs * ld));
    STCHK(dev_alloc(&R.ax2, ld));
    STCHK(dev_alloc(&R.abern, 2 * ld));
    STCHK(dev_alloc(&R.mixw, vk::kMixWords));
    HIPCHK(hipHostMalloc((void**)&R.mixh, (vk::kMixWords + 4) * sizeof(double),
                         hipHostMallocMapped | hipHostMallocCoherent));
    {
        const char* e = std::getenv("VAMPOMI_PRE_AHEAD");
        R.pre_ahead_on = !e || std::atoi(e) != 0;
    }
    HIPCHK(hipHostGetDevicePointer((void**)&R.mixh_dev, R.mixh, 0));
    HIPCHK(hipMemsetAsync(R.ax2, 0, ld * 8, c->st));
    HIPCHK(hipMemsetAsync(R.abern, 0, 2 * ld * 8, c->st));
    HIPCHK(hipMemsetAsync(R.z1buf, 0, ld * 8, c->st));
    HIPCHK(hipMemsetAsync(R.nb3, 0, vk::kMaxRhs * ld * 8, c->st));
    HIPCHK(hipMemsetAsync(R.nsc, 0, vk::kMaxRhs * ld * 8, c->st));
    return VAMPOMI_OK;
}

extern "C" vampomi_status vampomi_vamp_begin(vampomi_ctx* c, const vampomi_params* p, vampomi_result* r) {
    CollScope cs_(c);
    if (!c || !p) return fail(VAMPOMI_ERR_ARG, "null argument");
    if (!c->have_X || !c->have_y) return fail(VAMPOMI_ERR_STATE, "load methylation data and phenotype first");
    const bool probit = p->model && std::strcmp(p->model, "bin_class") == 0;
    if (p->model && !probit && std::strcmp(p->model, "linear") != 0)
        return fail(VAMPOMI_ERR_MODEL, std::string("Invalid model specification! ('") + p->model + "')");
    if (p->L < 1 || p->L > VAMPOMI_MAX_L) return fail(VAMPOMI_ERR_ARG, "number of mixture components out of range");
    HIPCHK(hipSetDevice(c->device));
    STCHK(op_agree(c));
    c->run.reset(new VampRun());
    VampRun& R = *c->run;
    R.prm = *p;
    R.res = r;
    R.probit = probit;
    R.fuse = p->batch_rhs != 0;
    R.recur = p->batch_rhs >= 2;
    R.arec = p->batch_rhs >= 3;
    R.onepass = p->batch_rhs >= 4;
    R.out_dir = p->out_dir ? p->out_dir : "";
    R.out_name = p->out_name ? p->out_name : "";
    R.write = !R.out_dir.empty();
    R.mix.L = p->L;
    for (int j = 0; j < p->L; ++j) {
        R.mix.probs[j] = p->probs[j];
        R.mix.vars[j] = p->vars[j] * (double)c->N;
    }
    R.gam1 = p->gam1;
    R.gamw = 1.0 / (1.0 - p->h2);
    R.gam2 = 0;
    STCHK(vamp_alloc(c, R));
    if (R.write || keeps_hist(R)) STCHK(ensure_writer(c, R));
    STCHK(upload_or_zero(c, R.ts, p->true_signal, c->M));
    std::vector<double> h((size_t)std::max<int64_t>(c->M, 1), 0.0);
    for (int64_t i = 0; i < c->M; ++i) h[i] = (p->x1hat_init ? p->x1hat_init[i] : 0.0) / std::sqrt((double)c->N);
    STCHK(upload_or_zero(c, R.x1, h.data(), c->M));
    STCHK(upload_or_zero(c, R.r1, h.data(), c->M));
    STCHK(upload_or_zero(c, R.x2, nullptr, c->M));
    if (R.probit) {
        if (r) {
            r->iterations_run = 0;
            r->a_passes_ref = 0;
            r->a_passes_exec = 0;
        }
        STCHK(probit_begin(c, R));
        STCHK(sync_stream(c, c->st));
        return VAMPOMI_OK;
    }
    {
        const double* u[1] = {c->y};
        double* o[1] = {R.atxy};
        STCHK(atx_dev(c, 1, u, o, 0, 0.0, 0.0, nullptr));
    }
    if (R.write) {
        R.p_metrics = R.out_dir + "/" + R.out_name + "_metrics.csv";
        R.p_params = R.out_dir + "/" + R.out_name + "_params.csv";
        R.p_prior = R.out_dir + "/" + R.out_name + "_prior.csv";
        if (c->rank == 0) {
            std::vector<std::string> prior_h{"iteration", "number of components"};
            for (int i = 0; i < R.mix.L; ++i) prior_h.push_back("prob" + std::to_string(i));
            for (int i = 0; i < R.mix.L; ++i) prior_h.push_back("var" + std::to_string(i));
            const bool ok =
                vio::csv_create_with_header(R.p_metrics, {"iteration", "R2 denoising", "x1 correlation denoising",
                                                          "R2 LMMSE", "x2 correlation LMMSE", "z1 correlation denoising",
                                                          "z2 correlation LMMSE"}) &&
                vio::csv_create_with_header(R.p_params, {"iteration", "alpha1", "gam1", "alpha2", "gam2", "gamw"}) &&
                vio::csv_create_with_header(R.p_prior, prior_h);
            if (!ok) {
                R.io_err = true;
                R.io_msg = "cannot create output CSV files in " + R.out_dir;
            }
        }
        STCHK(agree_io(c, R));
    }
    if (r) {
        r->iterations_run = 0;
        r->a_passes_ref = 0;
        r->a_passes_exec = 0;
    }
    STCHK(sync_stream(c, c->st));
    return VAMPOMI_OK;
}

vampomi_status ensure_writer(vampomi_ctx* c, VampRun& R) {
    if (R.writer) return VAMPOMI_OK;
    if (!c->writer) return fail(VAMPOMI_ERR_STATE, "context without an iteration writer");
    c->writer->drain(nullptr);
    c->writer->clear_error();
    R.writer = c->writer.get();
    return VAMPOMI_OK;
}

vampomi_status write_bins(vampomi_ctx* c, VampRun& R) {
    const bool hist = keeps_hist(R);
// ... 26 lines not shown
            R.io_msg = msg;
        }
    }
}

vampomi_status agree_io(vampomi_ctx* c, VampRun& R, bool wait_all) {
    if (R.writer && !R.io_err) {
        std::string msg;
        if (wait_all ? R.writer->drain(&msg) : R.writer->failed(&msg)) {
            R.io_err = true;
            R.io_msg = msg;
        }
    }
    double bad = 0.0;
    STCHK(sum_over_ranks(c, R.io_err ? 1.0 : 0.0, &bad));
    if (bad > 0)
        return fail(VAMPOMI_ERR_IO, R.io_err ? R.io_msg
                                             : "output file write failed on " + std::to_string((int)bad) + " other rank(s)");
    return VAMPOMI_OK;
}

vampomi_status end_iteration_io(vampomi_ctx* c, VampRun& R) {
    if (keeps_hist(R) && R.writer) R.writer->drain(nullptr);
    if (R.write) return agree_io(c, R, R.stopped);
    std::string msg;
    if (R.writer && R.writer->failed(&msg)) return fail(VAMPOMI_ERR_HIP, msg);
    return VAMPOMI_OK;
}

static vampomi_status check_device_mix(VampRun& R) {
    if (!R.mix_pending) return VAMPOMI_OK;
    R.mix_pending = false;
    const Mixture& m = R.mix_expect;
    bool same = (double)m.L == R.mixh[0];
    for (int j = 0; same && j < m.L; ++j)
        same = std::memcmp(&m.probs[j], &R.mixh[1 + j], 8) == 0 &&
               std::memcmp(&m.vars[j], &R.mixh[1 + vk::kMaxL + j], 8) == 0;
    if (!same) return fail(VAMPOMI_ERR_STATE, "vamp: the device's EM update differs from the host's");
    return VAMPOMI_OK;
}

struct LmmseSetup {
    CgSystem sx{}, so{};
    bool rec = false, arec = false, hs_av = false, pre_in_cg = false;
    HeadStart hs;
    vk::Prelude pr{};
};

static vampomi_status lmmse_setup(vampomi_ctx* c, VampRun& R, int it, const double* x1, LmmseSetup& L) {
    const int64_t ld = c->ld;
    CgSystem& sx = L.sx;
    CgSystem& so = L.so;
    sx.v = R.v;
    sx.mu = R.x2;
    sx.mu0_nonzero = it > 1;
    sx.atx0 = (it > 1 && R.have_next) ? R.atx0 : nullptr;
    sx.r = R.cgw[0];
    sx.z = R.cgw[1];
    sx.p = R.cgw[2];
    sx.d = R.cgw[3];
    so.v = R.bern;
    so.mu = R.invQ;
    so.onsager = true;
    so.r = R.cgw[4];
    so.z = R.cgw[5];
    so.p = R.cgw[6];
    so.d = R.cgw[7];
    L.rec = R.recur && R.fuse && (it == 1 || sx.atx0);
    if (L.rec) {
        sx.W = R.atx0;
        sx.S = R.cgw[8];
        so.W = R.tmpM;
        so.S = R.cgw[9];
    }
    L.arec = R.arec && L.rec;
    if (L.arec) sx.AW = R.ax2;
    if (R.fuse && L.arec && R.onepass) STCHK(headstart_available(c, &L.hs_av));
    if (L.hs_av) {
        L.hs.abern = R.hs_it == it ? R.abern + (it & 1) * ld : nullptr;
        if (it < R.prm.max_iter) {
            L.hs.xnext = R.bern_next;
            L.hs.axnext = R.abern + ((it + 1) & 1) * ld;
        }
    }
    vk::Prelude& pr = L.pr;
    pr.eta1 = R.eta1;
    pr.gam1 = R.gam1;
    pr.gam2 = R.gam2;
    pr.gamw = R.gamw;
    pr.x1 = x1;
    pr.r1 = R.r1;
    pr.atxy = R.atxy;
    pr.r2 = R.r2;
    pr.v = R.v;
    pr.seed = R.prm.seed;
    pr.it = it;
    pr.S = c->S;
    pr.sqrtMt = std::sqrt((double)c->Mt);
    pr.bern = R.bern;
    pr.bern_next = L.hs.xnext ? R.bern_next : nullptr;
    pr.zero[0] = R.invQ;
    pr.zero[1] = L.rec ? R.tmpM : nullptr;
    L.pre_in_cg = R.fuse && (L.hs_av || L.arec);
    return VAMPOMI_OK;
}

static vampomi_status check_device_values(vampomi_ctx* c, VampRun& R, int it) {
    STCHK(check_device_mix(R));
    if (R.pre_ahead != it) return VAMPOMI_OK;
    R.pre_ahead = 0;
    const double diag = R.gamw * (double)(c->N - 1) / (double)c->N + R.gam2;
    const double want[4] = {R.eta1, R.gam2, R.gamw, diag};
    if (std::memcmp(want, R.mixh + vk::kMixWords, sizeof want) != 0)
        return fail(VAMPOMI_ERR_STATE, "vamp: the prelude queued ahead formed other scalars than the host");
    return VAMPOMI_OK;
}

extern "C" vampomi_status vampomi_vamp_step(vampomi_ctx* c, int* stopped) {
    CollScope cs_(c);
    if (!c || !c->run) return fail(VAMPOMI_ERR_STATE, "vampomi_vamp_begin not called");
    VampRun& R = *c->run;
    if (R.stopped || R.it >= R.prm.max_iter) {
        R.stopped = true;
        if (stopped) *stopped = 1;
        return VAMPOMI_OK;
    }
    HIPCHK(hipSetDevice(c->device));
    const auto t_step = std::chrono::steady_clock::now();
    if (R.probit) {
        STCHK(probit_step(c, R));
        R.ph_step_s = std::chrono::duration<double>(std::chrono::steady_clock::now() - t_step).count();
        if (c->timing) resolve_timing(c);
        if (stopped) *stopped = R.stopped ? 1 : 0;
        return VAMPOMI_OK;
    }
    const int64_t M = c->M, N = c->N, Mt = c->Mt, ld = c->ld;
    const int it = ++R.it;
    vampomi_result* res = R.res;

    if (!R.have_next) {
        if (it > R.prm.learn_prior_delay) STCHK(update_prior(c, R, R.mix, R.gam1, R.r1));
        std::swap(R.x1, R.x1p);
        DotBatch b(c);
        STCHK(denoise_into(c, R.mix, R.gam1, R.r1, R.x1, R.x1p, it > 1, R.prm.rho, R.x1d, b, &R.sum_d));
        STCHK(b.flush());
        R.alpha1 = R.sum_d / (double)Mt;
        if (!R.arec) {
            const double* xs[1] = {R.x1};
            STCHK(ax_dev(c, 1, xs, R.z1buf));
        }
        R.z1 = R.z1buf;
    } else {
        double* old = R.x1p;
        R.x1p = R.x1;
        R.x1 = R.x1n;
        R.x1n = old;
        R.mix = R.mix_next;
        R.alpha1 = R.alpha1_next;
        R.z1 = R.arec ? R.z1buf : R.nb3 + R.z1n_slot * ld;
    }
    R.passes_ref += 1;
    if (res && res->L_hist) res->L_hist[it - 1] = R.mix.L;
    R.eta1 = R.gam1 / R.alpha1;
    STCHK(write_bins(c, R));
    R.gam2 = smin(smax(R.eta1 - R.gam1, 1e-11), 1e11);
    DotBatch e1(c);
    if (!R.arec) STCHK(err_queue(c, R, R.x1, R.z1, e1, R.e1m, R.e1n, R.e1s));
    R.params[0] = R.alpha1;
    R.params[1] = R.gam1;

    R.passes_ref += 1;
    LmmseSetup L;
    STCHK(lmmse_setup(c, R, it, R.x1, L));
    CgSystem& sx = L.sx;
    CgSystem& so = L.so;
    const bool rec = L.rec, arec = L.arec, hs_av = L.hs_av;
    HeadStart& hs = L.hs;
    vk::Prelude& pr = L.pr;
    if (it == 1) {
        HIPCHK(hipMemsetAsync(R.x2, 0, (size_t)std::max<int64_t>(M, 1) * 8, c->st));
        if (rec) HIPCHK(hipMemsetAsync(R.atx0, 0, (size_t)std::max<int64_t>(M, 1) * 8, c->st));
        if (arec) HIPCHK(hipMemsetAsync(R.ax2, 0, (size_t)ld * 8, c->st));
    }
    const PreMode pm = R.pre_ahead == it ? PreMode::queued : PreMode::normal;
    if (pm == PreMode::queued && !(L.pre_in_cg && R.fuse && hs_av))
        return fail(VAMPOMI_ERR_STATE, "vamp: the start queued ahead does not match this iteration's schedule");
    if (!L.pre_in_cg) HIPCHK(vk::prelude(M, pr, c->st));
    const auto t_solve = std::chrono::steady_clock::now();
    if (R.fuse && hs_av) {
        STCHK(pcg_run(c, {&so, &sx}, R.gamw, R.gam2, R.prm.CG_max_iter, R.prm.CG_err_tol, R.nsc, &R.passes_ref,
                      nullptr, R.x1, R.z1buf, true, nullptr, &hs, &pr, pm));
        R.hs_it = hs.xnext ? it + 1 : 0;
    } else if (R.fuse) {
        STCHK(pcg_run(c, {&sx, &so}, R.gamw, R.gam2, R.prm.CG_max_iter, R.prm.CG_err_tol, R.nsc, &R.passes_ref,
                      arec ? nullptr : &e1, arec ? R.x1 : nullptr, arec ? R.z1buf : nullptr, R.onepass, nullptr,
                      nullptr, arec ? &pr : nullptr));
        R.hs_it = 0;
    } else {
        STCHK(pcg_run(c, {&sx}, R.gamw, R.gam2, R.prm.CG_max_iter, R.prm.CG_err_tol, R.nsc, &R.passes_ref, &e1));
        STCHK(pcg_run(c, {&so}, R.gamw, R.gam2, R.prm.CG_max_iter, R.prm.CG_err_tol, R.nsc, &R.passes_ref, nullptr));
    }
    R.ph_solve_s = std::chrono::duration<double>(std::chrono::steady_clock::now() - t_solve).count();
    STCHK(check_device_values(c, R, it));
    if (res && res->cg_iters) res->cg_iters[it - 1] = sx.iters;
    if (res && res->ons_iters) res->ons_iters[it - 1] = so.iters;
    const bool next = R.fuse && it < R.prm.max_iter;
    const bool em_next = next && it + 1 > R.prm.learn_prior_delay;
    const bool r1_in_em = next && arec && em_next && R.prm.EM_max_iter >= 1;
    const bool chain = r1_in_em && (!c->use_comm || c->mr_tail);
    const bool mr = chain && c->use_comm;
    const DotBatch::Group ga2{{T(R.bern, R.invQ)}, true, &R.a2};
    const double gam1_prev = R.gam1;
    auto host_gam1 = [&] {
        R.alpha2 = R.gam2 * R.a2;
        err_finish(R, R.e1m, R.e1n, R.e1s, 1);
        R.eta2 = R.gam2 / R.alpha2;
        R.gam1 = smin(smax(R.eta2 - R.gam2, 1e-11), 1e11);
        R.gam1 = R.prm.rho * R.gam1 + (1 - R.prm.rho) * gam1_prev;
    };
    DotBatch fin(c);
    double* dsc = c->scal + SL_CHAIN;
    const DotBatch::Group gtc{{T(R.bern, R.tmpM)}, true, &R.tc};
    const DotBatch::Group gtn{{T(R.ax2, c->y, vk::DIFF2)}, false, &R.tn};
    const DotBatch::Group gnm{{T(R.x1p, R.x1, vk::DIFF2), T(R.x1p, R.x1p)}, true, R.nm};
    if (chain) {
        std::vector<DotBatch::Group> gm{ga2}, gn;
        err_groups(c, R, R.x1, R.z1, R.e1m, R.e1n, R.e1s, gm, gn);
        gm.push_back(gtc);
        gm.push_back(gnm);
        gn.push_back(gtn);
        err_groups(c, R, R.x2, R.ax2, R.e2m, R.e2n, R.e2s, gm, gn);
        vk::G1Chain g1;
        g1.gam2 = R.gam2;
        g1.rho = R.prm.rho;
        g1.gam1_prev = gam1_prev;
        g1.out = dsc;
        if (!mr) {
            STCHK(fin.add_pair(M, gm, &g1, &R.a2, {{&R.tc, dsc + 9}}, N, gn, {{&R.tn, dsc + 8}}));
        } else {
            STCHK(fin.add_pair(M, gm, nullptr, nullptr, {}, N, gn, {}));
            STCHK(fin.reduce_now());
            vk::TailPost t;
            t.mode = 0;
            t.src = fin.dev_slot(&R.a2);
            t.g1 = g1;
            t.cp_src[0] = fin.dev_slot(&R.tc);
            t.cp_dst[0] = dsc + 9;
            t.cp_src[1] = fin.dev_slot(&R.tn);
            t.cp_dst[1] = dsc + 8;
            HIPCHK(vk::tail_post(t, c->st));
        }
    } else {
        DotBatch b(c);
        if (arec)
            STCHK(err_queue(c, R, R.x1, R.z1, b, R.e1m, R.e1n, R.e1s, {ga2}));
        else
            STCHK(b.add_many(M, {ga2}));
        STCHK(b.flush());
        host_gam1();
        if (!r1_in_em) HIPCHK(vk::lincomb_div(M, R.eta2, R.x2, R.gam2, R.r2, R.gam1, R.r1, c->st));
    }
    R1From r1from{R.x2, R.r2, R.eta2, R.gam2, R.gam1};
    if (chain) r1from.dsc = dsc;
    const bool devem = chain && R.prm.EM_max_iter == 1;
    LmmseSetup A;
    vk::PreOut po;
    bool ahead = false;
    if (devem && R.pre_ahead_on && next) {
        const bool had = R.have_next;
        R.have_next = true;
        const vampomi_status st = lmmse_setup(c, R, it + 1, R.x1n, A);
        R.have_next = had;
        STCHK(st);
        po.tn = dsc + 8;
        po.tc = dsc + 9;
        po.Mt = (double)Mt;
        po.N = (double)N;
        po.out = dsc + 3;
        po.mirror = R.mixh_dev + vk::kMixWords;
        ahead = A.pre_in_cg && R.fuse && A.hs_av && A.sx.atx0 && po.tn && po.tc;
        A.pr.dev.scal = po.out;
// ... 243 lines not shown
```

Measured before the change: 167.3.

## Precompute next iteration's first CG step in idle slot of fused A^T A pass

```diff
diff --git a/include/vampomi.h b/include/vampomi.h
--- a/include/vampomi.h
+++ b/include/vampomi.h
@@ -163,6 +163,7 @@
 vampomi_status vampomi_reset_stats(vampomi_ctx* ctx);
 
 vampomi_status vampomi_dev_set_variant(vampomi_ctx* ctx, int which, int variant);
+vampomi_status vampomi_dev_prestep_counts(const vampomi_ctx* ctx, int64_t* made, int64_t* used);
 vampomi_status vampomi_dev_time_pass(vampomi_ctx* ctx, int which, int K, int reps, double* avg_ms);
 vampomi_status vampomi_dev_read_ceiling(vampomi_ctx* ctx, int reps, double* us_med, double* bytes, int* variant);
 vampomi_status vampomi_dev_kernel_name(const vampomi_ctx* ctx, int which, int K, int mode, char* out, int cap);
diff --git a/vampomi_amd/__init__.py b/vampomi_amd/__init__.py
--- a/vampomi_amd/__init__.py
+++ b/vampomi_amd/__init__.py
@@ -240,6 +240,11 @@
 
     def set_variant(self, which: int, variant: int):
         check(self._lib.vampomi_dev_set_variant(self.ctx, which, variant))
+
+    def prestep_counts(self) -> tuple:
+        made, used = C.c_int64(), C.c_int64()
+        check(self._lib.vampomi_dev_prestep_counts(self.ctx, C.byref(made), C.byref(used)))
+        return made.value, used.value
 
     def all_ok(self, local_ok: bool) -> bool:
         out = C.c_int()
diff --git a/vampomi_amd/_lib.py b/vampomi_amd/_lib.py
--- a/vampomi_amd/_lib.py
+++ b/vampomi_amd/_lib.py
@@ -125,6 +125,7 @@
     "vampomi_get_stats": (C.c_int, [_P, C.POINTER(Stats)]),
     "vampomi_reset_stats": (C.c_int, [_P]),
     "vampomi_dev_set_variant": (C.c_int, [_P, C.c_int, C.c_int]),
+    "vampomi_dev_prestep_counts": (C.c_int, [_P, C.POINTER(C.c_int64), C.POINTER(C.c_int64)]),
     "vampomi_dev_time_pass": (C.c_int, [_P, C.c_int, C.c_int, C.c_int, C.POINTER(C.c_double)]),
     "vampomi_dev_read_ceiling": (C.c_int, [_P, C.c_int, C.POINTER(C.c_double), C.POINTER(C.c_double),
                                            C.POINTER(C.c_int)]),
diff --git a/vampomi_amd/csrc/atax_team.hip b/vampomi_amd/csrc/atax_team.hip
--- a/vampomi_amd/csrc/atax_team.hip
+++ b/vampomi_amd/csrc/atax_team.hip
@@ -165,6 +165,33 @@
     return p;
 }
 
+template <int K>
+struct TmSlots {
+    const double* ar[K];
+    const double* p[K];
+    double* d[K];
+    double* sraw[K];
+    double diag[K], tau[K], gam2[K];
+};
+template <int K>
+__device__ __forceinline__ TmSlots<K> tm_slots(const OpArgs& a, int alt) {
+    TmSlots<K> s;
+#pragma unroll
+    for (int k = 0; k < K; ++k) {
+        int idx = k == alt ? kOpMaxK : k;
+        asm volatile("" : "+s"(idx));
+        const OpAlt::Slot& t = a.alt.tab[idx];
+        s.ar[k] = t.ar;
+        s.p[k] = t.p;
+        s.d[k] = t.d;
+        s.sraw[k] = t.sraw;
+        s.diag[k] = t.diag;
+        s.tau[k] = t.tau;
+        s.gam2[k] = t.gam2;
+    }
+    return s;
+}
+
 template <int K, int S, int F, int L, int P, bool COMM, int E, bool FMA, int KP>
 __device__ __forceinline__ void atax_team_body(const double* __restrict__ X, int64_t ld, int64_t N, int64_t M,
                                                const double* __restrict__ mave, const double* __restrict__ msig,
@@ -195,6 +222,11 @@
     }
     const double* beta = a.fold.on ? s_beta : a.beta;
     static_assert(K + KP <= kMaxRhs, "partial slots per team");
+    int fuse = a.fuse, alt = -1;
+    if constexpr (KP == 0) {
+        if (a.alt.cs && !a.fold.on) alt = cg_pre_slot(a.alt.cs->active, K, *a.alt.done == a.alt.token);
+        if (alt >= 0) fuse &= ~(1 << alt);
+    }
 #if TM_TS
     const unsigned long long ts0 = __builtin_amdgcn_s_memrealtime();
 #endif
@@ -232,6 +264,7 @@
     const int nbytes = (E == 2 ? (nrows + 1) & ~1 : nrows) * 8;
 
     if (COMM && wave == CW) {
+        const TmSlots<K> sl = tm_slots<K>(a, alt);
         const int nq = K * T;
         unsigned long long* xg = a.xg + (int64_t)team * nmax * nq * 2;
         unsigned long long* dummy = a.xg + gwords + (int64_t)blockIdx.x * 2 * K;
@@ -243,14 +276,14 @@
         const double* scp = msig;
 #pragma unroll
         for (int k = 0; k < K; ++k) {
-            if (lane == 1 + k) scp = a.p.p[k];
-            if (lane == 1 + K + k && ((a.fuse >> k) & 1)) scp = a.z.p[k];
+            if (lane == 1 + k) scp = sl.p[k];
+            if (lane == 1 + K + k && ((fuse >> k) & 1)) scp = a.z.p[k];
         }
         scp += mb;
         double bk[K], dpacc[K];
 #pragma unroll
         for (int k = 0; k < K; ++k) {
-            bk[k] = ((a.fuse >> k) & 1) ? beta[k] : 0.0;
+            bk[k] = ((fuse >> k) & 1) ? beta[k] : 0.0;
             dpacc[k] = 0.0;
         }
         v4u pl[RING];
@@ -332,9 +365,9 @@
                             double t = sg * readlane_d(v, 32 * k);
                             t *= a.scale;
                             double p = readlane_d(scv, 1 + k);
-                            if ((a.fuse >> k) & 1) p = readlane_d(scv, 1 + K + k) + bk[k] * p;
-                            double val = t * a.tau;
-                            val += a.gam2 * p;
+                            if ((fuse >> k) & 1) p = readlane_d(scv, 1 + K + k) + bk[k] * p;
+                            double val = t * sl.tau[k];
+                            val += sl.gam2[k] * p;
                             tsc[k] = t;
                             dval[k] = val;
                             pdir[k] = p;
@@ -346,8 +379,8 @@
 #pragma unroll
                             for (int k = 0; k < K; ++k) {
                                 if (lane == 0 && !(dbg & 1024)) {
-                                    if (a.sraw.p[0]) a.sraw.p[k][mg] = tsc[k];
-                                    *tm_chk(a.d.p[k] + mg, a.d.p[k], a.d.p[k] + M, 128, a.err) = dval[k];
+                                    if (a.sraw.p[0]) sl.sraw[k][mg] = tsc[k];
+                                    *tm_chk(sl.d[k] + mg, sl.d[k], sl.d[k] + M, 128, a.err) = dval[k];
                                 }
                                 dpacc[k] += dval[k] * pdir[k];
                             }
@@ -387,6 +420,7 @@
         return;
     }
 
+    const TmSlots<K> sl = tm_slots<K>(a, alt);
 #pragma unroll
     for (int s = 0; s < S; ++s) {
         const int jl = RS * s + jb;
@@ -398,8 +432,8 @@
                 double q = 0.0;
                 if (jl + h < nrows) {
                     const int64_t j = r0 + jl + h;
-                    q = a.ar.p[k][j] / a.diag;
-                    if ((a.fuse >> k) & 1) q = q + beta[k] * a.qo.p[k][j];
+                    q = sl.ar[k][j] / sl.diag[k];
+                    if ((fuse >> k) & 1) q = q + beta[k] * a.qo.p[k][j];
                 }
                 q_lds[k * QS + jl + h] = q;
             }
@@ -407,13 +441,13 @@
     }
     double bk[K];
 #pragma unroll
-    for (int k = 0; k < K; ++k) bk[k] = ((a.fuse >> k) & 1) ? beta[k] : 0.0;
+    for (int k = 0; k < K; ++k) bk[k] = ((fuse >> k) & 1) ? beta[k] : 0.0;
     const double* pkp = mave;
     if (lane == 1) pkp = msig;
 #pragma unroll
     for (int k = 0; k < K; ++k) {
-        if (lane == 2 + k) pkp = a.p.p[k];
-        if (lane == 2 + K + k && ((a.fuse >> k) & 1)) pkp = a.z.p[k];
+        if (lane == 2 + k) pkp = sl.p[k];
+        if (lane == 2 + K + k && ((fuse >> k) & 1)) pkp = a.z.p[k];
     }
 #pragma unroll
     for (int k = 0; k < KP; ++k)
@@ -542,13 +576,13 @@
                 double t = sg * tot[k];
                 t *= a.scale;
                 double p = readlane_d(pk[slot], 2 + k);
-                if ((a.fuse >> k) & 1) p = readlane_d(pk[slot], 2 + K + k) + bk[k] * p;
-                double val = t * a.tau;
-                val += a.gam2 * p;
+                if ((fuse >> k) & 1) p = readlane_d(pk[slot], 2 + K + k) + bk[k] * p;
+                double val = t * sl.tau[k];
+                val += sl.gam2[k] * p;
                 if (own) {
                     if (threadIdx.x == 0) {
-                        if (a.sraw.p[0]) a.sraw.p[k][mg] = t;
-                        a.d.p[k][mg] = val;
+                        if (a.sraw.p[0]) sl.sraw[k][mg] = t;
+                        sl.d[k][mg] = val;
                     }
                     dpacc[k] += val * p;
                 }
@@ -862,9 +896,18 @@
     }
 }
 
+static OpArgs tm_with_slots(const OpArgs& a, int K) {
+    OpArgs x = a;
+    for (int k = 0; k < K && k < kOpMaxK; ++k)
+        x.alt.tab[k] = OpAlt::Slot{a.ar.p[k], a.p.p[k], a.d.p[k], a.sraw.p[k], a.diag, a.tau, a.gam2};
+    x.alt.tab[kOpMaxK] = OpAlt::Slot{a.alt.ar, a.alt.p, a.alt.d, a.sraw.p[0] ? a.alt.d : nullptr, 1.0, 1.0, 0.0};
+    return x;
+}
+
 template <int K, bool PL = false>
-static hipError_t launch_tm_c(const Shard& s, const OpPlan& pl, const OpArgs& a, hipStream_t st, const Timing& tm,
+static hipError_t launch_tm_c(const Shard& s, const OpPlan& pl, const OpArgs& a0, hipStream_t st, const Timing& tm,
                         const int* gate, int* occ = nullptr) {
+    const OpArgs a = tm_with_slots(a0, K);
     if constexpr (PL) {
         switch (pl.cfg) {
             case 0: return launch_tm_s<1, 0, true>(pl.S, s, pl, a, st, tm, gate, occ);
diff --git a/vampomi_amd/csrc/ctx.h b/vampomi_amd/csrc/ctx.h
--- a/vampomi_amd/csrc/ctx.h
+++ b/vampomi_amd/csrc/ctx.h
@@ -119,6 +119,9 @@
     bool hs_ok = false;
     bool hs_on = true;
     bool hs_on_req = true;
+    int pre_mode = 2;
+    unsigned long long pre_seq = 0;
+    int64_t pre_made_n = 0, pre_used_n = 0;
     unsigned long long* op_ts = nullptr;
     double* nbuf = nullptr;
     double* mbuf = nullptr;
@@ -220,6 +223,13 @@
     const double* xnext = nullptr;
     double* axnext = nullptr;
     bool used = false;
+    double* T1 = nullptr;
+    double* U1 = nullptr;
+    unsigned long long* pre_done = nullptr;
+    bool pre_have = false;
+    bool pre_offer = false;
+    bool pre_made = false;
+    bool pre_used = false;
 };
 enum class PreMode { normal, ahead, queued };
 vampomi_status pcg_run(vampomi_ctx* c, const std::vector<CgSystem*>& sys, double tau, double gam2, int max_iter,
@@ -230,6 +240,8 @@
 vampomi_status op_prepare(vampomi_ctx* c);
 vampomi_status op_agree(vampomi_ctx* c);
 vampomi_status headstart_available(vampomi_ctx* c, bool* yes);
+constexpr int64_t kPreMinBytes = (int64_t)256 << 20;
+bool prestep_on(const vampomi_ctx* c);
 unsigned* op_err_dev(vampomi_ctx* c);
 vampomi_status op_check_err(vampomi_ctx* c);
 vampomi_status op_dev(vampomi_ctx* c, int K, const vk::OpArgs& a, const int* gate, bool reduce = true,
diff --git a/vampomi_amd/csrc/engine.cpp b/vampomi_amd/csrc/engine.cpp
--- a/vampomi_amd/csrc/engine.cpp
+++ b/vampomi_amd/csrc/engine.cpp
@@ -1054,6 +1054,10 @@
     if (const char* mv = std::getenv("VAMPOMI_MR_TAIL")) c->mr_tail = c->mr_tail_req = std::atoi(mv) != 0;
     if (const char* fv = std::getenv("VAMPOMI_CG_FOLD")) c->cg_fold = std::atoi(fv) != 0;
     if (const char* hv = std::getenv("VAMPOMI_HEADSTART")) c->hs_on = c->hs_on_req = std::atoi(hv) != 0;
+    if (const char* pv = std::getenv("VAMPOMI_PRESTEP")) {
+        const int v = std::atoi(pv);
+        if (v >= 0 && v <= 2) c->pre_mode = v;
+    }
     const char* mode = std::getenv("VAMPOMI_COMM");
     if (c->use_comm && mode && std::strcmp(mode, "loopback") == 0) {
         if (!d->comm_id) return fail(VAMPOMI_ERR_ARG, "the loopback communicator needs a communicator id");
@@ -1612,6 +1616,9 @@
         if (variant != 0 && variant != 1) return fail(VAMPOMI_ERR_ARG, "head start: 0 or 1");
         c->hs_on_req = variant == 1;
         if (!c->use_comm) c->hs_on = c->hs_on_req;
+    } else if (which == 7) {
+        if (variant < 0 || variant > 2) return fail(VAMPOMI_ERR_ARG, "pre-step: 0, 1 or 2");
+        c->pre_mode = variant;
     } else if (which == 6) {
         if (variant != 0 && variant != 1) return fail(VAMPOMI_ERR_ARG, "multi-rank tail: 0 or 1");
         c->mr_tail_req = variant == 1;
@@ -1620,6 +1627,18 @@
         if (!vk::loo_variant_ok(variant)) return fail(VAMPOMI_ERR_ARG, "no such association-pass variant");
         c->loo_variant = variant;
     }
+    return VAMPOMI_OK;
+}
+
+bool prestep_on(const vampomi_ctx* c) {
+    if (c->use_comm || c->nranks != 1 || !c->hs_ok || c->pre_mode == 0) return false;
+    return c->pre_mode == 1 || std::max<int64_t>(c->M, 1) * c->ld * 8 >= kPreMinBytes;
+}
+
+extern "C" vampomi_status vampomi_dev_prestep_counts(const vampomi_ctx* c, int64_t* made, int64_t* used) {
+    if (!c || !made || !used) return fail(VAMPOMI_ERR_ARG, "null argument");
+    *made = c->pre_made_n;
+    *used = c->pre_used_n;
     return VAMPOMI_OK;
 }
 
@@ -1814,6 +1833,7 @@
     for (int q = 0; q < 25; ++q) add(Mx, 8);
     add(ld, 8), add((int64_t)vk::kMaxRhs * ld, 8), add((int64_t)vk::kMaxRhs * ld, 8), add(ld, 8);
     add(2 * ld, 8);
+    add(Mx, 8), add(ld + 2, 8);
     if (probit) {
         for (int q = 0; q < 3; ++q) add(ld, 8);
         for (int q = 0; q < 3; ++q) add(Mx, 8);
diff --git a/vampomi_amd/csrc/kdev.h b/vampomi_amd/csrc/kdev.h
--- a/vampomi_amd/csrc/kdev.h
+++ b/vampomi_amd/csrc/kdev.h
@@ -82,11 +82,11 @@
 }
 
 __device__ inline void cg_publish(const CgState& s, bool ran, int it, CgMirror* mirror, unsigned long long* flag,
-                                  unsigned long long seq, int pack) {
+                                  unsigned long long seq, int pack, bool pre = false) {
     if (pack) {
         if (flag && ran)
-            __hip_atomic_store(flag, cg_pack(seq, s.any, s.iters[0], s.iters[1]), __ATOMIC_RELAXED,
-                               __HIP_MEMORY_SCOPE_SYSTEM);
+            __hip_atomic_store(flag, cg_pack(seq, s.any, s.iters[0], s.iters[1]) | (pre ? kCgPackPre : 0ull),
+                               __ATOMIC_RELAXED, __HIP_MEMORY_SCOPE_SYSTEM);
         return;
     }
     if (mirror) {
@@ -104,10 +104,11 @@
 }
 
 __device__ inline void cg_decide_from(CgState s, CgState* cs, const double* red, int it, CgMirror* mirror,
-                                      unsigned long long* flag, unsigned long long seq, int mask, int pack = 0) {
+                                      unsigned long long* flag, unsigned long long seq, int mask, int pack = 0,
+                                      bool pre = false) {
     const bool ran = cg_decide_into(s, red, it, mask);
     if (ran) *cs = s;
-    cg_publish(s, ran, it, mirror, flag, seq, pack);
+    cg_publish(s, ran, it, mirror, flag, seq, pack, pre);
 }
 
 __device__ inline void cg_decide_body(CgState* cs, const double* red, int it, CgMirror* mirror, unsigned long long* flag,
diff --git a/vampomi_amd/csrc/kernels.h b/vampomi_amd/csrc/kernels.h
--- a/vampomi_amd/csrc/kernels.h
+++ b/vampomi_amd/csrc/kernels.h
@@ -103,6 +103,22 @@
     unsigned long long* flag = nullptr;
     unsigned long long seq = 0;
 };
+struct OpAlt {
+    const CgState* cs = nullptr;
+    const unsigned long long* done = nullptr;
+    unsigned long long token = 0;
+    const double* ar = nullptr;
+    const double* p = nullptr;
+    double* d = nullptr;
+    struct Slot {
+        const double* ar;
+        const double* p;
+        double* d;
+        double* sraw;
+        double diag, tau, gam2;
+    };
+    Slot tab[2 + 1];
+};
 struct OpArgs {
     CPtrs ar, qo;
     CPtrs p, z;
@@ -119,7 +135,9 @@
     unsigned long long* ts;
     int dbg;
     OpFold fold;
-};
+    OpAlt alt;
+};
+static_assert(sizeof(OpAlt::tab) / sizeof(OpAlt::Slot) == kOpMaxK + 1, "one entry per system and the alternate's");
 std::string op_kernel_name(int K, const OpPlan& pl);
 std::string team_kernel_name(int K, const OpPlan& pl);
 int team_occupancy(const OpPlan& pl, int K);
@@ -295,7 +313,16 @@
     int64_t adld;
     int adslots;
     double addiv;
-};
+    double* pre_u1;
+    unsigned long long* pre_done;
+    unsigned long long pre_token;
+};
+__host__ __device__ inline int cg_pre_slot(const int* active, int K, bool made) {
+    if (made) return -1;
+    for (int k = 0; k < K && k < kMaxRhs; ++k)
+        if (!active[k]) return k;
+    return -1;
+}
 hipError_t cg_init(int K, int64_t M, const CgVecs& c, double diag, const RedOut& ro, hipStream_t st);
 struct CgState {
     double rz[kMaxRhs], vv[kMaxRhs], prev_ons[kMaxRhs], beta[kMaxRhs];
@@ -308,6 +335,7 @@
     return (seq << 32) | ((unsigned long long)(any ? 1 : 0) << 30) | ((unsigned long long)(it1 & 0x7fff) << 15) |
            (unsigned long long)(it0 & 0x7fff);
 }
+constexpr unsigned long long kCgPackPre = 1ull << 31;
 struct CgMirror {
     unsigned long long seq;
     int any;
@@ -331,5 +359,16 @@
                      const double* pp_dev, int fuse, const RedOut& ro, const CgDecide& dc, hipStream_t st);
 hipError_t cg_decide(CgState* cs, const double* red, int it, CgMirror* mirror, unsigned long long* flag,
                      unsigned long long seq, hipStream_t st, int mask = 0xf, int pack = 0);
+struct PreCompose {
+    const double* T1;
+    const double* U1;
+    const double* ab;
+    const double* p;
+    double* d;
+    double* S;
+    double* AD;
+    double diag, tau, gam2;
+};
+hipError_t pre_compose(int64_t M, int64_t N, const PreCompose& a, const RedOut& ro, hipStream_t st);
 
 }
diff --git a/vampomi_amd/csrc/kernels.hip b/vampomi_amd/csrc/kernels.hip
--- a/vampomi_amd/csrc/kernels.hip
+++ b/vampomi_amd/csrc/kernels.hip
@@ -1822,6 +1822,7 @@
     }
 #endif
     if (!st.any) return;
+    const int pre = c.pre_u1 ? cg_pre_slot(st.active, K, *c.pre_done == c.pre_token) : -1;
     __shared__ double fin[3 * kMaxRhs];
     const bool mpart = (int)blockIdx.x < mblocks;
     double alpha[K];
@@ -1934,6 +1935,10 @@
                     if (c.AW[k]) c.AW[k][j] = awv[e] + alk * q;
                     c.AR[k][j] = arv[e] - ad[e] * alk;
                 }
+            } else if (w == 0 && ok && k == pre) {
+                const v2d ad = (((wsum[0][lane] + wsum[1][lane]) + wsum[2][lane]) + wsum[3][lane]) / c.addiv;
+                c.pre_u1[i] = ad[0];
+                if (i + 1 < c.nA) c.pre_u1[i + 1] = ad[1];
             }
             __syncthreads();
         }
@@ -1984,8 +1989,9 @@
         double r[3 * kMaxRhs];
 #pragma unroll
         for (int q = 0; q < 3 * kMaxRhs; ++q) r[q] = q < 3 * K ? fin[q] : 0.0;
-        cg_decide_from(st, cs, r, dc.it, dc.mirror, dc.flag, dc.seq, dc.mask, dc.pack);
-    }
+        cg_decide_from(st, cs, r, dc.it, dc.mirror, dc.flag, dc.seq, dc.mask, dc.pack, pre >= 0);
+    }
+    if (last && pre >= 0 && threadIdx.x == 0) *c.pre_done = c.pre_token;
 }
 
 constexpr int kCguBlocks = 512;
@@ -2024,6 +2030,34 @@
 hipError_t cg_decide(CgState* cs, const double* red, int it, CgMirror* mirror, unsigned long long* flag,
                      unsigned long long seq, hipStream_t st, int mask, int pack) {
     hipLaunchKernelGGL(cg_decide_kernel, dim3(1), dim3(64), 0, st, cs, red, it, mirror, flag, seq, mask, pack);
+    return hipGetLastError();
+}
+
+__global__ __launch_bounds__(kBlock) void pre_compose_kernel(int64_t M, int64_t N, PreCompose a, RedOut ro) {
+    if (ro.gate && !*ro.gate) return;
+    __shared__ double lds[4];
+    double acc[1] = {0.0};
+    const int64_t stride = (int64_t)gridDim.x * kBlock;
+    for (int64_t i = (int64_t)blockIdx.x * kBlock + threadIdx.x; i < M; i += stride) {
+        const double t = a.T1[i] / a.diag;
+        const double p = a.p[i];
+        double d = t * a.tau;
+        d += a.gam2 * p;
+        a.d[i] = d;
+        if (a.S) a.S[i] = t;
+        acc[0] += d * p;
+    }
+    for (int64_t j = (int64_t)blockIdx.x * kBlock + threadIdx.x; j < N; j += stride) {
+        double u = a.tau * a.U1[j];
+        u += a.gam2 * a.ab[j];
+        a.AD[j] = u / a.diag;
+    }
+    block_put_sums<1>(acc, 1, ro, (int64_t)blockIdx.x);
+    red_finish(ro, 1, lds);
+}
+
+hipError_t pre_compose(int64_t M, int64_t N, const PreCompose& a, const RedOut& ro, hipStream_t st) {
+    hipLaunchKernelGGL(pre_compose_kernel, dim3(red_blocks(M)), dim3(kBlock), 0, st, M, N, a, ro);
     return hipGetLastError();
 }
 
diff --git a/vampomi_amd/csrc/pcg.cpp b/vampomi_amd/csrc/pcg.cpp
--- a/vampomi_amd/csrc/pcg.cpp
+++ b/vampomi_amd/csrc/pcg.cpp
@@ -14,6 +14,7 @@
 
 struct CgOutcome {
     int any = 0;
+    bool pre = false;
     int iters[vk::kMaxRhs] = {};
 };
 
@@ -42,6 +43,7 @@
                 return fail(VAMPOMI_ERR_STATE, "CG step " + std::to_string(i - 1) + ": decision word holds sequence " +
                                                    std::to_string(w >> 32) + ", expected " + std::to_string(prev));
             o.any = (int)((w >> 30) & 1);
+            o.pre = last->pre || (w & vk::kCgPackPre) != 0;
             o.iters[0] = (int)(w & 0x7fff);
             o.iters[1] = (int)((w >> 15) & 0x7fff);
         } else {
@@ -75,6 +77,7 @@
     if (extra_x && (!ex_out || K + 1 >= vk::kMaxRhs)) return fail(VAMPOMI_ERR_ARG, "pcg: extra A.x needs K <= 2");
     if (hs) {
         hs->used = false;
+        hs->pre_made = hs->pre_used = false;
         if (!onepass || K != 2 || !extra_x || ar0 || sys[0]->mu0_nonzero || (hs->xnext && !hs->axnext))
             return fail(VAMPOMI_ERR_ARG, "pcg: the head start needs the one-pass form, two systems, extra_x, "
                                          "system 0 from zero and no ar0");
@@ -126,12 +129,15 @@
         cv.d[k] = (s->mu0_nonzero && !s->atx0) ? s->d : nullptr;
     }
     const bool head = hs && hs->abern && c->hs_ok && c->op_ok && max_iter > 0;
+    const bool pre_ok = hs && op1 && !c->use_comm && c->opp.T >= 1 && hs->T1 && hs->U1 && hs->pre_done &&
+                        max_iter > 0 && max_iter < vk::kCgPackMaxIter;
+    const bool pre2 = head && pre_ok && hs->pre_have;
     vk::CgState s0{};
     s0.K = K;
     s0.gam2 = gam2;
     s0.tol = tol;
     s0.maxit = max_iter;
-    s0.off[0] = head ? 1 : 0;
+    s0.off[0] = head ? (pre2 ? 2 : 1) : 0;
     s0.any = max_iter > 0 ? 1 : 0;
     for (int k = 0; k < K; ++k) {
         s0.active[k] = 1;
@@ -260,6 +266,31 @@
             for (int k = 0; k < K; ++k)
                 if (!sys[k]->S) return fail(VAMPOMI_ERR_ARG, "pcg: W needs an S scratch vector for every system");
         const int all = (1 << K) - 1;
+        if (pre2) {
+            vk::PreCompose pc{};
+            pc.T1 = hs->T1;
+            pc.U1 = hs->U1;
+            pc.ab = cu.AR[0];
+            pc.p = sys[0]->p;
+            pc.d = sys[0]->d;
+            pc.S = rec ? sys[0]->S : nullptr;
+            pc.AD = const_cast<double*>(cu.AD[0]);
+            pc.diag = diag;
+            pc.tau = tau;
+            pc.gam2 = gam2;
+            HIPCHK(vk::pre_compose(M, N, pc, vk::RedOut{c->red_part, c->scal + SL_DP, c->ticket, nullptr, 0, gate},
+                                   c->st));
+            vk::CgVecs cp = cu;
+            cp.adpart = nullptr;
+            cp.addiv = 0.0;
+            const vk::RedOut ro{c->red_part, c->scal + SL_CG, c->ticket, nullptr, 0, gate};
+            vk::CgDecide dc{};
+            dc.on = 1;
+            dc.it = -2;
+            dc.mask = 1;
+            HIPCHK(vk::cg_update(1, M, cp, diag, c->cgs, c->scal + SL_DP, nullptr, 0, ro, dc, c->st));
+            hs->pre_used = true;
+        }
         if (head) {
             vk::OpArgs a{};
             a.ar.p[0] = cu.AR[0];
@@ -269,7 +300,7 @@
             a.d.p[0] = sys[0]->d;
             a.sraw.p[0] = rec ? sys[0]->S : nullptr;
             a.beta = beta;
-            a.fuse = 0;
+            a.fuse = pre2 ? 1 : 0;
             a.diag = diag;
             a.tau = tau;
             a.gam2 = gam2;
@@ -285,7 +316,7 @@
             dc.on = !c->use_comm;
             dc.it = -1;
             dc.mask = 1;
-            HIPCHK(vk::cg_update(1, M, ch, diag, c->cgs, dp, nullptr, 0, ro, dc, c->st));
+            HIPCHK(vk::cg_update(1, M, ch, diag, c->cgs, dp, nullptr, pre2 ? 1 : 0, ro, dc, c->st));
             if (c->use_comm) {
                 STCHK(allreduce_dev(c, c->scal + SL_CG, 3));
                 if (fold) {
@@ -299,6 +330,14 @@
             hs->used = true;
         }
         const bool packed = K <= 2 && max_iter < vk::kCgPackMaxIter;
+        const bool offer = pre_ok && packed && hs->pre_offer && hs->xnext && hs->axnext && !fold;
+        const unsigned long long token = offer ? ++c->pre_seq : 0;
+        vk::CgVecs cuo = cu;
+        if (offer) {
+            cuo.pre_u1 = hs->U1;
+            cuo.pre_done = hs->pre_done;
+            cuo.pre_token = token;
+        }
         auto enqueue = [&](int i, unsigned long long* seq) -> vampomi_status {
             const int fuse = i > 0 ? all : head ? 1 : 0;
             vk::OpArgs a{};
@@ -311,6 +350,14 @@
                 a.sraw.p[k] = rec ? sys[k]->S : nullptr;
             }
             a.beta = fold ? nullptr : beta;
+            if (offer) {
+                a.alt.cs = c->cgs;
+                a.alt.done = hs->pre_done;
+                a.alt.token = token;
+                a.alt.ar = hs->axnext;
+                a.alt.p = hs->xnext;
+                a.alt.d = hs->T1;
+            }
             a.fuse = fuse;
             a.diag = diag;
             a.tau = tau;
@@ -351,7 +398,7 @@
                 dc.seq = *seq;
                 dc.pack = packed ? 1 : 0;
             }
-            HIPCHK(vk::cg_update(K, M, cu, diag, cs, dp, nullptr, fuse, ro, dc, c->st));
+            HIPCHK(vk::cg_update(K, M, cuo, diag, cs, dp, nullptr, fuse, ro, dc, c->st));
             if (c->use_comm) {
                 STCHK(allreduce_dev(c, c->scal + SL_CG, (size_t)(3 * K)));
                 if (fold) {
@@ -382,6 +429,7 @@
             sys[k]->iters = last.iters[k];
             if (ref_passes) *ref_passes += 2 * (int64_t)sys[k]->iters;
         }
+        if (offer) hs->pre_made = last.pre;
         return VAMPOMI_OK;
     }
     if (xnext) {
diff --git a/vampomi_amd/csrc/run.h b/vampomi_amd/csrc/run.h
--- a/vampomi_amd/csrc/run.h
+++ b/vampomi_amd/csrc/run.h
@@ -50,6 +50,9 @@
     double* ax2 = nullptr;
     double* abern = nullptr;
     double* bern_next = nullptr;
+    double* pre_t1 = nullptr;
+    double* pre_u1 = nullptr;
+    int pre_it = 0;
     double* mixw = nullptr;
     double* mixh = nullptr;
     double* mixh_dev = nullptr;
diff --git a/vampomi_amd/csrc/vamp.cpp b/vampomi_amd/csrc/vamp.cpp
--- a/vampomi_amd/csrc/vamp.cpp
+++ b/vampomi_amd/csrc/vamp.cpp
@@ -11,7 +11,7 @@
 VampRun::~VampRun() {
     if (writer) writer->drain(nullptr);
     for (double** p : {&r1, &x1, &x1p, &x1n, &x1d, &r2, &x2, &bern, &invQ, &v, &atxy, &ts, &tmpM, &atx0, &z1buf,
-                       &nb3, &nsc, &ax2, &p1, &p2, &z1h, &x1s, &x1sn, &x2s, &abern, &bern_next})
+                       &nb3, &nsc, &ax2, &p1, &p2, &z1h, &x1s, &x1sn, &x2s, &abern, &bern_next, &pre_t1, &pre_u1})
         dev_free(*p);
     for (auto& p : cgw) dev_free(p);
     dev_free(mixw);
@@ -208,6 +208,10 @@
     STCHK(dev_alloc(&R.nsc, vk::kMaxRhs * ld));
     STCHK(dev_alloc(&R.ax2, ld));
     STCHK(dev_alloc(&R.abern, 2 * ld));
+    STCHK(dev_alloc(&R.pre_t1, M));
+    STCHK(dev_alloc(&R.pre_u1, ld + 2));
+    HIPCHK(hipMemsetAsync(R.pre_t1, 0, M * 8, c->st));
+    HIPCHK(hipMemsetAsync(R.pre_u1, 0, (ld + 2) * 8, c->st));
     STCHK(dev_alloc(&R.mixw, vk::kMixWords));
     HIPCHK(hipHostMalloc((void**)&R.mixh, (vk::kMixWords + 4) * sizeof(double),
                          hipHostMallocMapped | hipHostMallocCoherent));
@@ -235,6 +239,7 @@
     HIPCHK(hipSetDevice(c->device));
     STCHK(op_agree(c));
     c->run.reset(new VampRun());
+    c->pre_made_n = c->pre_used_n = 0;
     VampRun& R = *c->run;
     R.prm = *p;
     R.res = r;
@@ -427,6 +432,13 @@
             L.hs.xnext = R.bern_next;
             L.hs.axnext = R.abern + ((it + 1) & 1) * ld;
         }
+        if (prestep_on(c)) {
+            L.hs.T1 = R.pre_t1;
+            L.hs.U1 = R.pre_u1;
+            L.hs.pre_done = reinterpret_cast<unsigned long long*>(R.pre_u1 + ld);
+            L.hs.pre_have = L.hs.abern && R.pre_it == it;
+            L.hs.pre_offer = L.hs.xnext != nullptr;
+        }
     }
     vk::Prelude& pr = L.pr;
     pr.eta1 = R.eta1;
@@ -536,12 +548,16 @@
         STCHK(pcg_run(c, {&so, &sx}, R.gamw, R.gam2, R.prm.CG_max_iter, R.prm.CG_err_tol, R.nsc, &R.passes_ref,
                       nullptr, R.x1, R.z1buf, true, nullptr, &hs, &pr, pm));
         R.hs_it = hs.xnext ? it + 1 : 0;
+        R.pre_it = hs.pre_made ? it + 1 : 0;
+        c->pre_made_n += hs.pre_made ? 1 : 0;
+        c->pre_used_n += hs.pre_used ? 1 : 0;
     } else if (R.fuse) {
         STCHK(pcg_run(c, {&sx, &so}, R.gamw, R.gam2, R.prm.CG_max_iter, R.prm.CG_err_tol, R.nsc, &R.passes_ref,
                       arec ? nullptr : &e1, arec ? R.x1 : nullptr, arec ? R.z1buf : nullptr, R.onepass, nullptr,
                       nullptr, arec ? &pr : nullptr));
-        R.hs_it = 0;
+        R.hs_it = R.pre_it = 0;
     } else {
+        R.pre_it = 0;
         STCHK(pcg_run(c, {&sx}, R.gamw, R.gam2, R.prm.CG_max_iter, R.prm.CG_err_tol, R.nsc, &R.passes_ref, &e1));
         STCHK(pcg_run(c, {&so}, R.gamw, R.gam2, R.prm.CG_max_iter, R.prm.CG_err_tol, R.nsc, &R.passes_ref, nullptr));
     }
```

Result: faster. 183.0 (median of 6 runs) (+9.4%).
